# Deltares/xugrid

Hardware: AMD Instinct MI355X
Metric: target cells regridded/s (OverlapRegridder 1M->1M tri, weights + mean apply) (higher is better)
Workload: dtype f64; 1 GPU; BASELINE config 2: ~1M-triangle jittered-lattice Delaunay source -> ~1M-triangle target (seed 1, rotated 30 deg, scaled 0.7), OverlapRegridder area-weighted mean, K=1; target_faces=999660, candidate_pairs=6677422, nnz=4052965, parallelism=1 GPU

## Files before the change

include/xugrid_amd.h:

```cpp
#ifndef XUGRID_AMD_H
#define XUGRID_AMD_H

#include <stdint.h>

#ifdef __cplusplus
extern "C" {
#endif

#define XR_OK 0
#define XR_ERR_INVALID (-1)
#define XR_ERR_NO_DEVICE (-2)
#define XR_ERR_HIP (-3)
#define XR_ERR_LIMIT (-4)

#define XR_MEAN 0
#define XR_HARMONIC_MEAN 1
#define XR_GEOMETRIC_MEAN 2
#define XR_SUM 3
#define XR_MINIMUM 4
#define XR_MAXIMUM 5
#define XR_MODE 6
#define XR_PERCENTILE 7
#define XR_FIRST_ORDER_CONSERVATIVE 8
#define XR_MAX_OVERLAP 9
// ... 46 lines not shown
int xr_mesh_face_bounds_dev(xr_mesh *mesh, double *out_dev);

int xr_overlap(xr_mesh *tree, xr_mesh *query, int relative, xr_csr **out);
int xr_overlap_stats(const xr_mesh *tree, int64_t *n_candidates);
int xr_overlap_apply_dev(xr_mesh *tree, xr_mesh *query, int relative, int method, double percentile,
                         const void *source_dev, int source_dtype, int64_t K, double *out_dev, xr_csr **out);

int xr_locate_points(xr_mesh *mesh, const double *points, int64_t n, double tolerance,
                     int64_t *face_index_out);
int xr_locate_raster(xr_mesh *mesh, const double *x, int64_t nx, const double *y, int64_t ny,
                     double tolerance, int64_t *face_index_out);
int xr_barycentric(xr_mesh *mesh, const double *points, int64_t n, double tolerance,
                   int64_t *face_index_out, double *weights_out);

int xr_replace_interpolated_weights(const double *vertices, int64_t n_vertex, const int64_t *faces, int64_t n_face,
                                    int64_t m, const int64_t *face_index, double *weights, int64_t n,
                                    const int64_t *node_to_node_map, int64_t n_map);

int xr_locate_csr(xr_mesh *tree, xr_mesh *query, const double *points, int64_t n, double tolerance,
                  xr_csr **out);

int xr_barycentric_csr(xr_mesh *voronoi, xr_mesh *source, xr_mesh *query, const double *points,
                       int64_t n, double tolerance, const int64_t *vertex_face,
                       const int64_t *node_to_node_map, int64_t n_extra, xr_csr **out);
int xr_barycentric_csr_tail(xr_mesh *voronoi, xr_mesh *source, xr_mesh *query, const double *points, int64_t n,
                            double tolerance, int64_t n_identity, const int64_t *vertex_face_tail,
                            const int64_t *node_to_node_map, int64_t n_extra, int tree_order, xr_csr **out);

typedef struct xr_points xr_points;
int xr_locate_flags_begin(xr_mesh *source, xr_mesh *query, const double *points, int64_t n, xr_points **out);
int xr_points_destroy(xr_points *points);
int xr_barycentric_csr_points(xr_mesh *voronoi, xr_mesh *source, xr_points *points, double tolerance, int64_t n_identity,
                              const int64_t *vertex_face_tail, const int64_t *node_to_node_map, int64_t n_extra,
                              int tree_order, xr_csr **out);

typedef struct xr_voronoi xr_voronoi;
int xr_voronoi_create(xr_mesh *mesh, xr_voronoi **out);
int xr_voronoi_create_flags(xr_mesh *mesh, int add_exterior, int add_vertices, int skip_concave, const double *generators_dev,
                            xr_voronoi **out);
int xr_voronoi_vertex_info(const xr_voronoi *v, int64_t *n_generator_vertex, int64_t *max_used_face);
int xr_voronoi_info(const xr_voronoi *v, int64_t *n_node, int64_t *nnz, int64_t *n_exterior_edge,
                    int64_t *n_interior_cell, int64_t *max_interior_degree);
int xr_voronoi_download(const xr_voronoi *v, int64_t *indptr, int64_t *indices, int64_t *edge_nodes,
                        int64_t *edge_face, double *centroids);
int xr_voronoi_boundary_info(xr_voronoi *v, int64_t *n_boundary_node, int64_t *n_boundary_entry);
int xr_voronoi_boundary(xr_voronoi *v, int64_t *nodes, int64_t *row_ptr, int64_t *faces, double *face_xy,
                        int64_t *edge_nodes, int64_t *edge_face, double *edge_face_xy);
int xr_voronoi_mesh(const xr_voronoi *v, const double *extra_xy, int64_t n_extra_vertex,
                    const int64_t *boundary_cells, int64_t n_boundary_cell, int64_t n_max_boundary,
                    xr_mesh **out);
int xr_voronoi_mesh_auto(xr_voronoi *v, xr_mesh **out, int64_t *n_tail, int64_t *n_map);
int xr_voronoi_tail(xr_voronoi *v, int64_t *tail_face_index, int64_t *interpolation_map);
int xr_voronoi_boundary_cells_info(xr_voronoi *v, int64_t *n_extra_vertex, int64_t *n_cell, int64_t *n_max);
int xr_voronoi_boundary_cells(xr_voronoi *v, double *extra_xy, int64_t *cells);
int xr_voronoi_destroy(xr_voronoi *v);

int xr_csr_info(const xr_csr *csr, int64_t *n, int64_t *m, int64_t *nnz);
int xr_csr_download(const xr_csr *csr, double *data, int64_t *indices, int64_t *indptr);
int xr_csr_upload(const double *data, const int64_t *indices, const int64_t *indptr, int64_t n,
                  int64_t m, int64_t nnz, xr_csr **out);
int xr_csr_from_triplet(const int64_t *row, const int64_t *col, const double *data, int64_t nnz,
                        int64_t n, int64_t m, xr_csr **out);
int xr_csr_from_outer(const int64_t *indptr_y, const int64_t *source_y, const double *weight_y,
                      int64_t n_target_y, int64_t n_source_y, const int64_t *indptr_x,
                      const int64_t *source_x, const double *weight_x, int64_t n_target_x,
                      int64_t n_source_x, xr_csr **out);
int xr_outer_create(const int64_t *indptr_y, const int64_t *source_y, const double *weight_y,
                    int64_t n_target_y, int64_t n_source_y, const int64_t *indptr_x,
                    const int64_t *source_x, const double *weight_x, int64_t n_target_x,
                    int64_t n_source_x, xr_outer **out);
int xr_outer_info(const xr_outer *outer, int64_t *n, int64_t *m, int64_t *nnz);
int xr_outer_csr(xr_outer *outer, const xr_csr **out);
int xr_outer_destroy(xr_outer *outer);
int xr_edge_length_csr(xr_mesh *tree, const double *edge_xy, int64_t n_edge, xr_csr **out);
int xr_edge_length_csr_dev(xr_mesh *tree, const double *edge_xy_dev, int64_t n_edge, xr_csr **out);
int xr_edge_pieces(xr_mesh *tree, const xr_csr *csr, const double *edge_xy, int64_t n_edge,
                   double *intersections);
int xr_csr_set_row_keys(xr_csr *csr, const int64_t *keys, int64_t key_range);
int xr_csr_set_col_keys(xr_csr *csr, const int64_t *keys, int64_t key_range);
int xr_csr_col_order(const xr_csr *csr, int64_t *order_out);
int xr_csr_expect_permuted(xr_csr *csr, int permuted);
int xr_csr_output_stored_order(xr_csr *csr, int stored);
int xr_csr_row_order(const xr_csr *csr, int64_t K_hint, int64_t *order_out);
int xr_csr_destroy(xr_csr *csr);

int xr_apply_csr(const xr_csr *csr, int method, double percentile, const void *source,
                 int source_dtype, int64_t K, double *out);
int xr_apply_csr_dev(const xr_csr *csr, int method, double percentile, const void *source_dev,
                     int source_dtype, int64_t K, double *out_dev);
int xr_apply_outer(xr_outer *outer, int method, double percentile, const void *source,
                   int source_dtype, int64_t K, double *out);
int xr_apply_outer_dev(xr_outer *outer, int method, double percentile, const void *source_dev,
                       int source_dtype, int64_t K, double *out_dev);
int xr_apply_coo(const int64_t *row, const int64_t *col, int64_t nnz, int64_t T,
                 const void *source, int source_dtype, int64_t K, int64_t S, double *out);

int xr_shard_plan_dev(const double *src_xy_dev, const int64_t *src_faces_dev, int64_t n_src_face, int src_m,
                      const double *tgt_xy_dev, const int64_t *tgt_faces_dev, int64_t n_tgt_face, int tgt_m, int world, int rank,
                      int mode, int64_t *local_faces_dev, int64_t *n_local_faces, int64_t *local_targets_dev,
                      int64_t *n_local_targets, int32_t *owner_dev);

int xr_partial_components(int method);
int xr_partial_combine_is_max(int method);
int xr_apply_partial_dev(const xr_csr *csr, int method, const void *source_dev, int source_dtype, int64_t K,
                         double *out_dev, int rows_layout);
int xr_overlap_partial_dev(xr_mesh *tree, xr_mesh *query, int relative, int method, const void *source_dev, int source_dtype,
                           int64_t K, double *out_dev, int rows_layout, xr_csr **out);
int xr_partial_fill_identity_dev(int method, double *planes_dev, int64_t K, int64_t T);
int xr_finalize_partial_dev(int method, const double *planes_dev, int64_t K, int64_t T, double *out_dev);
int xr_reduce_partial_rows_dev(int method, const double *rows_dev, const int64_t *indptr_dev, const int64_t *order_dev,
                               int64_t n_targets, int64_t K, double *out_dev);

typedef struct xr_graph xr_graph;
int xr_graph_from_csr(const int64_t *indptr, const int64_t *indices, const double *data, int64_t n, int64_t nnz,
                      const int64_t *labels, xr_graph **out);
int xr_graph_info(const xr_graph *graph, int64_t *n, int64_t *nnz);
int xr_graph_download(const xr_graph *graph, int64_t *indptr, int64_t *indices, double *data, int64_t *labels);
int xr_graph_destroy(xr_graph *graph);
#define XR_FILL_CONVERGED 0
#define XR_FILL_MAXITER 1
#define XR_FILL_BREAKDOWN 2
#define XR_FILL_NODATA 3
int xr_graph_laplace_fill_dev(const xr_graph *graph, const double *in_dev, double *out_dev, int64_t K, int use_weights,
                              double atol, double rtol, int64_t maxiter, int64_t chunk, int64_t *iterations_out,
                              int *status_out);
int xr_nearest_fill_dev(const double *xy_dev, int64_t n, const double *in_dev, double *out_dev, int64_t K, double max_distance);

typedef struct xr_topology xr_topology;
int xr_topology_create(xr_mesh *mesh, xr_topology **out);
int xr_topology_info(const xr_topology *topology, int64_t *n_edge, int64_t *n_exterior_edge, int64_t *face_face_nnz,
                     int64_t *node_node_nnz, int64_t *n_nonmanifold);
int xr_topology_long_nodes(const xr_topology *topology, int64_t *n_long_nodes);
int xr_topology_download(const xr_topology *topology, int64_t *edge_node, int64_t *face_edge, int64_t *edge_face,
                         int64_t *ff_indptr, int64_t *ff_indices, int64_t *ff_data, int64_t *nn_indptr, int64_t *nn_indices,
                         int64_t *nn_data, int64_t *exterior_edge, int64_t *exterior_face);
int xr_topology_edge_xy_dev(const xr_topology *topology, double *xy_dev);
int xr_topology_exterior_face_dev(const xr_topology *topology, uint8_t *flags_dev);
int xr_topology_destroy(xr_topology *topology);
int xr_topology_download_node_tables(const xr_topology *topology, int64_t *nf_indptr, int64_t *nf_indices, int64_t *ne_indptr,
                                     int64_t *ne_indices);
int xr_graph_from_topology(const xr_topology *topology, int facet, xr_graph **out);
int xr_graph_label_rounds(const xr_graph *graph, int64_t *rounds);

int xr_graph_components_dev(const xr_graph *graph, int64_t *labels_dev, int64_t *n_components);
int xr_graph_binary_iterate_dev(const xr_graph *graph, const uint8_t *in_dev, uint8_t *out_dev, int64_t K, int value,
                                int64_t iterations, const uint8_t *mask_dev, const uint8_t *exterior_dev);

int xr_graph_rcm_dev(const xr_graph *graph, int64_t *order_dev, int64_t *levels_out);

int xr_graph_partition_dev(const xr_graph *graph, const double *xy_dev, const int64_t *weights_dev, int64_t n_part,
                           int64_t *labels_dev, int64_t *info);
int xr_mesh_reorder_faces_dev(const xr_mesh *mesh, const int64_t *order_dev, xr_mesh **out);

int xr_network_graph_dev(const double *node_xy_dev, int64_t n_node, const int64_t *edges_dev, int64_t n_edge, int facet,
                         xr_graph **out, int64_t *problems);
int xr_graph_nearest_dev(const xr_graph *graph, const uint8_t *is_source_dev, int64_t K, double limit, int64_t chunk,
                         double *distance_dev, int64_t *source_dev, int64_t *rounds_out);
int xr_graph_nearest_fill_dev(const xr_graph *graph, const double *in_dev, double *out_dev, int64_t K, double limit,
                              int64_t chunk, int64_t *rounds_out);

#define XR_FACET_MEAN 0
#define XR_FACET_SUM 1
#define XR_FACET_MIN 2
#define XR_FACET_MAX 3
#define XR_FACET_RAW 4
int xr_topology_facet_map_dev(xr_topology *topology, int target, int source, int form, const void *in_dev, int dtype, int64_t K,
// ... 139 lines not shown
```

xugrid_amd/_lib.py:

```python
import ctypes
import os

_HERE = os.path.dirname(os.path.abspath(__file__))
LIB_PATH = os.environ.get("XUGRID_AMD_LIB") or os.path.join(_HERE, "libxugrid_amd.so")

XR_OK = 0
XR_ERR_INVALID = -1
XR_ERR_NO_DEVICE = -2
XR_ERR_HIP = -3
XR_ERR_LIMIT = -4

XR_F64 = 0
XR_F32 = 1
XR_I32 = 2


class XugridAmdError(RuntimeError):
    """HIP runtime failure, missing device or missing shared library."""


c_i64 = ctypes.c_int64
c_f64 = ctypes.c_double
c_int = ctypes.c_int
vp = ctypes.c_void_p
# ... 2 lines not shown
p_int = ctypes.POINTER(ctypes.c_int)
p_vp = ctypes.POINTER(ctypes.c_void_p)

SIGNATURES = {
    "xr_last_error": (ctypes.c_char_p, []),
    "xr_device_count": (c_int, [p_int]),
    "xr_init": (c_int, [c_int]),
    "xr_current_device": (c_int, [p_int]),
    "xr_trim_pool": (c_int, []),
    "xr_version": (c_int, []),
    "xr_set_stream": (c_int, [vp, c_int, c_int]),
    "xr_set_async": (c_int, [c_int]),
    "xr_set_option": (c_int, [ctypes.c_char_p, ctypes.c_int64]),
    "xr_get_option": (c_int, [ctypes.c_char_p, ctypes.POINTER(ctypes.c_int64)]),
    "xr_host_copy": (c_int, [vp, vp, c_i64]),
    "xr_host_interleave2": (c_int, [vp, c_i64, vp, c_i64, c_i64, vp]),
    "xr_mesh_create": (c_int, [vp, c_i64, vp, c_int, c_i64, c_i64, c_i64, p_vp]),
    "xr_mesh_create_dev": (c_int, [vp, c_i64, vp, c_int, c_i64, c_i64, c_i64, p_vp]),
    "xr_mesh_create_rectilinear": (c_int, [vp, c_i64, vp, c_i64, p_vp]),
    "xr_mesh_destroy": (c_int, [vp]),
    "xr_mesh_info": (c_int, [vp, p_i64, p_i64, p_i64]),
    "xr_mesh_device_bytes": (c_int, [vp, p_i64]),
    "xr_mesh_prepare": (c_int, [vp]),
    "xr_mesh_build_index": (c_int, [vp]),
    "xr_mesh_invalidate": (c_int, [vp]),
    "xr_mesh_area": (c_int, [vp, vp]),
    "xr_mesh_centroids": (c_int, [vp, vp]),
    "xr_mesh_centroids_dev": (c_int, [vp, vp]),
    "xr_mesh_faces": (c_int, [vp, vp]),
    "xr_mesh_download": (c_int, [vp, vp, vp]),
    "xr_mesh_triangulate": (c_int, [vp, p_vp]),
    "xr_mesh_triangle_face_dev": (c_int, [vp, vp]),
    "xr_mesh_circumcenters_dev": (c_int, [vp, vp]),
    "xr_mesh_perimeter_dev": (c_int, [vp, vp]),
    "xr_mesh_face_bounds_dev": (c_int, [vp, vp]),
    "xr_voronoi_create": (c_int, [vp, p_vp]),
    "xr_voronoi_create_flags": (c_int, [vp, c_int, c_int, c_int, vp, p_vp]),
    "xr_voronoi_vertex_info": (c_int, [vp, p_i64, p_i64]),
    "xr_voronoi_info": (c_int, [vp, p_i64, p_i64, p_i64, p_i64, p_i64]),
    "xr_voronoi_download": (c_int, [vp, vp, vp, vp, vp, vp]),
    "xr_voronoi_boundary_info": (c_int, [vp, vp, vp]),
    "xr_voronoi_boundary": (c_int, [vp, vp, vp, vp, vp, vp, vp, vp]),
    "xr_voronoi_mesh": (c_int, [vp, vp, c_i64, vp, c_i64, c_i64, p_vp]),
    "xr_voronoi_mesh_auto": (c_int, [vp, p_vp, p_i64, p_i64]),
    "xr_voronoi_tail": (c_int, [vp, vp, vp]),
    "xr_voronoi_boundary_cells_info": (c_int, [vp, p_i64, p_i64, p_i64]),
    "xr_voronoi_boundary_cells": (c_int, [vp, vp, vp]),
    "xr_voronoi_destroy": (c_int, [vp]),
    "xr_overlap": (c_int, [vp, vp, c_int, p_vp]),
    "xr_overlap_stats": (c_int, [vp, p_i64]),
    "xr_overlap_apply_dev": (c_int, [vp, vp, c_int, c_int, c_f64, vp, c_int, c_i64, vp, p_vp]),
    "xr_overlap_partial_dev": (c_int, [vp, vp, c_int, c_int, vp, c_int, c_i64, vp, c_int, p_vp]),
    "xr_shard_plan_dev": (c_int, [vp, vp, c_i64, c_int, vp, vp, c_i64, c_int, c_int, c_int, c_int, vp, p_i64, vp, p_i64, vp]),
    "xr_locate_points": (c_int, [vp, vp, c_i64, c_f64, vp]),
    "xr_locate_raster": (c_int, [vp, vp, c_i64, vp, c_i64, c_f64, vp]),
    "xr_barycentric": (c_int, [vp, vp, c_i64, c_f64, vp, vp]),
    "xr_locate_csr": (c_int, [vp, vp, vp, c_i64, c_f64, p_vp]),
    "xr_replace_interpolated_weights": (c_int, [vp, c_i64, vp, c_i64, c_i64, vp, vp, c_i64, vp, c_i64]),
    "xr_barycentric_csr": (c_int, [vp, vp, vp, vp, c_i64, c_f64, vp, vp, c_i64, p_vp]),
    "xr_barycentric_csr_tail": (c_int, [vp, vp, vp, vp, c_i64, c_f64, c_i64, vp, vp, c_i64, c_int, p_vp]),
    "xr_locate_flags_begin": (c_int, [vp, vp, vp, c_i64, p_vp]),
    "xr_points_destroy": (c_int, [vp]),
    "xr_barycentric_csr_points": (c_int, [vp, vp, vp, c_f64, c_i64, vp, vp, c_i64, c_int, p_vp]),
    "xr_csr_info": (c_int, [vp, p_i64, p_i64, p_i64]),
    "xr_csr_download": (c_int, [vp, vp, vp, vp]),
    "xr_csr_upload": (c_int, [vp, vp, vp, c_i64, c_i64, c_i64, p_vp]),
    "xr_csr_from_triplet": (c_int, [vp, vp, vp, c_i64, c_i64, c_i64, p_vp]),
    "xr_csr_from_outer": (c_int, [vp, vp, vp, c_i64, c_i64, vp, vp, vp, c_i64, c_i64, p_vp]),
    "xr_outer_create": (c_int, [vp, vp, vp, c_i64, c_i64, vp, vp, vp, c_i64, c_i64, p_vp]),
    "xr_outer_info": (c_int, [vp, vp, vp, vp]),
    "xr_outer_csr": (c_int, [vp, p_vp]),
    "xr_outer_destroy": (c_int, [vp]),
    "xr_apply_outer": (c_int, [vp, c_int, c_f64, vp, c_int, c_i64, vp]),
    "xr_apply_outer_dev": (c_int, [vp, c_int, c_f64, vp, c_int, c_i64, vp]),
    "xr_edge_length_csr": (c_int, [vp, vp, c_i64, p_vp]),
    "xr_edge_length_csr_dev": (c_int, [vp, vp, c_i64, p_vp]),
    "xr_edge_pieces": (c_int, [vp, vp, vp, c_i64, vp]),
    "xr_csr_set_row_keys": (c_int, [vp, vp, c_i64]),
    "xr_csr_set_col_keys": (c_int, [vp, vp, c_i64]),
    "xr_csr_col_order": (c_int, [vp, vp]),
    "xr_csr_expect_permuted": (c_int, [vp, c_int]),
    "xr_csr_output_stored_order": (c_int, [vp, c_int]),
    "xr_csr_row_order": (c_int, [vp, c_i64, vp]),
    "xr_csr_destroy": (c_int, [vp]),
    "xr_apply_csr": (c_int, [vp, c_int, c_f64, vp, c_int, c_i64, vp]),
    "xr_apply_csr_dev": (c_int, [vp, c_int, c_f64, vp, c_int, c_i64, vp]),
    "xr_apply_coo": (c_int, [vp, vp, c_i64, c_i64, vp, c_int, c_i64, c_i64, vp]),
    "xr_partial_components": (c_int, [c_int]),
    "xr_partial_combine_is_max": (c_int, [c_int]),
    "xr_apply_partial_dev": (c_int, [vp, c_int, vp, c_int, c_i64, vp, c_int]),
    "xr_partial_fill_identity_dev": (c_int, [c_int, vp, c_i64, c_i64]),
    "xr_finalize_partial_dev": (c_int, [c_int, vp, c_i64, c_i64, vp]),
    "xr_reduce_partial_rows_dev": (c_int, [c_int, vp, vp, vp, c_i64, c_i64, vp]),
    "xr_graph_from_csr": (c_int, [vp, vp, vp, c_i64, c_i64, vp, p_vp]),
    "xr_graph_info": (c_int, [vp, p_i64, p_i64]),
    "xr_graph_download": (c_int, [vp, vp, vp, vp, vp]),
    "xr_graph_destroy": (c_int, [vp]),
    "xr_graph_laplace_fill_dev": (c_int, [vp, vp, vp, c_i64, c_int, c_f64, c_f64, c_i64, c_i64, vp, vp]),
    "xr_nearest_fill_dev": (c_int, [vp, c_i64, vp, vp, c_i64, c_f64]),
    "xr_network_graph_dev": (c_int, [vp, c_i64, vp, c_i64, c_int, p_vp, p_i64]),
    "xr_graph_nearest_dev": (c_int, [vp, vp, c_i64, c_f64, c_i64, vp, vp, p_i64]),
    "xr_graph_nearest_fill_dev": (c_int, [vp, vp, vp, c_i64, c_f64, c_i64, p_i64]),
    "xr_topology_create": (c_int, [vp, p_vp]),
    "xr_topology_info": (c_int, [vp, p_i64, p_i64, p_i64, p_i64, p_i64]),
    "xr_topology_long_nodes": (c_int, [vp, p_i64]),
    "xr_topology_download": (c_int, [vp, vp, vp, vp, vp, vp, vp, vp, vp, vp, vp, vp]),
    "xr_topology_download_node_tables": (c_int, [vp, vp, vp, vp, vp]),
    "xr_topology_edge_xy_dev": (c_int, [vp, vp]),
    "xr_topology_exterior_face_dev": (c_int, [vp, vp]),
    "xr_topology_destroy": (c_int, [vp]),
    "xr_graph_from_topology": (c_int, [vp, c_int, p_vp]),
    "xr_graph_label_rounds": (c_int, [vp, p_i64]),
    "xr_graph_components_dev": (c_int, [vp, vp, p_i64]),
    "xr_graph_binary_iterate_dev": (c_int, [vp, vp, vp, c_i64, c_int, c_i64, vp, vp]),
    "xr_graph_rcm_dev": (c_int, [vp, vp, p_i64]),
    "xr_mesh_reorder_faces_dev": (c_int, [vp, vp, p_vp]),
    "xr_graph_partition_dev": (c_int, [vp, vp, vp, c_i64, vp, p_i64]),
    "xr_topology_facet_map_dev": (c_int, [vp, c_int, c_int, c_int, vp, c_int, c_i64, vp]),
    "xr_topology_facet_width": (c_int, [vp, c_int, c_int, p_i64]),
    "xr_facet_map_dev": (c_int, [vp, vp, c_i64, c_i64, c_i64, c_int, vp, c_int, c_i64, vp]),
    "xr_nn_create_dev": (c_int, [vp, c_i64, p_vp]),
    "xr_nn_create_mesh": (c_int, [vp, c_int, p_vp]),
    "xr_nn_info": (c_int, [vp, p_i64, p_i64]),
    "xr_nn_destroy": (c_int, [vp]),
    "xr_nn_query_dev": (c_int, [vp, vp, c_i64, c_f64, vp]),
    "xr_gather_points_dev": (c_int, [vp, c_int, c_i64, c_i64, vp, c_i64, c_f64, vp]),
    "xr_section_coords_dev": (c_int, [vp, vp, c_i64, vp, c_i64, vp, vp]),
    "xr_burn_polygons_dev": (c_int, [vp, vp, c_i64, vp, c_i64, vp, c_i64, c_int, vp]),
    "xr_burn_lines_dev": (c_int, [vp, vp, c_i64, vp, c_i64, vp]),
    "xr_burn_points_dev": (c_int, [vp, vp, c_i64, vp]),
    "xr_burn_combine_dev": (c_int, [c_i64, vp, vp, vp, vp, vp, vp, c_f64, vp]),
    "xr_polygonize_dev": (c_int, [vp, vp, c_int, p_vp]),
    "xr_polygons_info": (c_int, [vp, p_i64, p_i64, p_i64, p_i64, p_i64]),
    "xr_polygons_readbacks": (c_int, [vp, p_i64]),
    "xr_polygons_copy_dev": (c_int, [vp, vp, vp, vp, vp, vp]),
    "xr_polygons_destroy": (c_int, [vp]),
    "xr_mesh_subset_dev": (c_int, [vp, vp, c_i64, p_vp, p_int, p_i64]),
    "xr_mesh_subset_node_index_dev": (c_int, [vp, vp]),
    "xr_index_check_dev": (c_int, [vp, c_i64, c_i64, p_i64]),
    "xr_index_mismatch_dev": (c_int, [vp, vp, c_i64, p_i64]),
    "xr_index_from_mask_dev": (c_int, [vp, c_i64, p_vp]),
    "xr_mesh_box_faces_dev": (c_int, [vp, c_f64, c_f64, c_f64, c_f64, p_vp]),
    "xr_mesh_faces_of_nodes_dev": (c_int, [vp, vp, c_i64, p_vp]),
    "xr_topology_faces_of_edges_dev": (c_int, [vp, vp, c_i64, p_vp]),
    "xr_topology_subset_edges_dev": (c_int, [vp, vp, c_i64, p_vp]),
    "xr_index_info": (c_int, [vp, p_i64]),
    "xr_index_copy_dev": (c_int, [vp, vp]),
    "xr_index_destroy": (c_int, [vp]),
    "xr_merge_meshes_dev": (c_int, [vp, c_i64, p_vp]),
    "xr_merge_edges_dev": (c_int, [vp, vp, c_i64, vp]),
    "xr_merge_info": (c_int, [vp, p_i64, p_i64, p_i64]),
    "xr_merge_take_mesh": (c_int, [vp, p_vp]),
    "xr_merge_index_info": (c_int, [vp, c_int, c_i64, p_i64]),
    "xr_merge_index_copy_dev": (c_int, [vp, c_int, c_i64, c_int, vp]),
    "xr_merge_node_inverse_copy_dev": (c_int, [vp, vp]),
    "xr_merge_destroy": (c_int, [vp]),
    "xr_index_like_dev": (c_int, [vp, vp, c_i64, c_f64, vp, p_i64]),
    "xr_labels_range_dev": (c_int, [vp, c_i64, p_i64, p_i64]),
    "xr_labels_order_dev": (c_int, [vp, c_i64, c_i64, p_vp, p_i64]),
    "xr_label_order_copy_dev": (c_int, [vp, c_i64, c_i64, vp]),
    "xr_label_order_destroy": (c_int, [vp]),
    "xr_dev_copy_columns": (c_int, [vp, c_i64, vp, c_i64, c_i64]),
    "xr_periodic_wrap_dev": (c_int, [vp, p_vp, p_i64]),
    "xr_periodic_unwrap_dev": (c_int, [vp, c_f64, p_vp]),
    "xr_periodic_edges_dev": (c_int, [vp, vp, vp, p_i64]),
    "xr_periodic_info": (c_int, [vp, p_i64]),
# ... 80 lines not shown
```

xugrid_amd/csrc/xr_apply.hip:

```cpp
#include <cstdlib>
#include <cstring>
#include <vector>

#include "xr_apply.h"
#include "xr_reduce.h"
#include "xr_prims.h"

namespace xr {

static constexpr int KT = 16;

template <int METHOD, typename SRC>
__device__ __forceinline__ void apply_row_block(const int32_t *__restrict__ indptr, const int32_t *__restrict__ indices,
                                                const double *__restrict__ data, const int32_t *__restrict__ row_order,
                                                int t, int64_t T, int64_t S, const SRC *__restrict__ source, int64_t K,
                                                double *__restrict__ out, double (*lds)[3]) {
    const int s = indptr[t], e = indptr[t + 1];
    const int64_t t_out = row_order ? (int64_t)row_order[t] : t;
    double normsum = 0.0;
    if (METHOD == XR_GEOMETRIC_MEAN) {
        Red<XR_SUM> ws;
        for (int j = s + threadIdx.x; j < e; j += AP_BLOCK) ws.b += data[j];
        block_merge<XR_SUM>(ws, lds);
        normsum = ws.b;
    }
    for (int64_t k = blockIdx.y; k < K; k += gridDim.y) {
        const SRC *src = source + k * S;
        Red<METHOD> r;
        int j = s + threadIdx.x;
        for (; j + 3 * AP_BLOCK < e; j += 4 * AP_BLOCK) {
            const int c0 = indices[j], c1 = indices[j + AP_BLOCK], c2 = indices[j + 2 * AP_BLOCK],
                      c3 = indices[j + 3 * AP_BLOCK];
            const double w0 = data[j], w1 = data[j + AP_BLOCK], w2 = data[j + 2 * AP_BLOCK],
                         w3 = data[j + 3 * AP_BLOCK];
            const double v0 = ld_src(src, c0), v1 = ld_src(src, c1), v2 = ld_src(src, c2), v3 = ld_src(src, c3);
            r.add(v0, w0, normsum);
            r.add(v1, w1, normsum);
            r.add(v2, w2, normsum);
            r.add(v3, w3, normsum);
        }
        for (; j < e; j += AP_BLOCK) r.add(ld_src(src, indices[j]), data[j], normsum);
        block_merge<METHOD>(r, lds);
        if (threadIdx.x == 0) {
            double v = r.fin();
            if (METHOD == XR_GEOMETRIC_MEAN && normsum == 0) v = NAN;
            out[k * T + t_out] = v;
        }
    }
}

template <int METHOD, typename SRC>
__global__ void __launch_bounds__(AP_BLOCK)
k_apply_long(const int32_t *__restrict__ indptr, const int32_t *__restrict__ indices, const double *__restrict__ data,
             const int32_t *__restrict__ row_order, const int32_t *__restrict__ long_rows,
             const int32_t *__restrict__ n_long, int64_t T, int64_t S, const SRC *__restrict__ source, int64_t K,
             double *__restrict__ out) {
    __shared__ double lds[AP_BLOCK / 64][3];
    const int nl = *n_long;
    for (int li = blockIdx.x; li < nl; li += gridDim.x)
        apply_row_block<METHOD, SRC>(indptr, indices, data, row_order, long_rows[li], T, S, source, K, out, lds);
}

static constexpr int APPLY_GROUP16 = 512;

template <int METHOD, typename SRC, int KTILE, int G>
__device__ __forceinline__ void apply_row_group(const int32_t *__restrict__ indices, const double *__restrict__ data,
                                                int s, int e, int64_t t_out, int64_t T, int64_t S,
                                                const SRC *__restrict__ source, int64_t K, double *__restrict__ out) {
    const int gl = threadIdx.x & (G - 1);
    int col4[4];
    double w4[4];
#pragma unroll
    for (int u = 0; u < 4; u++) {
        const int j = s + gl + G * u;
        col4[u] = j < e ? indices[j] : -1;
        w4[u] = j < e ? data[j] : 0.0;
    }
    double normsum = 0.0;
    if (METHOD == XR_GEOMETRIC_MEAN) {
        Red<XR_SUM> ws;
        for (int j = s + gl; j < e; j += G) ws.b += data[j];
        group_merge<XR_SUM, G>(ws);
        normsum = ws.b;
    }
    for (int64_t k0 = (int64_t)blockIdx.y * KTILE; k0 < K; k0 += (int64_t)gridDim.y * KTILE) {
        const int kn = (int)((K - k0) < KTILE ? (K - k0) : KTILE);
        const SRC *src = source + k0 * S;
        Red<METHOD> r[KTILE];
        double v[4][KTILE];
#pragma unroll
        for (int u = 0; u < 4; u++)
#pragma unroll
            for (int kk = 0; kk < KTILE; kk++)
                v[u][kk] = (col4[u] >= 0 && kk < kn) ? ld_src(src, (int64_t)kk * S + col4[u]) : 0.0;
#pragma unroll
        for (int u = 0; u < 4; u++) {
            if (col4[u] >= 0) {
#pragma unroll
                for (int kk = 0; kk < KTILE; kk++)
                    if (kk < kn) r[kk].add(v[u][kk], w4[u], normsum);
            }
        }
        for (int j = s + gl + 4 * G; j < e; j += G) {
            const int64_t col = indices[j];
            const double w = data[j];
            double vv[KTILE];
#pragma unroll
            for (int kk = 0; kk < KTILE; kk++) vv[kk] = kk < kn ? ld_src(src, (int64_t)kk * S + col) : 0.0;
#pragma unroll
            for (int kk = 0; kk < KTILE; kk++)
                if (kk < kn) r[kk].add(vv[kk], w, normsum);
        }
#pragma unroll
        for (int kk = 0; kk < KTILE; kk++) group_merge<METHOD, G>(r[kk]);
        if (gl == 0) {
#pragma unroll
            for (int kk = 0; kk < KTILE; kk++) {
                if (kk < kn) {
                    double res = r[kk].fin();
                    if (METHOD == XR_GEOMETRIC_MEAN && normsum == 0) res = NAN;
                    out[(k0 + kk) * T + t_out] = res;
                }
            }
        }
    }
}

template <int METHOD, typename SRC, int KTILE>
__device__ __forceinline__ void apply_wave_rows(const int32_t *__restrict__ indptr, const int32_t *__restrict__ indices,
                                                const double *__restrict__ data, const int32_t *__restrict__ row_order,
                                                const int32_t *__restrict__ long_rows, int nl, int wave, int n_waves,
                                                int64_t T, int64_t S, const SRC *__restrict__ source, int64_t K,
                                                double *__restrict__ out, int32_t *__restrict__ huge_rows) {
    const int lane = threadIdx.x & 63;
    for (int li0 = wave * 4; li0 < nl; li0 += n_waves * 4) {
        const int li = li0 + (lane >> 4);
        int s = 0, e = 0;
        int64_t t_out = 0;
        if (li < nl) {
            const int t = long_rows[li];
            s = indptr[t];
            e = indptr[t + 1];
            t_out = row_order ? (int64_t)row_order[t] : t;
            if (e - s > APPLY_GROUP16) e = s;
        }
        if (__any(e > s)) {
            if (e > s) apply_row_group<METHOD, SRC, KTILE, 16>(indices, data, s, e, t_out, T, S, source, K, out);
        }
    }
    for (int li = wave; li < nl; li += n_waves) {
        const int t = long_rows[li];
        const int s = indptr[t], e = indptr[t + 1];
        if (e - s <= APPLY_GROUP16) continue;
        if (e - s > APPLY_WAVE) {
            if (huge_rows && lane == 0 && blockIdx.y == 0) huge_rows[1 + atomicAdd(huge_rows, 1)] = t;
            continue;
        }
        const int64_t t_out = row_order ? (int64_t)row_order[t] : t;
        apply_row_group<METHOD, SRC, KTILE, 64>(indices, data, s, e, t_out, T, S, source, K, out);
    }
}

template <int METHOD, typename SRC, int KTILE>
__global__ void __launch_bounds__(AP_BLOCK)
k_apply_wave(const int32_t *__restrict__ indptr, const int32_t *__restrict__ indices, const double *__restrict__ data,
             const int32_t *__restrict__ row_order, const int32_t *__restrict__ long_rows,
             const int32_t *__restrict__ n_long, int64_t T, int64_t S, const SRC *__restrict__ source, int64_t K,
             double *__restrict__ out, int32_t *__restrict__ huge_rows) {
    const int wave = (blockIdx.x * AP_BLOCK + threadIdx.x) >> 6, n_waves = gridDim.x * (AP_BLOCK / 64);
    apply_wave_rows<METHOD, SRC, KTILE>(indptr, indices, data, row_order, long_rows, *n_long, wave, n_waves, T, S, source, K,
                                        out, huge_rows);
}

template <int METHOD, typename SRC>
__global__ void __launch_bounds__(AP_BLOCK)
k_apply_rows1(const int32_t *__restrict__ indptr, const int32_t *__restrict__ indices, const double *__restrict__ data,
              const int32_t *__restrict__ row_order, const int32_t *__restrict__ long_rows,
              const int32_t *__restrict__ n_long, int n_long_blocks, bool any_huge, int64_t T, int64_t S,
              const SRC *__restrict__ source, double *__restrict__ out, const int32_t *__restrict__ gate) {
    __shared__ double2 sh_win[AP_BLOCK / 64][W1_CAP];
    if (gate && *gate == 0) return;
    double(*sh_merge)[3] = reinterpret_cast<double(*)[3]>(&sh_win[0][0]);
    const int lane = threadIdx.x & 63, wib = threadIdx.x >> 6;
    if ((int)blockIdx.x < n_long_blocks) {
        const int nl = *n_long;
        apply_wave_rows<METHOD, SRC, 1>(indptr, indices, data, row_order, long_rows, nl, (int)blockIdx.x * (AP_BLOCK / 64) + wib,
                                        n_long_blocks * (AP_BLOCK / 64), T, S, source, 1, out, nullptr);
        if (any_huge) {
            int *sh_list = reinterpret_cast<int *>(&sh_win[1][0]), *sh_cnt = reinterpret_cast<int *>(&sh_win[2][0]);
            for (int base = 0; base < nl; base += n_long_blocks * AP_BLOCK) {
                if (threadIdx.x == 0) *sh_cnt = 0;
                __syncthreads();
                const int li = base + (int)blockIdx.x + n_long_blocks * (int)threadIdx.x;
                if (li < nl) {
                    const int t = long_rows[li];
                    if (indptr[t + 1] - indptr[t] > APPLY_WAVE) sh_list[atomicAdd(sh_cnt, 1)] = t;
                }
                __syncthreads();
                const int n_hit = *sh_cnt;
                for (int i = 0; i < n_hit; i++)
                    apply_row_block<METHOD, SRC>(indptr, indices, data, row_order, sh_list[i], T, S, source, 1, out, sh_merge);
                __syncthreads();
            }
        }
        return;
    }
    const int64_t row0 = ((int64_t)(gridDim.x - 1 - blockIdx.x) * (AP_BLOCK / 64) + wib) * 64;
    if (row0 >= T) return;
    const int64_t t = row0 + lane;
    int s = 0, e = 0;
    if (t < T) {
        s = indptr[t];
        e = indptr[t + 1];
    }
    const bool skip = n_long_blocks > 0 && (e - s > APPLY_LONG);
    const int seg0 = __shfl(s, 0, 64);
    const int seg1 = wave_reduce<OpMax>(e);
    if (skip) e = s;
    const bool jumpy = __any(skip);
    double2 *win = sh_win[wib];
    auto next_chunk = [&](int c0) -> int {
        if (!jumpy) return c0;
        int mine = (e > s && e > c0) ? (s > c0 ? s : c0) : INT_MAX;
        return wave_reduce<OpMin>(mine);
    };
    double normsum = 0.0;
    if (METHOD == XR_GEOMETRIC_MEAN) {
        for (int c0 = seg0; c0 < seg1; c0 += W1_CAP) {
            c0 = next_chunk(c0);
            if (c0 >= seg1) break;
            for (int j = c0 + lane; j < c0 + W1_CAP && j < seg1; j += 64) win[j - c0].x = data[j];
            __builtin_amdgcn_fence(__ATOMIC_RELEASE, "wavefront");
            __builtin_amdgcn_wave_barrier();
            __builtin_amdgcn_fence(__ATOMIC_ACQUIRE, "wavefront");
            const int a = s > c0 ? s : c0, b = e < c0 + W1_CAP ? e : c0 + W1_CAP;
            for (int j = a; j < b; j++) normsum += win[j - c0].x;
            __builtin_amdgcn_fence(__ATOMIC_RELEASE, "wavefront");
            __builtin_amdgcn_wave_barrier();
        }
    }
    Red<METHOD> red;
    for (int c0 = seg0; c0 < seg1; c0 += W1_CAP) {
        c0 = next_chunk(c0);
        if (c0 >= seg1) break;
        {
            constexpr int PER = W1_CAP / 64;
            int col[PER];
            double w[PER];
#pragma unroll
            for (int u = 0; u < PER; u++) {
                const int j = c0 + u * 64 + lane;
                col[u] = j < seg1 ? indices[j] : -1;
                w[u] = j < seg1 ? data[j] : 0.0;
            }
            double v[PER];
#pragma unroll
            for (int u = 0; u < PER; u++) v[u] = col[u] >= 0 ? ld_src(source, (int64_t)col[u]) : 0.0;
#pragma unroll
            for (int u = 0; u < PER; u++)
                if (col[u] >= 0) win[u * 64 + lane] = make_double2(w[u], v[u]);
        }
        __builtin_amdgcn_fence(__ATOMIC_RELEASE, "wavefront");
        __builtin_amdgcn_wave_barrier();
        __builtin_amdgcn_fence(__ATOMIC_ACQUIRE, "wavefront");
        const int a = s > c0 ? s : c0, b = e < c0 + W1_CAP ? e : c0 + W1_CAP;
        for (int j = a; j < b; j++) {
            const double2 wv = win[j - c0];
            red.add(wv.y, wv.x, normsum);
        }
        __builtin_amdgcn_fence(__ATOMIC_RELEASE, "wavefront");
        __builtin_amdgcn_wave_barrier();
    }
    if (t < T && !skip) {
        const int64_t t_out = row_order ? (int64_t)row_order[t] : t;
        double r = NAN;
        if (e > s) {
            r = red.fin();
            if (METHOD == XR_GEOMETRIC_MEAN && normsum == 0) r = NAN;
        }
        out[t_out] = r;
    }
}

template <int METHOD, typename SRC, int KTILE>
__global__ void __launch_bounds__(AP_BLOCK)
k_apply_direct(const int32_t *__restrict__ indptr, const int32_t *__restrict__ indices,
               const double *__restrict__ data, const int32_t *__restrict__ row_order, bool skip_long, int64_t T,
               int64_t S, const SRC *__restrict__ source, int64_t K, double *__restrict__ out,
               const int32_t *__restrict__ block_list) {
    const int64_t t = (int64_t)(block_list ? block_list[blockIdx.x] : blockIdx.x) * AP_BLOCK + threadIdx.x;
    if (t >= T) return;
    const int64_t k0 = (int64_t)blockIdx.y * KTILE;
    const int kn = (int)((K - k0) < KTILE ? (K - k0) : KTILE);
    const int s = indptr[t], e = indptr[t + 1];
    if (skip_long && e - s > APPLY_LONG) return;
    const int64_t t_out = row_order ? (int64_t)row_order[t] : t;
    const SRC *src = source + k0 * S;
    double normsum = 0.0;
    if (METHOD == XR_GEOMETRIC_MEAN)
        for (int j = s; j < e; j++) normsum += data[j];
    Red<METHOD> red[KTILE];
    int j = s;
    if (KTILE <= 4) {
        for (; j + 3 < e; j += 4) {
            int64_t col[4];
            double w[4], v[4][KTILE];
#pragma unroll
            for (int u = 0; u < 4; u++) {
                col[u] = indices[j + u];
                w[u] = data[j + u];
            }
#pragma unroll
            for (int u = 0; u < 4; u++)
#pragma unroll
                for (int kk = 0; kk < KTILE; kk++) v[u][kk] = kk < kn ? ld_src(src, (int64_t)kk * S + col[u]) : 0.0;
#pragma unroll
            for (int u = 0; u < 4; u++)
#pragma unroll
                for (int kk = 0; kk < KTILE; kk++)
                    if (kk < kn) red[kk].add(v[u][kk], w[u], normsum);
        }
    }
    for (; j < e; j++) {
        const int64_t col = indices[j];
        const double w = data[j];
        double v[KTILE];
#pragma unroll
        for (int kk = 0; kk < KTILE; kk++) v[kk] = kk < kn ? ld_src(src, (int64_t)kk * S + col) : 0.0;
#pragma unroll
        for (int kk = 0; kk < KTILE; kk++)
            if (kk < kn) red[kk].add(v[kk], w, normsum);
    }
#pragma unroll
    for (int kk = 0; kk < KTILE; kk++) {
        if (kk < kn) {
            double r = NAN;
            if (e > s) {
                r = red[kk].fin();
                if (METHOD == XR_GEOMETRIC_MEAN && normsum == 0) r = NAN;
            }
            out[(k0 + kk) * T + t_out] = r;
        }
    }
}

static constexpr int PLAN_LMAX = 4096;
static constexpr int PLAN_UMAX = 512;

__global__ void __launch_bounds__(AP_BLOCK)
k_plan_build(const int32_t *__restrict__ indptr, const int32_t *__restrict__ indices, int64_t T,
             int32_t *__restrict__ ucol, int32_t *__restrict__ nuniq, uint16_t *__restrict__ loc,
             int32_t *__restrict__ max_entries, int32_t *__restrict__ unplanned, int32_t *__restrict__ n_unplanned,
             int entry_cap) {
    __shared__ int32_t keys[PLAN_LMAX];
    __shared__ int32_t uniq[PLAN_UMAX];
    __shared__ int32_t sh_wave[4];
    __shared__ int32_t sh_lines;
    const int64_t row0 = (int64_t)blockIdx.x * AP_BLOCK;
    const int64_t row_end = row0 + AP_BLOCK < T ? row0 + AP_BLOCK : T;
    const int seg0 = indptr[row0], seg1 = indptr[row_end];
    const int n = seg1 - seg0;
    if (n > entry_cap) {
        if (threadIdx.x == 0) {
            nuniq[blockIdx.x] = -1;
// ... 700 lines not shown

template <int METHOD, typename SRC, int KT, int SUBS, bool MERGED, bool FAST>
static void launch_plan(const xr_csr *csr, const SRC *src, int64_t K, double *out) {
    const int plan_dbg = (int)option(OPT_PLAN_DBG);
    const int lmax = csr->plan_lmax;
    const size_t sub_bytes = ((sizeof(double) * ((size_t)KT * PLAN_UMAX + lmax) + sizeof(uint16_t) * lmax) + 15) / 16 * 16;
    const size_t stage_bytes = ((sizeof(double) * (size_t)lmax + sizeof(uint16_t) * (size_t)lmax) + 15) / 16 * 16;
    const size_t shmem = MERGED ? sizeof(double) * (size_t)KT * PLAN_GUMAX + stage_bytes * PLAN_GROUP : sub_bytes * SUBS;
    XR_REQUIRE(shmem <= (size_t)160 * 1024, XR_ERR_LIMIT, "internal: apply plan needs %zu bytes of LDS", shmem);
    {
        static std::mutex attr_mutex;
        static size_t granted = 0;
        std::lock_guard<std::mutex> lock(attr_mutex);
        if (shmem > granted) {
            XR_HIP(hipFuncSetAttribute(reinterpret_cast<const void *>(&k_apply_plan<METHOD, SRC, KT, SUBS, MERGED, FAST>),
                                       hipFuncAttributeMaxDynamicSharedMemorySize, (int)shmem));
            granted = shmem;
        }
    }
    const int64_t n_groups = div_up(div_up(csr->n, AP_BLOCK), SUBS);
    const int item_tiles = 64 / KT;
    const int super_blocks = K > (int64_t)KT * item_tiles ? (int)std::min<int64_t>((n_groups + 7) / 8, 1 << 30) : 0;
    int64_t plan_grid = (n_groups + 7) / 8 * 8;
    if (super_blocks > 0) {
        const int64_t per_xcd = (n_groups + 7) / 8;
        const int64_t n_items = div_up(K, (int64_t)KT * item_tiles);
        plan_grid = 8 * div_up(per_xcd, super_blocks) * super_blocks * n_items;
    }
    XR_LAUNCH("apply_plan", (k_apply_plan<METHOD, SRC, KT, SUBS, MERGED, FAST>), dim3((unsigned)plan_grid), dim3(AP_BLOCK * SUBS),
              shmem, csr->indptr.get(), csr->indices.get(), csr->data.get(), csr->plan_ucol.get(), csr->plan_nuniq.get(),
              csr->plan_loc.get(), row_order_of(csr), csr->has_long, csr->n, csr->m, src, K, out, csr->plan_lmax, super_blocks,
              item_tiles, plan_dbg);
}

template <int METHOD, typename SRC>
static void launch_stream(const xr_csr *csr, const SRC *src, int64_t K, double *out) {
    DevBuf<int32_t> huge;
    if (csr->has_long) huge.alloc((size_t)(csr->nnz / APPLY_WAVE + 2));
    auto launch_long_rows = [&](bool zeroed) {
        if (!zeroed) XR_HIP(hipMemsetAsync(huge.get(), 0, sizeof(int32_t), launch_stream()));
        if (K == 1) {
            dim3 wgrid((unsigned)engine().num_cu * 16, 1);
            XR_LAUNCH("apply_wave", (k_apply_wave<METHOD, SRC, 1>), wgrid, dim3(AP_BLOCK), 0, csr->indptr.get(),
                      csr->indices.get(), csr->data.get(), row_order_of(csr), csr->long_rows.get(), csr->n_long.get(),
                      csr->n, csr->m, src, K, out, huge.get());
        } else {
            constexpr int WT = 8;
            const unsigned wy = (unsigned)std::min<int64_t>(div_up(K, WT), 8);
            dim3 wgrid((unsigned)engine().num_cu * 16 / wy, wy);
            XR_LAUNCH("apply_wave", (k_apply_wave<METHOD, SRC, WT>), wgrid, dim3(AP_BLOCK), 0, csr->indptr.get(),
                      csr->indices.get(), csr->data.get(), row_order_of(csr), csr->long_rows.get(), csr->n_long.get(),
                      csr->n, csr->m, src, K, out, huge.get());
        }
        if (csr->max_row_len >= 0 && csr->max_row_len <= APPLY_WAVE) return;
        const unsigned gy = (unsigned)(K < 8 ? K : 8);
        dim3 grid((unsigned)engine().num_cu * (8 / gy), gy);
        XR_LAUNCH("apply_long", (k_apply_long<METHOD, SRC>), grid, dim3(AP_BLOCK), 0, csr->indptr.get(),
                  csr->indices.get(), csr->data.get(), row_order_of(csr), huge.get() + 1, huge.get(),
                  csr->n, csr->m, src, K, out);
    };
    const bool long_on_side = csr->has_long && K >= PLAN_KT;
    const bool use_plan = K > 1 && K >= PLAN_KT && option(OPT_APPLY_PLAN) != 0;
    if (use_plan) {
        ensure_tiled(csr);
        ensure_plan(csr);
    }
    auto launch_unplanned = [&]() {
        if (csr->plan_n_unplanned <= 0) return;
        dim3 grid((unsigned)csr->plan_n_unplanned, div_up(K, 4));
        XR_LAUNCH("apply_direct", (k_apply_direct<METHOD, SRC, 4>), grid, dim3(AP_BLOCK), 0, csr->indptr.get(),
                  csr->indices.get(), csr->data.get(), row_order_of(csr), csr->has_long, csr->n, csr->m, src, K, out,
                  csr->plan_unplanned.get());
    };
    const bool side_late = long_on_side && use_plan && side_mark();
    if (long_on_side && !side_late) {
        SideScope side;
        launch_long_rows(false);
        if (use_plan) launch_unplanned();
    }
    if (K == 1) {
        const int n_long_blocks = csr->has_long ? engine().num_cu / 2 : 0;
        const bool any_huge = csr->has_long && !(csr->max_row_len >= 0 && csr->max_row_len <= APPLY_WAVE);
        dim3 grid((unsigned)(div_up(csr->n, AP_BLOCK) + n_long_blocks), 1);
        XR_LAUNCH("apply_rows1", (k_apply_rows1<METHOD, SRC>), grid, dim3(AP_BLOCK), 0, csr->indptr.get(), csr->indices.get(),
                  csr->data.get(), row_order_of(csr), csr->long_rows.get(), csr->n_long.get(), n_long_blocks, any_huge,
                  csr->n, csr->m, src, out, csr->apply_gated ? csr->n_long.get() + 1 : (const int32_t *)nullptr);
    } else {
        if (use_plan) {
            constexpr bool FAST_OK = METHOD == XR_MEAN || METHOD == XR_FIRST_ORDER_CONSERVATIVE;
            const bool fast = FAST_OK && option(OPT_APPLY_CONTRACT) != 0;
            if (csr->plan_merged && fast) launch_plan<METHOD, SRC, 4, PLAN_GROUP, true, FAST_OK>(csr, src, K, out);
            else if (csr->plan_merged) launch_plan<METHOD, SRC, 4, PLAN_GROUP, true, false>(csr, src, K, out);
            else if (fast) launch_plan<METHOD, SRC, PLAN_KT, 1, false, FAST_OK>(csr, src, K, out);
            else launch_plan<METHOD, SRC, PLAN_KT, 1, false, false>(csr, src, K, out);
            if (side_late) {
                SideScope side(true);
                launch_long_rows(false);
                launch_unplanned();
            } else if (!long_on_side) {
                launch_unplanned();
            }
        } else {
            dim3 grid(div_up(csr->n, AP_BLOCK), div_up(K, KT));
            XR_LAUNCH("apply_direct", (k_apply_direct<METHOD, SRC, KT>), grid, dim3(AP_BLOCK), 0, csr->indptr.get(),
                      csr->indices.get(), csr->data.get(), row_order_of(csr), csr->has_long, csr->n, csr->m, src, K,
                      out, (const int32_t *)nullptr);
        }
    }
    if (csr->has_long && K > 1 && !long_on_side) launch_long_rows(false);
    if (long_on_side) side_join();
}

template <int METHOD, typename SRC>
static void launch_workspace(const xr_csr *csr, const SRC *src, int64_t K, double p, double *out) {
    int64_t kchunk = csr->nnz > 0 ? ((int64_t)64 << 20) / csr->nnz : K;
    if (kchunk < 1) kchunk = 1;
    if (kchunk > K) kchunk = K;
    if (kchunk > 65535) kchunk = 65535;
    DevBuf<double> ws((size_t)kchunk * (size_t)(csr->nnz > 0 ? csr->nnz : 1));
    for (int64_t k0 = 0; k0 < K; k0 += kchunk) {
        const int64_t kc = (K - k0) < kchunk ? (K - k0) : kchunk;
        dim3 grid(div_up(csr->n, AP_BLOCK), (unsigned)kc);
        XR_LAUNCH("apply_workspace", (k_apply_workspace<METHOD, SRC>), grid, dim3(AP_BLOCK), 0, csr->indptr.get(),
                  csr->indices.get(), csr->data.get(), row_order_of(csr), csr->n, csr->m, csr->nnz, src, k0, p,
                  ws.get(), out, csr->has_long);
    }
    if (csr->has_long) {
        const unsigned gy = (unsigned)std::min<int64_t>(K, 16);
        dim3 grid((unsigned)engine().num_cu * 32 / gy, gy);
        XR_LAUNCH("apply_sorted", (k_apply_sorted<METHOD, SRC>), grid, dim3(64), 0, csr->indptr.get(), csr->indices.get(),
                  csr->data.get(), row_order_of(csr), csr->long_rows.get(), csr->n_long.get(), csr->n, csr->m, src, K, p,
                  out);
    }
}

template <typename SRC>
static void apply_dispatch(const xr_csr *csr, int method, double p, const SRC *src, int64_t K, double *out) {
    if (csr->n == 0 || K == 0) return;
    with_reducer(method, [&](auto m) {
        constexpr int METHOD = decltype(m)::value;
        if constexpr (streamed_reducer<METHOD>) {
            launch_stream<METHOD, SRC>(csr, src, K, out);
        } else {
            if (METHOD == XR_PERCENTILE)
                XR_REQUIRE(p >= 0.0 && p <= 100.0, XR_ERR_INVALID,
                           "percentile must be in the range [0, 100], received: %g", p);
            launch_workspace<METHOD, SRC>(csr, src, K, p, out);
        }
    });
}

static void apply_dev(const xr_csr *csr, int method, double p, const void *src, int dtype, int64_t K, double *out) {
    with_source_type(dtype, [&](auto tag) {
        using SRC = decltype(tag);
        DevBuf<char> permuted;
        apply_dispatch<SRC>(csr, method, p, stored_source(csr, static_cast<const SRC *>(src), K, permuted), K, out);
    });
}

void csr_apply_dev(const xr_csr *csr, int method, double percentile, const void *src_dev, int dtype, int64_t K, double *out_dev) {
    apply_dev(csr, method, percentile, src_dev, dtype, K, out_dev);
}

}

using namespace xr;

extern "C" {

// ... 69 lines not shown
```

xugrid_amd/csrc/xr_csr.hip:

```cpp
#include <vector>

#include "xr_apply.h"
#include "xr_prims.h"

namespace xr {

__global__ void k_narrow_i64(const int64_t *__restrict__ in, int32_t *__restrict__ out, int64_t n) {
    const int64_t i = (int64_t)blockIdx.x * 256 + threadIdx.x;
    if (i < n) out[i] = (int32_t)in[i];
}
__global__ void k_bincount(const int32_t *__restrict__ row, int64_t nnz, int32_t *__restrict__ count) {
    const int64_t i = (int64_t)blockIdx.x * 256 + threadIdx.x;
    if (i < nnz) atomicAdd(&count[row[i]], 1);
}

__global__ void k_gather_i32(const int32_t *__restrict__ table, const int32_t *__restrict__ idx, int64_t n,
                             int32_t *__restrict__ out) {
    const int64_t i = (int64_t)blockIdx.x * 256 + threadIdx.x;
    if (i < n) out[i] = table[idx[i]];
}
__global__ void k_scatter_iota_i32(const int32_t *__restrict__ perm, int64_t n, int32_t *__restrict__ inverse) {
    const int64_t i = (int64_t)blockIdx.x * 256 + threadIdx.x;
    if (i < n) inverse[perm[i]] = (int32_t)i;
}
// ... 289 lines not shown
        csr->tile_key_range = key_range;
        csr->has_tile_key = key_range > 1;
    }
    XR_API_END
}

int xr_csr_set_col_keys(xr_csr *csr, const int64_t *keys, int64_t key_range) {
    XR_API_BEGIN
    XR_REQUIRE(csr && (keys || csr->m == 0), XR_ERR_INVALID, "xr_csr_set_col_keys: NULL argument");
    XR_REQUIRE(key_range >= 1 && key_range <= ((int64_t)1 << 24), XR_ERR_INVALID,
               "xr_csr_set_col_keys: key_range must be in [1, 2^24]");
    XR_REQUIRE(!csr->has_col_perm, XR_ERR_INVALID, "xr_csr_set_col_keys: the columns of this matrix are renumbered already");
    for (int64_t i = 0; i < csr->m; i++)
        XR_REQUIRE(keys[i] >= 0 && keys[i] < key_range, XR_ERR_INVALID, "xr_csr_set_col_keys: key %lld outside [0,%lld)",
                   (long long)keys[i], (long long)key_range);
    const int64_t m = csr->m;
    if (m > 0 && key_range > 1) {
        DevBuf<int32_t> key((size_t)m), hist((size_t)key_range + 1), start((size_t)key_range + 1), members((size_t)m),
            rank((size_t)m);
        upload_narrow(keys, m, key.get());
        fill_i32(hist.get(), 0, key_range + 1);
        XR_LAUNCH("bincount", k_bincount, dim3(div_up(m, 256)), dim3(256), 0, key.get(), m, hist.get());
        exclusive_scan_i32(hist.get(), start.get(), key_range);
        fill_i32(hist.get(), 0, key_range + 1);
        XR_LAUNCH("tile_scatter", k_tile_scatter, dim3(div_up(m, 256)), dim3(256), 0, key.get(), m, start.get(), hist.get(),
                  members.get());
        csr->col_of.alloc((size_t)m);
        XR_LAUNCH("tile_rank", k_tile_rank, dim3(div_up(m, 256)), dim3(256), 0, key.get(), start.get(), members.get(), m,
                  csr->col_of.get());
        XR_LAUNCH("col_inverse", k_scatter_iota_i32, dim3(div_up(m, 256)), dim3(256), 0, csr->col_of.get(), m, rank.get());
        if (csr->nnz > 0)
            XR_LAUNCH("col_relabel", k_relabel_i32, dim3(div_up(csr->nnz, 256)), dim3(256), 0, rank.get(),
                      csr->indices.get(), csr->nnz);
        stream_sync();
        csr->has_col_perm = true;
        csr->plan_ready = false;
    }
    XR_API_END
}

int xr_csr_col_order(const xr_csr *csr, int64_t *order_out) {
    XR_API_BEGIN
    XR_REQUIRE(csr && (order_out || csr->m == 0), XR_ERR_INVALID, "xr_csr_col_order: NULL argument");
    if (csr->has_col_perm) {
        DevBuf<int64_t> wide((size_t)csr->m);
        download_wide(csr->col_of.get(), csr->m, order_out, wide);
        stream_sync();
    } else {
        for (int64_t i = 0; i < csr->m; i++) order_out[i] = i;
    }
    XR_API_END
}

int xr_csr_expect_permuted(xr_csr *csr, int permuted) {
    XR_API_BEGIN
    XR_REQUIRE(csr, XR_ERR_INVALID, "xr_csr_expect_permuted: NULL argument");
    csr->source_permuted = permuted != 0;
    XR_API_END
}

int xr_csr_output_stored_order(xr_csr *csr, int stored) {
    XR_API_BEGIN
    XR_REQUIRE(csr, XR_ERR_INVALID, "xr_csr_output_stored_order: NULL argument");
    if (stored) settle_row_layout(csr);
    csr->output_stored = stored != 0;
    XR_API_END
}

int xr_csr_row_order(const xr_csr *csr, int64_t K_hint, int64_t *order_out) {
    XR_API_BEGIN
    (void)K_hint;
    XR_REQUIRE(csr && (order_out || csr->n == 0), XR_ERR_INVALID, "xr_csr_row_order: NULL argument");
    settle_row_layout(csr);
    if (csr->has_row_order) {
        DevBuf<int64_t> wide((size_t)csr->n);
        download_wide(csr->row_order.get(), csr->n, order_out, wide);
        stream_sync();
    } else {
        for (int64_t i = 0; i < csr->n; i++) order_out[i] = i;
    }
    XR_API_END
}

int xr_csr_destroy(xr_csr *csr) {
    XR_API_BEGIN
    if (csr) {
        release_point();
        delete csr;
    }
    XR_API_END
}

}
```

xugrid_amd/csrc/xr_engine.hip:

```cpp
#include <cstdarg>

#include <algorithm>
#include <atomic>
#include <chrono>
#include <map>
#include <cstring>
#include <thread>
#include <condition_variable>
#include <functional>

#include "xr_internal.h"

namespace xr {

static thread_local char g_err[512] = "";

void set_error(const char *fmt, ...) {
    va_list ap;
    va_start(ap, fmt);
    vsnprintf(g_err, sizeof(g_err), fmt, ap);
    va_end(ap);
}

std::recursive_mutex &engine_mutex() {
    static std::recursive_mutex m;
    return m;
}
std::shared_mutex &engine_rw() {
    static std::shared_mutex m;
    return m;
}

static thread_local int t_exclusive_depth = 0;
static thread_local Lane *t_lane = nullptr;
static constexpr int N_LANES = 4;
static Lane g_lanes[N_LANES];
static std::mutex g_pool_mutex;
static std::mutex g_main_turn;

Lane *current_lane() { return t_lane; }
bool exclusive_held() { return t_exclusive_depth > 0; }

static thread_local hipStream_t t_stream_override = nullptr;
hipStream_t stream_override() { return t_stream_override; }
StreamOverride::StreamOverride(hipStream_t s) : prev(t_stream_override) { t_stream_override = s; }
StreamOverride::~StreamOverride() { t_stream_override = prev; }

namespace {
struct OptionDef {
    const char *name;
    int64_t def;
};
const OptionDef k_option_defs[] = {
    {"overlap_fused", 1}, {"queue_margin", 0}, {"clip_quad", 1}, {"dust", 1}, {"debug", 0}, {"host_stamps", 0}, {"apply_plan", 1},
    {"apply_contract", 0}, {"plan_merge", -1}, {"plan_dbg", 0}, {"apply_chunk_bytes", 0}, {"outer_apply", 0}, {"edge_big", 0},
    {"edge_stage", 0}, {"edge_queue", 0}, {"edge_sort", 1}, {"nn_query_sort", -1}, {"burn_strips", 0},
    {"facet_tile", 0}, {"scan_fused_tiles", 0}, {"merge_table_slack", 0},
    {"front_fused", 1},
};
static_assert(sizeof(k_option_defs) / sizeof(k_option_defs[0]) == OPT_COUNT, "one table row per enum Option");
std::atomic<int64_t> g_options[OPT_COUNT];
std::once_flag g_options_once;
int64_t option_word(const char *v) {
    static const struct { const char *word; int64_t value; } words[] = {{"free", 1}, {"csr", 2}};
    for (const auto &w : words)
        if (!strcmp(v, w.word)) return w.value;
    char *end = nullptr;
    const long long n = strtoll(v, &end, 10);
    return end && end != v ? (int64_t)n : 0;
}
void options_init() {
    std::call_once(g_options_once, [] {
        for (int i = 0; i < OPT_COUNT; i++) {
            char env[64] = "XR_";
            size_t k = 3;
            for (const char *c = k_option_defs[i].name; *c && k + 1 < sizeof(env); c++) env[k++] = (char)toupper((unsigned char)*c);
            env[k] = 0;
            const char *v = getenv(env);
            g_options[i].store(v ? option_word(v) : k_option_defs[i].def, std::memory_order_relaxed);
        }
    });
}
int option_index(const char *name) {
    for (int i = 0; i < OPT_COUNT; i++)
        if (!strcmp(name, k_option_defs[i].name)) return i;
    return -1;
}
}
int64_t option(Option o) {
    options_init();
    return g_options[o].load(std::memory_order_relaxed);
}

static thread_local bool t_mark_open = false;
ExclusiveScope::ExclusiveScope() {
    if (t_exclusive_depth++ == 0) {
        t_mark_open = false;
        engine_mutex().lock();
        engine_rw().lock();
    }
}
ExclusiveScope::~ExclusiveScope() {
    if (--t_exclusive_depth == 0) {
        engine_rw().unlock();
        engine_mutex().unlock();
    }
}

static void lane_release_blocks(Lane *lane);

SharedScope::SharedScope() {
    if (t_exclusive_depth > 0 || t_lane) return;
    t_mark_open = false;
    engine_rw().lock_shared();
    leased = true;
    Engine &e = engine();
    if (e.stream != e.own_stream || e.own_async) {
        g_main_turn.lock();
        serial = true;
        return;
    }
    const size_t h = std::hash<std::thread::id>()(std::this_thread::get_id());
    Lane *lane = nullptr;
    for (int i = 0; i < N_LANES && !lane; i++) {
        Lane &c = g_lanes[(h + i) % N_LANES];
        if (c.busy.try_lock()) lane = &c;
    }
    if (!lane) {
        lane = &g_lanes[h % N_LANES];
        lane->busy.lock();
    }
    if (!lane->stream) {
        if (hipStreamCreateWithFlags(&lane->stream, hipStreamNonBlocking) != hipSuccess) {
            (void)hipGetLastError();
            lane->stream = nullptr;
            lane->busy.unlock();
            engine_rw().unlock_shared();
            leased = false;
            set_error("could not create a HIP stream for a concurrent apply");
            throw Failure{XR_ERR_HIP};
        }
// ... 945 lines not shown
```

xugrid_amd/csrc/xr_internal.h:

```cpp
#pragma once
#include <memory>

#include <hip/hip_runtime.h>

#include <cstdint>
#include <cstdio>
#include <cstring>
#include <map>
#include <functional>
#include <mutex>
#include <shared_mutex>
#include <string>
#include <type_traits>
#include <vector>

#include "../../include/xugrid_amd.h"

namespace xr {

void set_error(const char *fmt, ...);

struct Failure {
    int code;
};
// ... 148 lines not shown
    return v;
}

struct ProfScope {
    const char *name;
    hipEvent_t e0 = nullptr, e1 = nullptr;
    bool on_side = false;
    hipStream_t lane_stream = nullptr;
    explicit ProfScope(const char *name);
    ~ProfScope();
};
void prof_flush();

#define XR_LAUNCH(name, kernel, grid, block, shmem, ...)                                        \
    do {                                                                                        \
        xr::ProfScope _ps(name);                                                                \
        hipLaunchKernelGGL(kernel, grid, block, shmem, xr::launch_stream(), __VA_ARGS__);       \
        XR_HIP(hipGetLastError());                                                              \
    } while (0)

struct Lane {
    hipStream_t stream = nullptr;
    char *stage[2] = {nullptr, nullptr};
    hipEvent_t stage_ev[2] = {nullptr, nullptr};
    hipStream_t side = nullptr;
    hipEvent_t fork_event = nullptr, join_event = nullptr;
    bool on_side = false;
    bool side_active = false;
    std::mutex busy;
};
Lane *current_lane();
bool exclusive_held();

hipStream_t stream_override();
inline hipStream_t launch_stream() {
    if (hipStream_t s = stream_override()) return s;
    if (Lane *l = current_lane()) return l->on_side ? l->side : l->stream;
    return engine().on_side ? engine().side : engine().stream;
}
struct StreamOverride {
    explicit StreamOverride(hipStream_t s);
    ~StreamOverride();
    hipStream_t prev;
};

struct SideScope {
    explicit SideScope(bool at_mark = false);
    ~SideScope();
    int mode = 0;
};
struct SideForkScope {
    SideForkScope();
    void end_launches();
    ~SideForkScope();
    bool active = false, launching = false;
    hipStream_t prev = nullptr;
};
void side_join();
bool side_mark();

enum Option : int {
    OPT_OVERLAP_FUSED,
    OPT_QUEUE_MARGIN,
    OPT_CLIP_QUAD,
    OPT_DUST,
    OPT_DEBUG,
    OPT_HOST_STAMPS,
    OPT_APPLY_PLAN,
    OPT_APPLY_CONTRACT,
    OPT_PLAN_MERGE,
    OPT_PLAN_DBG,
    OPT_APPLY_CHUNK_BYTES,
    OPT_OUTER_APPLY,
    OPT_EDGE_BIG,
    OPT_EDGE_STAGE,
    OPT_EDGE_QUEUE,
    OPT_EDGE_SORT,
    OPT_NN_QUERY_SORT,
    OPT_BURN_STRIPS,
    OPT_FACET_TILE,
    OPT_SCAN_FUSED_TILES,
    OPT_MERGE_TABLE_SLACK,
    OPT_FRONT_FUSED,
    OPT_COUNT
};
int64_t option(Option o);

inline unsigned div_up(int64_t a, int64_t b) { return (unsigned)((a + b - 1) / b); }

template <typename F> void with_nodes_per_face(int m, F &&f) {
    if (m == 3) f(std::integral_constant<int, 3>());
    else if (m == 4) f(std::integral_constant<int, 4>());
    else f(std::integral_constant<int, 0>());
}

template <typename F> void with_source_type(int dtype, F &&f) {
    XR_REQUIRE(dtype == XR_F64 || dtype == XR_F32, XR_ERR_INVALID, "unsupported source dtype id %d", dtype);
    if (dtype == XR_F64) f(double());
    else f(float());
}

template <auto KERNEL> void allow_dynamic_lds(size_t bytes) {
    static const bool set = [&] {
        XR_HIP(hipFuncSetAttribute(reinterpret_cast<const void *>(KERNEL), hipFuncAttributeMaxDynamicSharedMemorySize, (int)bytes));
        return true;
    }();
    (void)set;
}

enum class OnFailure { FreeOnly, WaitFirst };
template <typename T> struct Building {
    std::unique_ptr<T> p{new T()};
    OnFailure rule;
    explicit Building(OnFailure r = OnFailure::FreeOnly) : rule(r) {}
    Building(const Building &) = delete;
    Building &operator=(const Building &) = delete;
    ~Building() {
        if (!p || rule != OnFailure::WaitFirst) return;
        try {
            stream_sync();
        } catch (const Failure &) {
        }
    }
    T *operator->() const { return p.get(); }
    T *get() const { return p.get(); }
    T *release() { return p.release(); }
};

void exclusive_scan_i32(const int32_t *in, int32_t *out, int64_t n, int32_t *host_total = nullptr,
                        const int32_t *extra_src = nullptr, int32_t *extra_host = nullptr);
void fill_i32(int32_t *p, int32_t v, int64_t n);
void fill_f64(double *p, double v, int64_t n);

}
```

xugrid_amd/csrc/xr_objects.h:

```cpp
#pragma once
#include <memory>
#include <vector>

#include "xr_geom.h"
#include "xr_internal.h"

struct xr_mesh {
    int64_t n_node = 0, n_face = 0;
    int m = 0;

    xr::DevBuf<double> node_xy;
    xr::DevBuf<int32_t> faces_raw;

    bool prepared = false;
    bool has_attrs = false;
    bool area_valid = false;
    xr::DevBuf<double> fxy;
    bool fxy_valid = false;
    xr::DevBuf<int32_t> fxy_off;
    xr::DevBuf<uint8_t> len;
    xr::DevBuf<double> bbox;
    xr::DevBuf<double> area;
    hipEvent_t centroids_event = nullptr;
    hipStream_t centroids_stream = nullptr;
    std::shared_ptr<xr::DevBuf<double>> centroids_dev;
    xr::DevBuf<double> stats;
    bool stats_valid = false;
    bool stats_sampled = false;
    double h_stats[8] = {0, 0, 0, 0, 0, 0, 0, 0};
    double *stats_host = nullptr;
    hipEvent_t stats_event = nullptr;
    xr::DevBuf<unsigned> stats_done;
    double stats_seq = 0.0;
    bool stats_event_pending = false;
    bool stats_polled = false;
    xr_mesh() = default;
    xr_mesh(const xr_mesh &) = delete;
    xr_mesh &operator=(const xr_mesh &) = delete;
    ~xr_mesh() {
        if (stats_host) (void)hipHostFree(stats_host);
        if (centroids_event) (void)hipEventDestroy(centroids_event);
        if (stats_event) (void)hipEventDestroy(stats_event);
    }

    bool query_ready = false;
    bool query_identity = false;
    xr::DevBuf<int32_t> q_perm;
    xr::DevBuf<double> q_fxy;
    xr::DevBuf<int32_t> q_off;
    xr::DevBuf<uint8_t> q_len;
    xr::DevBuf<double> q_bbox;

    bool indexed = false;
    xr::GridParams grid{};
    xr::DevBuf<int32_t> cell_start;
    xr::DevBuf<float> rec_bb;
    xr::DevBuf<int32_t> rec_face;
    xr::DevBuf<double> rec_fxy;
    xr::DevBuf<int32_t> rec_off;
    xr::DevBuf<uint8_t> rec_len;

    int64_t last_candidates = 0;

    xr::DevBuf<int32_t> tri_face;
    bool is_triangulation = false;

    xr::DevBuf<int32_t> sub_node;
    bool is_subset = false;

    std::vector<int64_t> bary_ids_host;
    xr::DevBuf<int64_t> bary_ids;
    int64_t bary_n_identity = -1, bary_n_extra = -1;
    xr::DevBuf<uint8_t> bary_cell_flag;
    bool bary_flag_valid = false;

    bool ragged() const { return m > xr::DENSE_MAX_NODES; }
    const int32_t *caller_off() const { return ragged() ? fxy_off.get() : nullptr; }
    const int32_t *record_off() const { return ragged() ? rec_off.get() : nullptr; }
    const int32_t *qo_off() const { return !ragged() ? nullptr : query_identity ? fxy_off.get() : q_off.get(); }
    const double *qo_fxy() const { return query_identity ? fxy.get() : q_fxy.get(); }
    const uint8_t *qo_len() const { return query_identity ? len.get() : q_len.get(); }
    const double *qo_bbox() const { return query_identity ? bbox.get() : q_bbox.get(); }
    const int32_t *qo_perm() const { return query_identity ? nullptr : q_perm.get(); }
};

static constexpr int XR_APPLY_LONG_ROW = 32;
static constexpr int XR_APPLY_WAVE_ROW = 2048;

struct xr_csr {
    int64_t n = 0, m = 0, nnz = 0;
    xr::DevBuf<int32_t> indptr;
    xr::DevBuf<int32_t> indices;
    xr::DevBuf<double> data;
    xr::DevBuf<int32_t> row_order;
    bool has_row_order = false;
    xr::DevBuf<int32_t> long_rows;
    xr::DevBuf<int32_t> n_long;
    bool apply_gated = false;
    int64_t max_row_len = -1;
    bool has_long = false;
    xr::DevBuf<int32_t> tile_key;
    bool has_tile_key = false;
    int64_t tile_key_range = 0;
    xr::DevBuf<int32_t> col_of;
    bool has_col_perm = false;
    bool source_permuted = false;
    bool output_stored = false;
    bool plan_ready = false;
    bool plan_merged = false;
    xr::DevBuf<int32_t> plan_unplanned;
    int plan_n_unplanned = 0;
    int plan_lmax = 0;
    xr::DevBuf<int32_t> plan_ucol;
    xr::DevBuf<int32_t> plan_nuniq;
    xr::DevBuf<uint16_t> plan_loc;
};

struct xr_outer {
    int64_t nty = 0, nsy = 0, ntx = 0, nsx = 0, Py = 0, Px = 0;
    xr::DevBuf<int32_t> ipy, ipx;
    xr::DevBuf<int32_t> sy, sx;
    xr::DevBuf<double> wy, wx;
    xr::DevBuf<int32_t> tx;
    int64_t max_cy = 0, max_cx = 0;
    xr_csr *csr = nullptr;
    ~xr_outer() { delete csr; }
};

struct xr_graph {
    int64_t n = 0, nnz = 0;
    xr::DevBuf<int32_t> indptr;
    xr::DevBuf<int32_t> indices;
    xr::DevBuf<double> data;
    xr::DevBuf<int32_t> labels;
    bool has_data = false;
    int64_t label_rounds = 0;
};

namespace xr {
void label_components(xr_graph *g);
void mesh_prepare_pair(xr_mesh *tree, xr_mesh *query);
void mesh_prepare(xr_mesh *mesh, bool want_fxy = true, bool stats_on_side = false, bool allow_sampled = false);
const double *mesh_area(xr_mesh *mesh);
void mesh_face_coords(xr_mesh *mesh);
void mesh_query_order(xr_mesh *mesh);
void mesh_build_index(xr_mesh *mesh);
void flush_pending_points();
void flush_pending_points_of(const xr_mesh *mesh);
void mesh_read_stats(xr_mesh *mesh, bool need_exact = false);
void csr_apply_dev(const xr_csr *csr, int method, double percentile, const void *src_dev, int dtype, int64_t K, double *out_dev);
void csr_partial_dev(const xr_csr *csr, int method, const void *src_dev, int dtype, int64_t K, double *out_dev, int rows_layout);
void mesh_centroids_dev(xr_mesh *mesh, double *cxy_dev);
std::shared_ptr<xr::DevBuf<double>> mesh_centroids_shared(xr_mesh *mesh);
double locate_points_dev(xr_mesh *mesh, const double *pts_dev, int64_t n, double tolerance, int64_t *out_dev);
void mesh_faces_ccw_dev(xr_mesh *mesh, int64_t *faces_dev, bool caller_order = false);
}
```

xugrid_amd/csrc/xr_overlap.hip:

```cpp
#include "xr_objects.h"
#include "xr_clip_tri.h"
#include "xr_prims.h"

namespace xr {

static constexpr int BIG_VISITS = 160;

__device__ __forceinline__ bool rec_hit(float4 b, float qx0, float qx1, float qy0, float qy1) {
    return box_gap(b, qx0, qx1, qy0, qy1) < 0.0f;
}

static constexpr int SLOTS = 16;
static constexpr int QCUR_STRIDE = 32;
static constexpr int TILE_RUN = 16;

__device__ __forceinline__ int64_t xcd_block(int64_t n_blocks, bool remap) {
    if (!remap) return blockIdx.x;
    const int64_t per_xcd = (n_blocks + 7) >> 3;
    return (int64_t)(blockIdx.x & 7) * per_xcd + (blockIdx.x >> 3);
}

static constexpr int WALK_PAD = 8;
static constexpr int BIGREC_MAX = 1024;
static constexpr int BIGREC_BLOCK = 64;

template <bool PACK, int MC>
__global__ void __launch_bounds__(256)
k_search(const double *__restrict__ q_bbox, const double *__restrict__ q_fxy, const uint8_t *__restrict__ q_len,
         int64_t n_query, GridParams g, int64_t n_tree,
         const int32_t *__restrict__ cell_start,
         const float *__restrict__ rec_bb, int32_t *__restrict__ cand_count, int32_t *__restrict__ cand_off,
         int32_t *__restrict__ cand_tgt, int32_t *__restrict__ cand_src, int32_t *__restrict__ queue_cursor,
         int2 *__restrict__ block_seg, uint8_t *__restrict__ is_big, int32_t *__restrict__ big_list,
         int32_t *__restrict__ n_big, MortonParams tile, int32_t *__restrict__ tile_key, int32_t *__restrict__ nnz_row,
         bool remap, int32_t *__restrict__ blk_rows = nullptr ,
         int32_t *__restrict__ blk_surv = nullptr ,
         int region_cap = 0 ) {
    __shared__ __attribute__((aligned(16))) int32_t sh_slots[SLOTS + 1][256];
    __shared__ uint8_t sh_owner[PACK ? 1 : SLOTS * 256];
    __shared__ __attribute__((aligned(16))) float4 sh_bigbb[BIGREC_BLOCK];
    __shared__ int32_t sh_bigrec[BIGREC_BLOCK];
    __shared__ float sh_box[4][4];
    __shared__ int32_t sh_nbig;
    __shared__ int32_t sh_wave[4];
    __shared__ int32_t sh_base;
    const int64_t n_blocks = (n_query + 255) / 256;
    const int64_t lb = xcd_block(n_blocks, remap);
    if (threadIdx.x == 0 && blk_surv) blk_surv[lb] = 0;
    if (lb >= n_blocks) {
        if (threadIdx.x == 0 && blk_rows) blk_rows[lb] = 0;
        return;
    }
    const int64_t t = lb * 256 + threadIdx.x;
    const float4 *__restrict__ rbb = reinterpret_cast<const float4 *>(rec_bb);
    int l_split = g.n_levels, big0 = (int)n_tree;
    for (int l = g.n_levels - 1; l >= 1; l--) {
        const int first = cell_start[g.base[l]];
        if ((int)n_tree - first > BIGREC_MAX) break;
        l_split = l;
        big0 = first;
    }
    double4 bb = make_double4(0, 0, 0, 0);
    float qx0 = INFINITY, qx1 = -INFINITY, qy0 = INFINITY, qy1 = -INFINITY;
    if (t < n_query) {
        bb = query_face_box<MC>(q_bbox, q_fxy, q_len, t);
        qx0 = f32_below(bb.x - g.x0), qx1 = f32_above(bb.y - g.x0);
        qy0 = f32_below(bb.z - g.y0), qy1 = f32_above(bb.w - g.y0);
    }
    int l_coop = l_split;
    for (int l = l_split - 1; l >= 1; l--) {
        const int first = cell_start[g.base[l]];
        if (((int64_t)big0 - first) * 64 > n_tree) break;
        l_coop = l;
    }
    if (threadIdx.x == 0) sh_nbig = 0;
    if (big0 < (int)n_tree || l_coop < l_split) {
        float bx0 = wave_reduce<OpMin>(qx0), bx1 = wave_reduce<OpMax>(qx1), by0 = wave_reduce<OpMin>(qy0), by1 = wave_reduce<OpMax>(qy1);
        if ((threadIdx.x & 63) == 0) {
            const int w = threadIdx.x >> 6;
            sh_box[w][0] = bx0; sh_box[w][1] = bx1; sh_box[w][2] = by0; sh_box[w][3] = by1;
        }
        __syncthreads();
#pragma unroll
        for (int w = 0; w < 4; w++) {
            bx0 = fminf(bx0, sh_box[w][0]); bx1 = fmaxf(bx1, sh_box[w][1]);
            by0 = fminf(by0, sh_box[w][2]); by1 = fmaxf(by1, sh_box[w][3]);
        }
        for (int r = big0 + threadIdx.x; r < (int)n_tree; r += 256) {
            const float4 rb = rbb[r];
            if (rec_hit(rb, bx0, bx1, by0, by1)) {
                const int k = atomicAdd(&sh_nbig, 1);
                if (k < BIGREC_BLOCK) {
                    sh_bigrec[k] = r;
                    sh_bigbb[k] = rb;
                }
            }
// ... 708 lines not shown
           int32_t *__restrict__ indices, double *__restrict__ data, int32_t *__restrict__ long_rows,
           int32_t *__restrict__ n_long, int32_t *__restrict__ apply_long_rows,
           int32_t *__restrict__ n_apply_long, bool remap) {
    __shared__ int32_t sh_src[ROW_LDS];
    __shared__ uint16_t sh_row[ROW_LDS];
    __shared__ int32_t sh_c0[256];
    __shared__ int32_t sh_lds[257];
    __shared__ int32_t sh_ptr[256];
    __shared__ int32_t sh_wave[4];
    const int64_t n_blocks = (n_query + 255) / 256;
    const int64_t lb = xcd_block(n_blocks, remap);
    if (lb >= n_blocks) return;
    const int64_t t0 = lb * 256;
    const int64_t t = t0 + threadIdx.x;
    const int2 seg = block_seg[lb];
    const int seg0 = seg.x, seg1 = seg.x + seg.y;
    int c0 = 0, len = 0;
    bool is_short = true;
    if (t < n_query) {
        c0 = cand_off[t];
        len = cand_count[t];
        is_short = len <= ROW_SHORT && !is_big[t];
        sh_ptr[threadIdx.x] = indptr[t];
        if (!is_short) long_rows[atomicAdd(n_long, 1)] = (int32_t)t;
        if (indptr[t + 1] - indptr[t] > XR_APPLY_LONG_ROW) apply_long_rows[atomicAdd(n_apply_long, 1)] = (int32_t)t;
    }
    const int slen = is_short ? len : 0;
    sh_c0[threadIdx.x] = is_short ? c0 : -1;
    const int lane = threadIdx.x & 63, wave = threadIdx.x >> 6;
    const int incl = wave_incl_scan(slen);
    if (lane == 63) sh_wave[wave] = incl;
    __syncthreads();
    int woff = 0, total = 0;
#pragma unroll
    for (int w = 0; w < 4; w++) {
        if (w < wave) woff += sh_wave[w];
        total += sh_wave[w];
    }
    sh_lds[threadIdx.x] = woff + incl - slen;
    if (threadIdx.x == 0) sh_lds[256] = total;
    __syncthreads();
    if (total <= ROW_LDS) {
        for (int j = seg0 + threadIdx.x; j < seg1; j += 256) {
            const int row = cand_tgt[j] - (int)t0;
            const int rc0 = sh_c0[row];
            if (rc0 < 0) continue;
            const int k = sh_lds[row] + (j - rc0);
            sh_src[k] = cand_area[j] > 0 ? cand_sid[j] : 0x7fffffff;
            sh_row[k] = (uint16_t)row;
        }
        __syncthreads();
        for (int k = threadIdx.x; k < total; k += 256) {
            const int s = sh_src[k];
            if (s == 0x7fffffff) continue;
            const int row = sh_row[k];
            const int a0 = sh_lds[row], a1 = row == 255 ? total : sh_lds[row + 1];
            int rank = 0;
            for (int i = a0; i < a1; i++) rank += sh_src[i] < s ? 1 : 0;
            const double a = cand_area[sh_c0[row] + (k - a0)];
            const int pos = sh_ptr[row] + rank;
            indices[pos] = s;
            data[pos] = relative ? a / src_area[s] : a;
        }
    } else if (t < n_query && is_short) {
        const int base = indptr[t];
        for (int i = c0; i < c0 + len; i++) {
            const double a = cand_area[i];
            if (!(a > 0)) continue;
            const int s = cand_sid[i];
            int rank = 0;
            for (int j = c0; j < c0 + len; j++) rank += (cand_area[j] > 0 && cand_sid[j] < s) ? 1 : 0;
            indices[base + rank] = s;
            data[base + rank] = relative ? a / src_area[s] : a;
        }
    }
}

static constexpr int ROW_BLOCK = 512;

static constexpr int BM_WORDS = 32768;
static constexpr int BM_BITS = BM_WORDS * 32;
static constexpr int BM_SEG = BM_WORDS / 256;
static constexpr int BM_STAGE = 4096;
static constexpr size_t ROW_FILL_LIGHT_LDS = sizeof(int32_t) * (8 + BM_STAGE);
static constexpr size_t ROW_FILL_LONG_LDS =
    ROW_FILL_LIGHT_LDS + sizeof(uint32_t) * (256 + BM_WORDS) + sizeof(uint16_t) * (BM_WORDS / 8);

__global__ void __launch_bounds__(256)
k_row_fill_long(const int32_t *__restrict__ cand_off, const int32_t *__restrict__ cand_count,
                const int32_t *__restrict__ cand_sid,
                const double *__restrict__ cand_area, const int32_t *__restrict__ indptr,
                const double *__restrict__ src_area, bool relative, int64_t n_tree, int32_t *__restrict__ indices,
                double *__restrict__ data, const int32_t *__restrict__ long_rows,
                const int32_t *__restrict__ n_long, int64_t row_base ,
                const int32_t *__restrict__ skip_if ,
                const int32_t *__restrict__ scan_nnz = nullptr ,
                int32_t *__restrict__ scan_indptr = nullptr ,
                int32_t *__restrict__ scan_total = nullptr ,
                int row_class = 0 ) {
    __builtin_amdgcn_s_setprio(3);
    extern __shared__ __attribute__((aligned(16))) char smem[];
    int32_t *red = reinterpret_cast<int32_t *>(smem);
    int32_t *stage = red + 8;
    uint32_t *tbase = reinterpret_cast<uint32_t *>(stage + BM_STAGE);
    uint32_t *bm = tbase + 256;
    uint16_t *gcnt = reinterpret_cast<uint16_t *>(bm + BM_WORDS);
    const int tid = threadIdx.x, lane = tid & 63, wave = tid >> 6;
    if (skip_if && *skip_if > 0) return;
    const int nl = *n_long;
    auto length_sum = [&](int k0, int k1) -> long long {
        long long v = 0;
        for (int k = k0 + tid; k < k1; k += 256) v += scan_nnz[long_rows[k]];
        v = wave_reduce<OpSum>(v);
        __syncthreads();
        if (lane == 0) red[wave] = (int32_t)(v > 0x7fffffffll ? 0x7fffffff : v);
        __syncthreads();
        return (long long)red[0] + red[1] + red[2] + red[3];
    };
    long long scan_base = 0;
    if (scan_nnz) {
        scan_base = length_sum(0, blockIdx.x < nl ? (int)blockIdx.x : nl);
        if (blockIdx.x == 0 && nl == 0 && tid == 0) {
            scan_indptr[0] = 0;
            *scan_total = 0;
        }
    }
    for (int li = blockIdx.x; li < nl; li += gridDim.x) {
        const int t = long_rows[li];
        const int c0 = cand_off[t], n = cand_count[t];
        int base;
        if (scan_nnz) {
            const long long capped = scan_base > 0x7fffffffll ? 0x7fffffffll : scan_base;
            base = (int)capped;
            if (tid == 0) {
                scan_indptr[li] = base;
                if (li == nl - 1) {
                    const long long all = capped + scan_nnz[t];
                    scan_indptr[nl] = (int32_t)(all > 0x7fffffffll ? 0x7fffffff : all);
                    *scan_total = scan_indptr[nl];
                }
            }
            const int next = li + (int)gridDim.x;
            scan_base += length_sum(li, next < nl ? next : nl);
        } else {
            base = row_base >= 0 ? indptr[row_base + li] : indptr[t];
        }
        __syncthreads();
        if (row_class != 0 && (row_class == 1) != (n <= ROW_BLOCK)) continue;
        for (int i0 = tid; i0 < n && i0 < BM_STAGE; i0 += 4 * 256) {
            double a[4];
            int sd[4];
#pragma unroll
            for (int u = 0; u < 4; u++) {
                const int i = i0 + u * 256;
                const bool in = i < n && i < BM_STAGE;
                a[u] = in ? cand_area[c0 + i] : 0.0;
                sd[u] = in ? cand_sid[c0 + i] : -1;
            }
#pragma unroll
            for (int u = 0; u < 4; u++) {
                const int i = i0 + u * 256;
                if (i < n && i < BM_STAGE) stage[i] = a[u] > 0 ? sd[u] : -1;
            }
        }
        if (n <= ROW_BLOCK) {
            __syncthreads();
            const int n4 = (n + 3) & ~3;
            if (tid < n4 - n) stage[n + tid] = -1;
            __syncthreads();
            const int4 *quad = reinterpret_cast<const int4 *>(stage);
            for (int i = tid; i < n; i += 256) {
                const int sd = stage[i];
                if (sd < 0) continue;
                int rank = 0;
                for (int j = 0; j < n4 / 4; j++) {
                    const int4 q = quad[j];
                    rank += ((unsigned)q.x < (unsigned)sd) + ((unsigned)q.y < (unsigned)sd) + ((unsigned)q.z < (unsigned)sd) +
                            ((unsigned)q.w < (unsigned)sd);
                }
                const double a = cand_area[c0 + i];
                indices[base + rank] = sd;
                data[base + rank] = relative ? a / src_area[sd] : a;
            }
            continue;
        }
        auto survivor = [&](int i) -> int {
            if (i < BM_STAGE) return stage[i];
            return cand_area[c0 + i] > 0 ? cand_sid[c0 + i] : -1;
        };
        int running = 0;
        for (int64_t cb64 = 0; cb64 < n_tree; cb64 += BM_BITS) {
            const int cb = (int)cb64;
            __syncthreads();
            {
                uint4 *bm4 = reinterpret_cast<uint4 *>(bm);
                for (int w = tid; w < BM_WORDS / 4; w += 256) bm4[w] = make_uint4(0u, 0u, 0u, 0u);
            }
            __syncthreads();
            for (int i = tid; i < n; i += 256) {
                const int s = survivor(i) - cb;
                if (s >= 0 && s < BM_BITS) atomicOr(&bm[s >> 5], 1u << (s & 31));
            }
            __syncthreads();
            for (int g = tid; g < BM_WORDS / 8; g += 256) {
                const uint4 x = reinterpret_cast<const uint4 *>(bm)[2 * g], y = reinterpret_cast<const uint4 *>(bm)[2 * g + 1];
                gcnt[g] = (uint16_t)(__popc(x.x) + __popc(x.y) + __popc(x.z) + __popc(x.w) + __popc(y.x) + __popc(y.y) +
                                     __popc(y.z) + __popc(y.w));
            }
            __syncthreads();
            uint32_t acc = 0;
#pragma unroll
            for (int k = 0; k < BM_SEG / 8; k++) {
                const uint32_t c = gcnt[tid * (BM_SEG / 8) + k];
                gcnt[tid * (BM_SEG / 8) + k] = (uint16_t)acc;
                acc += c;
            }
            const uint32_t incl = wave_incl_scan(acc);
            if (lane == 63) red[wave] = (int32_t)incl;
            __syncthreads();
            uint32_t woff = 0, chunk_total = 0;
            for (int w = 0; w < 4; w++) {
                if (w < wave) woff += (uint32_t)red[w];
                chunk_total += (uint32_t)red[w];
            }
            tbase[tid] = woff + incl - acc;
            __syncthreads();
// ... 46 lines not shown
              dim3(div_up(C, BLOCK)), dim3(BLOCK), shmem, query->qo_fxy(), query->qo_len(), query->qo_off(), query->m,
              query->qo_perm(), tree->rec_fxy.get(), tree->rec_len.get(), tree->record_off(), tree->m, cand_tgt, cand_src, C, cand_area,
              redo_only, tree->rec_face.get(), cand_sid, overflow_count, nnz_row, overlap_dust_threshold(tree, query));
}

static void launch_clip_for(const xr_mesh *tree, const xr_mesh *query, const int32_t *cand_tgt, const int32_t *cand_src,
                            int64_t C, double *cand_area, int32_t *cand_sid, int32_t *overflow_count,
                            int32_t *nnz_row) {
    const int vmax = query->m + tree->m;
    if (vmax > 16) return launch_clip<64, 64>(tree, query, cand_tgt, cand_src, C, cand_area, false, cand_sid, overflow_count, nnz_row);
    if (vmax > 8) return launch_clip<16, 128>(tree, query, cand_tgt, cand_src, C, cand_area, false, cand_sid, overflow_count, nnz_row);
    constexpr int BLOCK = 256;
    const bool remap = REMAP_CLIP;
    const dim3 grid(xcd_grid(div_up(C, BLOCK), remap));
    const double dust = overlap_dust_threshold(tree, query);
    if (vmax <= 6) {
        constexpr int MAXV = 6;
        const size_t shmem = (size_t)(MAXV + 1) * BLOCK * sizeof(double2);
        XR_LAUNCH("clip_tri", (k_clip_tri<BLOCK, 3>), grid, dim3(BLOCK), shmem, query->qo_fxy(), (const uint8_t *)nullptr,
                  tree->rec_fxy.get(), cand_tgt, cand_src, C, cand_area, tree->rec_face.get(), cand_sid, overflow_count, nnz_row, remap,
                  dust);
    } else if (query->m == 4 && tree->m == 3 && option(OPT_CLIP_QUAD) != 0) {
        const size_t shmem = (size_t)(QUAD_MAXV + 2) * BLOCK * sizeof(double2);
        XR_LAUNCH("clip_quad_tri", (k_clip_tri<BLOCK, 4>), grid, dim3(BLOCK), shmem,
                  query->qo_fxy(), query->qo_len(), tree->rec_fxy.get(), cand_tgt, cand_src, C, cand_area, tree->rec_face.get(),
                  cand_sid, overflow_count, nnz_row, remap, dust);
    } else {
        constexpr int MAXV = 8;
        const size_t shmem = (size_t)(MAXV + 1) * BLOCK * sizeof(double2);
        XR_LAUNCH("clip_small", (k_clip_small<MAXV, BLOCK>), grid, dim3(BLOCK),
                  shmem, query->qo_fxy(), query->qo_len(), query->qo_off(), query->m, query->qo_perm(), tree->rec_fxy.get(),
                  tree->rec_len.get(), tree->record_off(), tree->m, cand_tgt, cand_src, C, cand_area, tree->rec_face.get(), cand_sid,
                  overflow_count, nnz_row, remap, dust);
    }
}

struct SearchLists {
    DevBuf<int32_t> cand_count, cand_off, big_list, pending, nnz_row;
    DevBuf<uint8_t> is_big;
    DevBuf<int2> block_seg;
    explicit SearchLists(int64_t T)
        : cand_count((size_t)T), cand_off((size_t)T + 1), big_list((size_t)T), pending((size_t)T), nnz_row((size_t)T),
          is_big((size_t)T), block_seg((size_t)div_up(T, 256)) {}
};
struct PairQueue {
    int32_t *tgt, *src, *cursor;
    int64_t capacity;
};

static void launch_search(const xr_mesh *tree, const xr_mesh *query, const SearchLists &l, const PairQueue &q, int32_t *n_big,
                          const MortonParams &tile, int32_t *tile_key, int32_t *blk_rows = nullptr, int32_t *blk_surv = nullptr) {
    const int64_t T = query->n_face;
    const dim3 grid(xcd_grid(div_up(T, 256), REMAP_SEARCH));
    auto launch = [&](auto packed) {
        with_nodes_per_face(query->m, [&](auto mc) {
            XR_LAUNCH("search", (k_search<decltype(packed)::value, mc()>), grid, dim3(256), 0, query->qo_bbox(), query->qo_fxy(),
                      query->qo_len(), T, tree->grid, tree->n_face, tree->cell_start.get(), tree->rec_bb.get(), l.cand_count.get(),
                      l.cand_off.get(), q.tgt, q.src, q.cursor, l.block_seg.get(), l.is_big.get(), l.big_list.get(), n_big, tile,
                      tile_key, l.nnz_row.get(), REMAP_SEARCH, blk_rows, blk_surv, blk_rows ? (int)q.capacity : 0);
        });
    };
    if (tree->n_face <= ((int64_t)1 << 24)) launch(std::true_type());
    else launch(std::false_type());
}

static void launch_search_big(const xr_mesh *tree, const xr_mesh *query, const SearchLists &l, const PairQueue &q,
                              const int32_t *n_big, int32_t *n_pending, int32_t *slot_face = nullptr) {
    XR_LAUNCH("search_big", k_search_big<true>, dim3(engine().num_cu * 8), dim3(256), sizeof(int32_t) * (size_t)BIG_STAGE,
              query->qo_bbox(), query->qo_fxy(), query->qo_len(), query->qo_off(), query->m, tree->grid, tree->cell_start.get(),
              tree->rec_bb.get(), tree->rec_face.get(), l.big_list.get(), n_big, l.cand_off.get(), l.cand_count.get(), q.tgt,
              q.src, q.cursor, q.capacity, l.pending.get(), n_pending, BIG_STAGE, slot_face);
}

struct LongRows {
    const int32_t *cand_sid;
    const double *cand_area;
    const int32_t *indptr;
    int32_t *indices;
    double *data;
    const int32_t *long_rows, *n_long;
    int64_t row_base;
    const int32_t *skip_if = nullptr, *scan_nnz = nullptr;
    int32_t *scan_indptr = nullptr, *scan_total = nullptr;
};
static void launch_row_fill_long(int row_class, const xr_mesh *tree, const SearchLists &l, const double *tree_area, bool relative,
                                 const LongRows &r) {
    allow_dynamic_lds<&k_row_fill_long>(ROW_FILL_LONG_LDS);
    const bool light = row_class == 1;
    XR_LAUNCH(row_class == 2 ? "row_fill_huge" : "row_fill_long", k_row_fill_long, dim3(engine().num_cu * (light ? 6 : 1)), dim3(256),
              light ? ROW_FILL_LIGHT_LDS : ROW_FILL_LONG_LDS, l.cand_off.get(), l.cand_count.get(), r.cand_sid, r.cand_area,
              r.indptr, tree_area, relative, tree->n_face, r.indices, r.data, r.long_rows, r.n_long, r.row_base, r.skip_if,
              r.scan_nnz, r.scan_indptr, r.scan_total, row_class);
}

struct EarlyApply {
    std::function<void(const xr_csr *)> fn;
    bool done = false;
};

static bool overlap_tri(xr_mesh *tree, xr_mesh *query, const double *tree_area, bool relative, xr_csr *csr,
                        const MortonParams &tile, EarlyApply *early) {
    const int64_t T = query->n_face;
    hipStream_t st = launch_stream();
    const int64_t n_blocks = div_up(T, FB);
    const bool remap = REMAP_SEARCH;
    const unsigned grid = xcd_grid(n_blocks, remap);
    const int64_t margin_opt = option(OPT_QUEUE_MARGIN);
    int64_t big_capacity = margin_opt > 0 ? margin_opt : ((int64_t)4 << 20);
    const int64_t region_cap = div_up(div_up(T, FB), 8) * FB * SLOTS;
    const int64_t reg_capacity = 8 * region_cap;
    int64_t per_face = 8;
    int32_t *mail = const_cast<int32_t *>(engine().mailbox);
    DevBuf<int32_t> ctl_tail(2 * (size_t)grid), ctl_own;
    int32_t *blk_surv = ctl_tail.get(), *blk_rows = blk_surv + grid;
    DevBuf<int32_t> blk_base(2 * (size_t)grid);
    const int scan_mode = grid <= 8192 ? 2 : 1;
    SearchLists l(T);
    DevBuf<int32_t> slot_face((size_t)T), big_indptr((size_t)T + 1);
    DevBuf<int32_t> cand_tgt((size_t)reg_capacity), cand_src((size_t)reg_capacity), cand_sid((size_t)reg_capacity);
    DevBuf<double> cand_area((size_t)reg_capacity);
    csr->n_long.alloc(2);
    csr->row_order.alloc((size_t)T);
    csr->has_row_order = true;
    int32_t *const tile_key = csr->has_tile_key ? csr->tile_key.get() : nullptr;
    const bool tri_pair = tree->m == 3 && query->m == 3;
    const double dust = overlap_dust_threshold(tree, query);
    auto launch_clip_queue = [&](const char *name, auto count, int blocks_per_cu, const PairQueue &q, double *area, int32_t *sid,
                                 int32_t *error, int32_t *nnz_row, const int32_t *skip_if, int32_t *blk_surv) {
        constexpr int BLOCK = 256;
        const int64_t capacity = count() == 1 ? -q.capacity : q.capacity;
        auto launch = [&](auto kind, size_t maxv, const uint8_t *q_len, const uint8_t *s_len) {
            XR_LAUNCH(name, (k_clip_tri_queue<BLOCK, count(), kind()>), dim3(engine().num_cu * blocks_per_cu), dim3(BLOCK),
                      (maxv + 1) * BLOCK * sizeof(double2), query->qo_fxy(), tree->rec_fxy.get(), tree->rec_face.get(), q.tgt, q.src,
                      q.cursor, capacity, area, sid, error, nnz_row, skip_if, blk_surv, dust, q_len, s_len, query->m, tree->m);
        };
        if (tri_pair) launch(std::integral_constant<int, 0>(), TRI_MAXV, nullptr, nullptr);
        else launch(std::integral_constant<int, 1>(), 8, query->qo_len(), tree->rec_len.get());
    };
    for (int attempt = 0;; attempt++) {
        XR_REQUIRE(attempt < 8, XR_ERR_LIMIT, "xr_overlap: the weight matrix does not fit the device buffers");
        const int64_t cap = per_face * T + big_capacity;
        XR_REQUIRE(cap < ((int64_t)1 << 31), XR_ERR_LIMIT, "nnz exceeds the int32 range");
        csr->indices.alloc((size_t)cap);
        csr->data.alloc((size_t)cap);
        csr->long_rows.alloc((size_t)(cap / XR_APPLY_LONG_ROW + 1));
        DevBuf<int32_t> big_tgt((size_t)big_capacity), big_src((size_t)big_capacity), big_sid((size_t)big_capacity),
            big_indices((size_t)big_capacity);
        DevBuf<double> big_area((size_t)big_capacity), big_data((size_t)big_capacity);
        int32_t *ctl = zero_scratch(1, CTL_WORDS);
        const bool ctl_cached = ctl != nullptr;
        if (!ctl_cached) {
            ctl_own.alloc(CTL_WORDS);
            ctl = ctl_own.get();
            XR_HIP(hipMemsetAsync(ctl, 0, CTL_WORDS * sizeof(int32_t), st));
        }
        FusedCounters *fc = reinterpret_cast<FusedCounters *>(ctl + CTL_COUNTERS);
        int32_t *const region_cursors = ctl + CTL_REGION_CURSOR, *const big_cursor = ctl + CTL_BIG_CURSOR,
                       *const n_big_dev = ctl + CTL_N_BIG, *const n_pending_dev = ctl + CTL_N_PENDING;
        const PairQueue reg_queue{cand_tgt.get(), cand_src.get(), region_cursors, region_cap},
            big_queue{big_tgt.get(), big_src.get(), big_cursor, big_capacity};
        launch_search(tree, query, l, reg_queue, n_big_dev, tile, nullptr, blk_rows, blk_surv);
        {
            SideScope side;
            launch_search_big(tree, query, l, big_queue, n_big_dev, n_pending_dev, slot_face.get());
            launch_clip_queue("clip_big", std::integral_constant<int, 2>(), 1, big_queue, big_area.get(), big_sid.get(),
                              &fc->error, l.nnz_row.get(), n_pending_dev, nullptr);
            const LongRows big_rows{big_sid.get(), big_area.get(), big_indptr.get(), big_indices.get(), big_data.get(), slot_face.get(),
                                    n_big_dev, 0, n_pending_dev, l.nnz_row.get(), big_indptr.get(), &fc->p_big};
            SideForkScope fork;
            launch_row_fill_long(2, tree, l, tree_area, relative, big_rows);
            fork.end_launches();
            launch_row_fill_long(1, tree, l, tree_area, relative, big_rows);
        }
        launch_clip_queue(tri_pair ? "clip_tri" : "clip_small", std::integral_constant<int, 1>(), tri_pair ? 5 : 4, reg_queue,
                          cand_area.get(), cand_sid.get(), &fc->error, nullptr, nullptr, blk_surv);
        if (scan_mode == 1)
            XR_LAUNCH("assemble_scan", k_assemble_scan, dim3(1), dim3(1024), 0, blk_rows, blk_surv, (int64_t)n_blocks, (int)grid,
                      remap, blk_base.get(), blk_base.get() + grid, fc, csr->indptr.get());
        XR_LAUNCH("assemble", k_assemble, dim3(grid), dim3(FB), 0, query->qo_bbox(), query->qo_fxy(), query->qo_len(), query->m,
                  query->qo_perm(), T, cand_tgt.get(), l.cand_off.get(), l.cand_count.get(), l.block_seg.get(), l.is_big.get(), cand_area.get(), cand_sid.get(),
                  tree_area, relative, tile, tile_key, fc,
                  csr->indptr.get(), csr->indices.get(), csr->data.get(), csr->row_order.get(),
                  csr->long_rows.get(), cap, remap, scan_mode == 1 ? blk_base.get() : (const int32_t *)nullptr,
                  scan_mode == 1 ? blk_base.get() + grid : (const int32_t *)nullptr,
                  scan_mode == 2 ? blk_rows : (const int32_t *)nullptr, scan_mode == 2 ? blk_surv : (const int32_t *)nullptr);
        side_join();
        XR_LAUNCH("place_big", k_place_big, dim3(64), dim3(256), 0, n_big_dev, slot_face.get(), big_indptr.get(),
                  big_indices.get(), big_data.get(), T, query->qo_perm(), query->qo_bbox(), query->qo_fxy(), query->qo_len(),
                  query->m, tile, tile_key, fc, csr->indptr.get(), csr->indices.get(),
                  csr->data.get(), csr->row_order.get(), csr->long_rows.get(), cap, n_pending_dev);
        host_stamp(5);
        const int32_t seq = mailbox_next_seq();
        XR_LAUNCH("publish", k_publish_all, dim3(1), dim3(64), 0, ctl, fc, csr->n_long.get(), mail, seq, cap, big_capacity);
        if (ctl_cached) zero_scratch_done(1);
        if (early) {
            csr->nnz = 0;
            csr->has_long = true;
            csr->max_row_len = -1;
            csr->apply_gated = true;
            early->fn(csr);
            csr->apply_gated = false;
        }
        host_stamp(6);
        mailbox_wait_seq(seq);
        host_stamp(7);
        const int32_t C_reg = mail[MAIL_REG_PAIRS], C_big = mail[MAIL_BIG_PAIRS], n_big = mail[MAIL_N_BIG], n_pending = mail[MAIL_N_PENDING];
        const int32_t err = mail[MAIL_ERROR], rows_regular = mail[MAIL_ROWS_REGULAR], n_apply_long = mail[MAIL_N_APPLY_LONG],
                      p_regular = mail[MAIL_P_REGULAR], p_big = mail[MAIL_P_BIG];
        XR_REQUIRE(C_reg >= 0 && C_big >= 0, XR_ERR_LIMIT, "candidate pair count exceeds the int32 range");
        if (debug_fused()) {
            const int32_t *len = mail + MAIL_REGION_LEN;
            fprintf(stderr, "[tri] T=%lld C=%d big: %d faces %d pairs (%d pending) p_regular=%d p_big=%d err=%d rows=%d long=%d regions %d %d %d %d %d %d %d %d of %lld\n",
                    (long long)T, C_reg, n_big, C_big, n_pending, p_regular, p_big, err, rows_regular, n_apply_long, len[0], len[1], len[2],
                    len[3], len[4], len[5], len[6], len[7], (long long)region_cap);
        }
        if (err & 1) {
            csr->has_row_order = false;
            return false;
        }
        if (n_pending > 0 || C_big > big_capacity) {
            big_capacity = (int64_t)C_big + 1024;
            continue;
        }
        if ((err & 4) || (int64_t)p_regular + p_big > cap) {
            per_face *= 2;
            continue;
        }
        XR_REQUIRE(rows_regular == T - n_big, XR_ERR_INVALID, "xr_overlap: internal row count mismatch");
        tree->last_candidates = (int64_t)C_reg + C_big;
        csr->nnz = (int64_t)p_regular + p_big;
        csr->has_long = n_apply_long > 0;
        csr->max_row_len = n_apply_long > 0 ? mail[MAIL_MAX_ROW] : XR_APPLY_LONG_ROW;
        if (early) early->done = true;
        return true;
    }
}

static MortonParams tile_key_params(const xr_mesh *query, xr_csr *csr) {
    MortonParams tile{};
    csr->has_tile_key = false;
    if (!query->query_identity) return tile;
    const int64_t T = query->n_face;
    const double *hs = query->h_stats;
    double span = std::max(hs[1] - hs[0], hs[3] - hs[2]);
    if (!(span > 0)) span = 1.0;
    double h = 12.0 * hs[4] / (double)T;
    if (!(h > 0)) h = span;
    int bits = 0;
    while (bits < 12 && ldexp(h, bits) < span) bits++;
    tile = MortonParams{hs[0], hs[2], (double)(1 << bits) / (span * (1.0 + 1e-9)), 1 << bits};
    tile.n_run = TILE_RUN;
    csr->tile_key.alloc((size_t)T);
    csr->tile_key_range = (int64_t)1 << (2 * bits);
    csr->has_tile_key = bits > 0;
    return tile;
}

static void overlap_general(xr_mesh *tree, xr_mesh *query, const double *tree_area, bool relative, xr_csr *csr,
                            const MortonParams &tile) {
    const int64_t T = query->n_face;
    hipStream_t st = launch_stream();
    DevBuf<int32_t> counters(GEN_WORDS);
    auto word = [&](GenWord w) { return counters.get() + w; };
    XR_HIP(hipMemsetAsync(counters.get(), 0, sizeof(int32_t) * GEN_WORDS, st));
    SearchLists l(T);
    const int64_t margin_opt = option(OPT_QUEUE_MARGIN);
    int64_t capacity = T * SLOTS + (margin_opt > 0 ? margin_opt : ((int64_t)4 << 20));
    XR_REQUIRE(capacity < ((int64_t)1 << 31), XR_ERR_LIMIT, "candidate pair queue exceeds the int32 range");
    DevBuf<int32_t> cand_tgt((size_t)capacity), cand_src((size_t)capacity);
    const PairQueue queue{cand_tgt.get(), cand_src.get(), word(GEN_QUEUE_CURSOR), capacity};
    launch_search(tree, query, l, queue, word(GEN_N_BIG), tile, csr->has_tile_key ? csr->tile_key.get() : nullptr);
    launch_search_big(tree, query, l, queue, word(GEN_N_BIG), word(GEN_N_PENDING));
    int32_t *mail = const_cast<int32_t *>(engine().mailbox);
    XR_LAUNCH("publish", k_publish, dim3(1), dim3(64), 0, word(GEN_QUEUE_CURSOR), mail + GMAIL_PAIRS, word(GEN_N_PENDING),
              mail + GMAIL_N_PENDING);
    mailbox_wait();
    const int32_t C32 = mail[GMAIL_PAIRS], n_pending = mail[GMAIL_N_PENDING];
    XR_REQUIRE(C32 >= 0, XR_ERR_LIMIT, "candidate pair count exceeds the int32 range");
    const int64_t C = C32;
    tree->last_candidates = C;
    if (n_pending > 0) {
        DevBuf<int32_t> bigger_tgt((size_t)C), bigger_src((size_t)C);
        XR_HIP(hipMemcpyAsync(bigger_tgt.get(), cand_tgt.get(), sizeof(int32_t) * (size_t)capacity, hipMemcpyDeviceToDevice, st));
        XR_HIP(hipMemcpyAsync(bigger_src.get(), cand_src.get(), sizeof(int32_t) * (size_t)capacity, hipMemcpyDeviceToDevice, st));
        stream_sync();
// ... 30 lines not shown
    const int64_t P = nnz;
    csr->nnz = P;
    csr->indices.alloc((size_t)P);
    csr->data.alloc((size_t)P);
    if (query->qo_perm()) {
        csr->row_order.alloc((size_t)T);
        XR_HIP(hipMemcpyAsync(csr->row_order.get(), query->qo_perm(), sizeof(int32_t) * (size_t)T,
                              hipMemcpyDeviceToDevice, st));
        csr->has_row_order = true;
    }
    if (P > 0) {
        DevBuf<int32_t> long_rows((size_t)T);
        csr->long_rows.alloc((size_t)(P / XR_APPLY_LONG_ROW + 1));
        csr->n_long.alloc(1);
        csr->has_long = true;
        XR_HIP(hipMemsetAsync(csr->n_long.get(), 0, sizeof(int32_t), st));
        const bool remap = REMAP_ROW_FILL;
        XR_LAUNCH("row_fill", k_row_fill, dim3(xcd_grid(div_up(T, 256), remap)), dim3(256), 0, l.cand_off.get(), l.cand_count.get(),
                  l.block_seg.get(), l.is_big.get(), cand_tgt.get(), cand_sid.get(), cand_area.get(), T, csr->indptr.get(), tree_area, relative,
                  csr->indices.get(), csr->data.get(), long_rows.get(), word(GEN_N_LONG_ROWS), csr->long_rows.get(),
                  csr->n_long.get(), remap);
        launch_row_fill_long(0, tree, l, tree_area, relative,
                             LongRows{cand_sid.get(), cand_area.get(), csr->indptr.get(), csr->indices.get(), csr->data.get(),
                                      long_rows.get(), word(GEN_N_LONG_ROWS), -1});
    }
}

static void overlap(xr_mesh *tree, xr_mesh *query, bool relative, xr_csr *csr, EarlyApply *early = nullptr) {
    mesh_prepare_pair(tree, query);
    host_stamp(2);
    mesh_build_index(tree);
    host_stamp(3);
    mesh_query_order(query);
    host_stamp(4);
    const double *tree_area = relative ? mesh_area(tree) : nullptr;
    const int64_t T = query->n_face, S = tree->n_face;
    XR_REQUIRE(T < ((int64_t)1 << 31) - 1, XR_ERR_LIMIT, "too many query faces for int32 row offsets");
    csr->n = T;
    csr->m = S;
    csr->nnz = 0;
    csr->indptr.alloc((size_t)T + 1);
    tree->last_candidates = 0;
    if (T == 0 || S == 0) {
        XR_HIP(hipMemsetAsync(csr->indptr.get(), 0, sizeof(int32_t) * ((size_t)T + 1), launch_stream()));
        csr->indices.alloc(0);
        csr->data.alloc(0);
        return;
    }
    const MortonParams tile = tile_key_params(query, csr);
    const bool fused = option(OPT_OVERLAP_FUSED) != 0 && tree->m <= DENSE_MAX_NODES && query->m <= DENSE_MAX_NODES &&
                       (T + 8 * FB) * SLOTS < ((int64_t)1 << 31);
    if (fused && overlap_tri(tree, query, tree_area, relative, csr, tile, early)) return;
    overlap_general(tree, query, tree_area, relative, csr, tile);
}

}

using namespace xr;

extern "C" {

int xr_overlap(xr_mesh *tree, xr_mesh *query, int relative, xr_csr **out) {
    XR_API_BEGIN
    XR_REQUIRE(tree && query && out, XR_ERR_INVALID, "xr_overlap: NULL argument");
    Building<xr_csr> csr;
    overlap(tree, query, relative != 0, csr.get());
    stream_sync();
    *out = csr.release();
    XR_API_END
}

int xr_overlap_apply_dev(xr_mesh *tree, xr_mesh *query, int relative, int method, double percentile, const void *source_dev,
                         int source_dtype, int64_t K, double *out_dev, xr_csr **out) {
    XR_API_BEGIN
    XR_REQUIRE(tree && query && out, XR_ERR_INVALID, "xr_overlap_apply_dev: NULL argument");
    XR_REQUIRE(K >= 0 && (source_dev || tree->n_face == 0 || K == 0) && (out_dev || query->n_face == 0 || K == 0), XR_ERR_INVALID,
               "xr_overlap_apply_dev: NULL data argument");
    XR_REQUIRE(source_dtype == XR_F64 || source_dtype == XR_F32, XR_ERR_INVALID, "unsupported source dtype id %d", source_dtype);
    host_stamp(0);
    Building<xr_csr> csr(OnFailure::WaitFirst);
    EarlyApply early;
    early.fn = [&](const xr_csr *c) { csr_apply_dev(c, method, percentile, source_dev, source_dtype, K, out_dev); };
    const bool can_early = K == 1 && method != XR_MODE && method != XR_PERCENTILE;
    overlap(tree, query, relative != 0, csr.get(), can_early ? &early : nullptr);
    host_stamp(8);
    if (!early.done && K > 0) csr_apply_dev(csr.get(), method, percentile, source_dev, source_dtype, K, out_dev);
    dev_call_done();
    host_stamp(9);
    *out = csr.release();
    XR_API_END
}

int xr_overlap_partial_dev(xr_mesh *tree, xr_mesh *query, int relative, int method, const void *source_dev, int source_dtype,
                           int64_t K, double *out_dev, int rows_layout, xr_csr **out) {
    XR_API_BEGIN
    XR_REQUIRE(tree && query && out, XR_ERR_INVALID, "xr_overlap_partial_dev: NULL argument");
    XR_REQUIRE(K >= 0 && (source_dev || tree->n_face == 0 || K == 0) && (out_dev || query->n_face == 0 || K == 0), XR_ERR_INVALID,
               "xr_overlap_partial_dev: NULL data argument");
    XR_REQUIRE(xr_partial_components(method) > 0, XR_ERR_INVALID, "xr_overlap_partial_dev: method %d has no partial state", method);
    XR_REQUIRE(source_dtype == XR_F32 || source_dtype == XR_F64, XR_ERR_INVALID, "xr_overlap_partial_dev: source_dtype must be XR_F32 or XR_F64");
    XR_REQUIRE(K < 65536, XR_ERR_LIMIT, "xr_overlap_partial_dev: at most 65535 variables per call");
    Building<xr_csr> csr(OnFailure::WaitFirst);
    EarlyApply early;
    early.fn = [&](const xr_csr *c) { csr_partial_dev(c, method, source_dev, source_dtype, K, out_dev, rows_layout); };
    const bool can_early = K == 1;
    overlap(tree, query, relative != 0, csr.get(), can_early ? &early : nullptr);
    if (!early.done && K > 0) csr_partial_dev(csr.get(), method, source_dev, source_dtype, K, out_dev, rows_layout);
    dev_call_done();
    *out = csr.release();
    XR_API_END
}

int xr_overlap_stats(const xr_mesh *tree, int64_t *n_candidates) {
    XR_API_BEGIN
    XR_REQUIRE(tree && n_candidates, XR_ERR_INVALID, "xr_overlap_stats: NULL argument");
    *n_candidates = tree->last_candidates;
    XR_API_END
}

}
```

xugrid_amd/csrc/xr_overlap_fused.h:

```cpp
#pragma once

namespace xr {

static constexpr int FB = 256;
static constexpr int FWAVES = FB / 64;

struct FusedCounters {
    int32_t n_apply_long;
    int32_t error;
    int32_t p_regular;
    int32_t rows_regular;
    int32_t p_big;
    int32_t pad0;
    int32_t max_row;
    int32_t pad2;
};

enum CtlWord : int {
    CTL_REG_CURSOR = 0,
    CTL_BIG_CURSOR = 1,
    CTL_N_BIG = 2,
    CTL_N_PENDING = 3,
    CTL_BIG_OVERFLOW = 4,
    CTL_COUNTERS = 8,
    CTL_LINE = 16,
    CTL_REGION_CURSOR = 32,
    CTL_WORDS = CTL_REGION_CURSOR + 8 * QCUR_STRIDE
};
#define XR_CTL_COUNTER(field) (xr::CTL_COUNTERS + (int)(offsetof(xr::FusedCounters, field) / sizeof(int32_t)))
static_assert(CTL_COUNTERS + sizeof(FusedCounters) / sizeof(int32_t) <= CTL_LINE && CTL_BIG_OVERFLOW < CTL_COUNTERS &&
                  CTL_LINE <= CTL_REGION_CURSOR && CTL_LINE + 8 <= 64,
              "the counters lie inside the line k_publish_all's one wave fetches, the region cursors behind it");
enum MailSlot : int {
    MAIL_REG_PAIRS = 0,
    MAIL_BIG_PAIRS = 1,
    MAIL_N_BIG = 2,
    MAIL_N_PENDING = 3,
    MAIL_BIG_OVERFLOW = 4,
    MAIL_ERROR = 5,
    MAIL_ROWS_REGULAR = 6,
    MAIL_N_APPLY_LONG = 7,
    MAIL_P_REGULAR = 8,
    MAIL_P_BIG = 9,
    MAIL_MAX_ROW = 10,
    MAIL_REGION_LEN = 11,
    MAIL_FUSED_SLOTS = MAIL_REGION_LEN + 8
};
static_assert(MAIL_BIG_OVERFLOW - MAIL_REG_PAIRS == CTL_BIG_OVERFLOW - CTL_REG_CURSOR && MAIL_FUSED_SLOTS <= MAIL_SEQ_SLOT,
              "the first control words map to the first mailbox slots one to one");

enum GenWord : int {
    GEN_CLIP_OVERFLOW = 0,
    GEN_N_PENDING = 1,
    GEN_N_LONG_ROWS = 1,
    GEN_N_BIG = 2,
    GEN_QUEUE_CURSOR = 3,
    GEN_WORDS = 4
};
enum GenMailSlot : int { GMAIL_PAIRS = 0, GMAIL_NNZ = 1, GMAIL_CLIP_OVERFLOW = 2, GMAIL_N_PENDING = 3 };

template <int BLOCK, int COUNT, int KIND = 0>
__global__ void __launch_bounds__(BLOCK) __attribute__((amdgpu_waves_per_eu(KIND == 0 ? 5 : 4)))
k_clip_tri_queue(const double *__restrict__ q_fxy, const double *__restrict__ rec_fxy,
                 const int32_t *__restrict__ rec_face, const int32_t *cand_tgt,
                 const int32_t *cand_src, const int32_t *__restrict__ n_cand_dev, int64_t capacity,
                 double *__restrict__ cand_area, int32_t *__restrict__ cand_sid, int32_t *__restrict__ error_bits,
                 int32_t *__restrict__ nnz_row ,
                 const int32_t *__restrict__ skip_if ,
                 int32_t *__restrict__ blk_surv = nullptr ,
                 double dust = 0.0 ,
                 const uint8_t *__restrict__ q_len = nullptr, const uint8_t *__restrict__ s_len = nullptr, int q_m = 3, int s_m = 3) {
    extern __shared__ __attribute__((aligned(16))) char smem[];
    constexpr int CS = 1;
    constexpr int SMALL_MAXV = 8;
    double2 *col = reinterpret_cast<double2 *>(smem) + (KIND == 1 ? threadIdx.x : threadIdx.x * (TRI_MAXV + 1));
    __shared__ uint2 sh_lut[KIND == 1 ? 1 : TRI_LUT];
    if (skip_if) __builtin_amdgcn_s_setprio(3);
    if (skip_if && *skip_if > 0) return;
    if (KIND == 0) {
        tri_lut_init(sh_lut);
        __syncthreads();
    }
    const bool regions = capacity < 0;
    const int64_t region_cap = regions ? -capacity : 0;
    int64_t n_cand = 0, per_xcd;
    auto region_len = [&](int x) -> int64_t {
        const int64_t n = n_cand_dev[x * QCUR_STRIDE];
        return n < region_cap ? n : region_cap;
    };
    if (regions) {
        int64_t longest = 0;
#pragma unroll
        for (int x = 0; x < 8; x++) longest = region_len(x) > longest ? region_len(x) : longest;
        per_xcd = (longest + BLOCK - 1) / BLOCK;
    } else {
        n_cand = *n_cand_dev < capacity ? *n_cand_dev : capacity;
        per_xcd = ((n_cand + BLOCK - 1) / BLOCK + 7) >> 3;
    }
    const int64_t n_slots = per_xcd * 8;
    auto slot_first = [&](int64_t j, int64_t *end) -> int64_t {
        if (regions) {
            const int x = (int)(j & 7);
            *end = (int64_t)x * region_cap + region_len(x);
            return (int64_t)x * region_cap + (j >> 3) * BLOCK;
        }
        *end = n_cand;
        return ((j & 7) * per_xcd + (j >> 3)) * BLOCK;
    };
    const double2 *tfx = reinterpret_cast<const double2 *>(q_fxy);
    const double2 *sfx = reinterpret_cast<const double2 *>(rec_fxy);
    const int tid = threadIdx.x;
    int n_tq = 0, n_s = 0;
    auto load_idx = [&](int64_t slot, int &tq, int &s) {
        tq = 0;
        s = 0;
// ... 38 lines not shown
                    const double2 a = tfx[(int64_t)n_tq * 3 + j], b2 = sfx[(int64_t)n_s * 3 + j];
                    tv[j] = P2{a.x, a.y};
                    sv[j] = P2{b2.x, b2.y};
                }
                sid = rec_face[n_s];
            }
            load_idx(slot + stride, n_tq, n_s);
            area = tri_clip_area<CS>(tv, sv, col, sh_lut, active);
            const bool suspicious = active && area > 0 && area <= dust;
            if (__any(suspicious)) {
                if (suspicious && !pair_passes_box_and_sat(tfx + (int64_t)cur_tq * 3, 3, sfx + (int64_t)cand_src[c] * 3, 3)) area = 0.0;
            }
        }
        const int tq_now = active ? cur_tq : -1;
        if (active) {
            overflow = overflow || area == TRI_AREA_OVERFLOW;
            cand_area[c] = area;
            cand_sid[c] = area > 0 ? sid : 0x7fffffff;
        }
        if (COUNT == 1) {
            const int lane = tid & 63;
            const int blk_now = active ? (cur_tq >> 8) : -1;
            const unsigned long long surv = __ballot(active && area > 0);
            const int blk_first = __builtin_amdgcn_readfirstlane(blk_now), blk_last = __shfl(blk_now, 63, 64);
            if (blk_first == blk_last) {
                if (lane == 0 && blk_first >= 0 && surv) atomicAdd(&blk_surv[blk_first], __popcll(surv));
            } else {
                wave_run_add(blk_now, active && area > 0, blk_surv);
            }
        }
        if (COUNT == 2) wave_run_add(tq_now, active && area > 0, nnz_row);
    }
    if (overflow) atomicOr(error_bits, 1);
}

__global__ void __launch_bounds__(1024)
k_assemble_scan(const int32_t *__restrict__ blk_rows, const int32_t *__restrict__ blk_surv, int64_t n_blocks, int n_chain,
                bool remap, int32_t *__restrict__ base_rows, int32_t *__restrict__ base_nnz, FusedCounters *counters,
                int32_t *__restrict__ indptr) {
    __shared__ long long sh_w[16];
    const int tid = threadIdx.x, lane = tid & 63, wave = tid >> 6;
    long long carry = 0;
    const int64_t per_xcd = (n_blocks + 7) >> 3;
    for (int b0 = 0; b0 < n_chain; b0 += 1024) {
        const int b = b0 + tid;
        long long v = 0;
        if (b < n_chain) {
            const int64_t lb = remap ? (int64_t)(b & 7) * per_xcd + (b >> 3) : b;
            if (lb < n_blocks) v = ((long long)blk_rows[lb] << 31) | (long long)blk_surv[lb];
        }
        const long long incl = wave_incl_scan(v);
        if (lane == 63) sh_w[wave] = incl;
        __syncthreads();
        long long woff = 0, tot = 0;
        for (int w = 0; w < 16; w++) {
            if (w < wave) woff += sh_w[w];
            tot += sh_w[w];
        }
        const long long excl = carry + woff + incl - v;
        if (b < n_chain) {
            base_nnz[b] = (int32_t)(excl & 0x7fffffffll);
            base_rows[b] = (int32_t)(excl >> 31);
        }
        carry += tot;
        __syncthreads();
    }
    if (tid == 0) {
        const long long entries = carry & 0x7fffffffll, rows = carry >> 31;
        counters->p_regular = (int32_t)entries;
        counters->rows_regular = (int32_t)rows;
        indptr[rows] = (int32_t)entries;
    }
}

__global__ void __launch_bounds__(FB, 2)
k_assemble(const double *__restrict__ q_bbox, const double *__restrict__ q_fxy, const uint8_t *__restrict__ q_len, int q_m,
           const int32_t *__restrict__ q_perm, int64_t n_query,
           const int32_t *__restrict__ cand_tgt, const int32_t *__restrict__ cand_off,
           const int32_t *__restrict__ cand_count, const int2 *__restrict__ block_seg,
           const uint8_t *__restrict__ is_big, const double *__restrict__ cand_area,
           const int32_t *__restrict__ cand_sid, const double *__restrict__ src_area, bool relative, MortonParams tile,
           int32_t *__restrict__ tile_key, FusedCounters *__restrict__ counters,
           int32_t *__restrict__ indptr, int32_t *__restrict__ indices, double *__restrict__ data, int32_t *__restrict__ row_order,
           int32_t *__restrict__ apply_long_rows, int64_t csr_capacity, bool remap,
           const int32_t *__restrict__ base_rows = nullptr, const int32_t *__restrict__ base_nnz = nullptr,
           const int32_t *__restrict__ blk_rows = nullptr, const int32_t *__restrict__ blk_surv = nullptr) {
    __shared__ int32_t sh_stage[SLOTS * FB];
    __shared__ int32_t sh_nnz[FB];
    __shared__ uint16_t sh_lo[FB];
    __shared__ uint16_t sh_rowoff[FB];
    __shared__ uint8_t sh_cnt[FB];
    __shared__ int32_t sh_wave[FWAVES];
    __shared__ long long sh_base;
    const int tid = threadIdx.x;
    const int64_t n_blocks = (n_query + FB - 1) / FB;
    const int64_t lb = xcd_block(n_blocks, remap);
    const bool valid_block = lb < n_blocks;
    sh_nnz[tid] = 0;
    const int64_t t0 = lb * FB;
    const int64_t t = t0 + tid;
    const bool in_range = valid_block && t < n_query;
    const int2 seg = valid_block ? block_seg[lb] : make_int2(0, 0);
    const int total = seg.y;
    bool regular = false;
    int my_cnt = 0;
    if (in_range) {
        regular = !is_big[t];
        my_cnt = regular ? cand_count[t] : 0;
        sh_lo[tid] = (uint16_t)(regular ? cand_off[t] - seg.x : 0);
    } else {
        sh_lo[tid] = 0;
    }
    sh_cnt[tid] = (uint8_t)my_cnt;
    __syncthreads();
    for (int i0 = tid; i0 < total; i0 += 4 * FB) {
        int s[4], row[4];
#pragma unroll
        for (int u = 0; u < 4; u++) {
            const int i = i0 + u * FB;
            const int64_t c = (int64_t)seg.x + (i < total ? i : total - 1);
            s[u] = cand_sid[c];
            row[u] = cand_tgt[c] - (int)t0;
        }
#pragma unroll
        for (int u = 0; u < 4; u++) {
            const int i = i0 + u * FB;
            if (i < total) {
                sh_stage[i] = s[u];
                if (s[u] != 0x7fffffff) atomicAdd(&sh_nnz[row[u]], 1);
            }
        }
    }
    __syncthreads();
    const int my_nnz = regular ? sh_nnz[tid] : 0;
    int block_nnz = 0, block_rows = 0;
    const int rowoff = block_excl_scan<FB>(my_nnz, &block_nnz, sh_wave);
    const int rowidx = block_excl_scan<FB>(regular ? 1 : 0, &block_rows, sh_wave);
    sh_rowoff[tid] = (uint16_t)rowoff;
    const int b = (int)blockIdx.x, n_chain = (int)gridDim.x;
    if (blk_surv) {
        const int64_t per_xcd = (n_blocks + 7) >> 3;
        long long acc = 0;
        for (int hb = tid; hb < b; hb += FB) {
            const int64_t plb = remap ? (int64_t)(hb & 7) * per_xcd + (hb >> 3) : hb;
            if (plb < n_blocks) acc += ((long long)blk_rows[plb] << 31) | (long long)blk_surv[plb];
        }
        acc = wave_reduce<OpSum>(acc);
        __shared__ long long sh_part[FWAVES];
        if ((tid & 63) == 0) sh_part[tid >> 6] = acc;
        __syncthreads();
        if (tid == 0) {
            long long tot = 0;
#pragma unroll
            for (int w = 0; w < FWAVES; w++) tot += sh_part[w];
            sh_base = tot;
        }
    } else {
        if (tid == 0) sh_base = ((long long)base_rows[b] << 31) | (long long)base_nnz[b];
    }
    __syncthreads();
    const long long base = sh_base & 0x7fffffffll, row_base = sh_base >> 31;
    if (!base_nnz && b == n_chain - 1 && tid == 0) {
        const long long entries = base + block_nnz, rows = row_base + block_rows;
        counters->p_regular = (int32_t)entries;
        counters->rows_regular = (int32_t)rows;
        indptr[rows] = (int32_t)entries;
    }
    if (regular) {
        const long long r = row_base + rowidx;
        indptr[r] = (int32_t)(base + rowoff);
        row_order[r] = q_perm ? q_perm[t] : (int32_t)t;
        if (tile_key) {
            const int64_t mid = (t & ~(int64_t)(tile.n_run - 1)) + tile.n_run / 2;
            tile_key[r] = morton_key(tile, query_face_box_rt(q_bbox, q_fxy, q_len, q_m, mid < n_query ? mid : n_query - 1));
        }
        if (my_nnz > XR_APPLY_LONG_ROW) {
            apply_long_rows[atomicAdd(&counters->n_apply_long, 1)] = (int32_t)r;
            atomicMax(&counters->max_row, my_nnz);
        }
    }
    bool overflow_cap = false;
    for (int i0 = tid; i0 < total; i0 += 4 * FB) {
        double area[4];
        int row[4];
#pragma unroll
        for (int u = 0; u < 4; u++) {
            const int i = i0 + u * FB;
            const int64_t c = (int64_t)seg.x + (i < total ? i : total - 1);
            area[u] = cand_area[c];
            row[u] = cand_tgt[c] - (int)t0;
        }
#pragma unroll
        for (int u = 0; u < 4; u++) {
            const int i = i0 + u * FB;
            if (i >= total) continue;
            const int s = sh_stage[i];
            if (s == 0x7fffffff) continue;
            const int a0 = sh_lo[row[u]], a1 = a0 + sh_cnt[row[u]];
            int rank = 0;
            for (int j = a0; j < a1; j++) rank += sh_stage[j] < s ? 1 : 0;
            const long long pos = base + sh_rowoff[row[u]] + rank;
            if (pos < csr_capacity) {
                indices[pos] = s;
                data[pos] = relative ? area[u] / src_area[s] : area[u];
            } else {
                overflow_cap = true;
            }
        }
    }
    if (overflow_cap) atomicOr(&counters->error, 4);
}


__global__ void __launch_bounds__(256)
k_place_big(const int32_t *__restrict__ n_big_dev, const int32_t *__restrict__ slot_face,
            const int32_t *__restrict__ big_indptr, const int32_t *__restrict__ big_indices,
            const double *__restrict__ big_data, int64_t n_query, const int32_t *__restrict__ q_perm,
            const double *__restrict__ q_bbox, const double *__restrict__ q_fxy, const uint8_t *__restrict__ q_len, int q_m,
            MortonParams tile, int32_t *__restrict__ tile_key,
            FusedCounters *counters, int32_t *__restrict__ indptr, int32_t *__restrict__ indices,
            double *__restrict__ data, int32_t *__restrict__ row_order, int32_t *__restrict__ apply_long_rows,
            int64_t csr_capacity, const int32_t *__restrict__ skip_if) {
    const int n_big = *n_big_dev;
    if (n_big == 0 || *skip_if > 0) return;
    const int64_t p_regular = counters->p_regular, t_reg = n_query - n_big;
    const int64_t p_big = big_indptr[n_big];
    if (p_regular + p_big > csr_capacity) {
        if (blockIdx.x == 0 && threadIdx.x == 0) atomicOr(&counters->error, 4);
        return;
    }
    const int64_t i0 = (int64_t)blockIdx.x * 256 + threadIdx.x, stride = (int64_t)gridDim.x * 256;
    for (int64_t k = i0; k < n_big; k += stride) {
        const int f = slot_face[k];
        const int64_t r = t_reg + k;
        const int n = big_indptr[k + 1] - big_indptr[k];
        indptr[r] = (int32_t)(p_regular + big_indptr[k]);
        row_order[r] = q_perm ? q_perm[f] : f;
        if (tile_key) {
            const int64_t mid = ((int64_t)f & ~(int64_t)(tile.n_run - 1)) + tile.n_run / 2;
            tile_key[r] = morton_key(tile, query_face_box_rt(q_bbox, q_fxy, q_len, q_m, mid < n_query ? mid : n_query - 1));
        }
        if (n > XR_APPLY_LONG_ROW) {
            apply_long_rows[atomicAdd(&counters->n_apply_long, 1)] = (int32_t)r;
            atomicMax(&counters->max_row, n);
        }
    }
    for (int64_t e = i0; e < p_big; e += stride) {
        indices[p_regular + e] = big_indices[e];
        data[p_regular + e] = big_data[e];
    }
    if (i0 == 0) indptr[n_query] = (int32_t)(p_regular + p_big);
}

__global__ void k_publish_all(int32_t *c , FusedCounters *fc,
                              int32_t *__restrict__ n_apply_long_out, int32_t *mail , int32_t seq, int64_t cap,
                              int64_t big_capacity) {
    const int t = threadIdx.x;
    int32_t w = 0;
    if (t < CTL_LINE) w = c[t];
    const bool region_lane = t >= CTL_LINE && t < CTL_LINE + 8;
    const int32_t cur = region_lane ? c[CTL_REGION_CURSOR + (t - CTL_LINE) * QCUR_STRIDE] : 0;
    const int32_t c_reg_sum = wave_reduce<OpSum>(cur);
    if (t == CTL_REG_CURSOR) w = c_reg_sum;
    int slot = -1;
    if (t <= CTL_BIG_OVERFLOW) slot = MAIL_REG_PAIRS + t;
    else if (t == XR_CTL_COUNTER(error)) slot = MAIL_ERROR;
    else if (t == XR_CTL_COUNTER(rows_regular)) slot = MAIL_ROWS_REGULAR;
    else if (t == XR_CTL_COUNTER(n_apply_long)) slot = MAIL_N_APPLY_LONG;
    else if (t == XR_CTL_COUNTER(p_regular)) slot = MAIL_P_REGULAR;
    else if (t == XR_CTL_COUNTER(p_big)) slot = MAIL_P_BIG;
    else if (t == XR_CTL_COUNTER(max_row)) slot = MAIL_MAX_ROW;
    if (slot >= 0) mail[slot] = w;
    if (region_lane) mail[MAIL_REGION_LEN + (t - CTL_LINE)] = cur;
    if (t == XR_CTL_COUNTER(n_apply_long)) *n_apply_long_out = w;
    if (t == 0) {
        const int32_t c_reg = c_reg_sum, c_big = c[CTL_BIG_CURSOR], n_pending = c[CTL_N_PENDING], err = c[XR_CTL_COUNTER(error)],
                      p_reg = c[XR_CTL_COUNTER(p_regular)], p_big = c[XR_CTL_COUNTER(p_big)];
        const bool ok = c_reg >= 0 && c_big >= 0 && !(err & (1 | 4 | 8)) && n_pending == 0 && (int64_t)c_big <= big_capacity &&
                        (int64_t)p_reg + p_big <= cap;
        n_apply_long_out[1] = ok ? 1 : 0;
    }
    __builtin_amdgcn_s_waitcnt(0);
    if (t < CTL_LINE) c[t] = 0;
    if (region_lane) c[CTL_REGION_CURSOR + (t - CTL_LINE) * QCUR_STRIDE] = 0;
    (void)fc;
    __threadfence_system();
    if (t == 0) __hip_atomic_store(&mail[MAIL_SEQ_SLOT], seq, __ATOMIC_RELEASE, __HIP_MEMORY_SCOPE_SYSTEM);
}

}
```

xugrid_amd/engine.py:

```python
import ctypes

import numpy as np

from . import _lib
from ._lib import XR_F32, XR_F64, check

IntDType = np.intp
FloatDType = np.float64

METHOD_IDS = {
    "mean": 0,
    "harmonic_mean": 1,
    "geometric_mean": 2,
    "sum": 3,
    "minimum": 4,
    "maximum": 5,
    "mode": 6,
    "percentile": 7,
    "first_order_conservative": 8,
    "conductance": 8,
    "max_overlap": 9,
    "select": 10,
}

# ... 1019 lines not shown
        self.n, self.m, self.nnz = n.value, m.value, nnz.value

    def __del__(self):
        if getattr(self, "_owner", None) is None:
            super().__del__()

    @classmethod
    def from_arrays(cls, data, indices, indptr, n, m):
        data = np.ascontiguousarray(data, dtype=np.float64)
        indices = np.ascontiguousarray(indices, dtype=np.int64)
        indptr = np.ascontiguousarray(indptr, dtype=np.int64)
        if indptr.size != n + 1 or indices.size != data.size:
            raise ValueError("inconsistent CSR arrays")
        handle = ctypes.c_void_p()
        check(
            _lib.load().xr_csr_upload(
                _ptr(data), _ptr(indices), _ptr(indptr), int(n), int(m), data.size, ctypes.byref(handle)
            )
        )
        return cls(handle)

    @classmethod
    def from_triplet(cls, row, col, data, n, m):
        row = np.ascontiguousarray(row, dtype=np.int64)
        col = np.ascontiguousarray(col, dtype=np.int64)
        data = np.ascontiguousarray(data, dtype=np.float64)
        handle = ctypes.c_void_p()
        check(
            _lib.load().xr_csr_from_triplet(
                _ptr(row), _ptr(col), _ptr(data), data.size, int(n), int(m), ctypes.byref(handle)
            )
        )
        return cls(handle)

    @classmethod
    def from_outer(cls, axis_y, n_source_y, axis_x, n_source_x):
        (ipy, sy, wy), (ipx, sx, wx) = _axis_arrays(axis_y, axis_x)
        handle = ctypes.c_void_p()
        check(
            _lib.load().xr_csr_from_outer(
                _ptr(ipy), _ptr(sy), _ptr(wy), ipy.size - 1, int(n_source_y),
                _ptr(ipx), _ptr(sx), _ptr(wx), ipx.size - 1, int(n_source_x), ctypes.byref(handle),
            )
        )
        return cls(handle)

    def set_row_keys(self, keys, key_range):
        keys = np.ascontiguousarray(keys, dtype=np.int64)
        if keys.shape != (self.n,):
            raise ValueError("one key per row expected")
        check(_lib.load().xr_csr_set_row_keys(self._h, _ptr(keys), int(key_range)))

    def set_col_keys(self, keys, key_range):
        keys = np.ascontiguousarray(keys, dtype=np.int64)
        if keys.shape != (self.m,):
            raise ValueError("one key per column expected")
        check(_lib.load().xr_csr_set_col_keys(self._h, _ptr(keys), int(key_range)))

    def col_order(self):
        out = np.empty(self.m, dtype=np.int64)
        check(_lib.load().xr_csr_col_order(self._h, _ptr(out)))
        return out

    def expect_permuted(self, permuted=True):
        check(_lib.load().xr_csr_expect_permuted(self._h, 1 if permuted else 0))

    def engine_order(self, source_xy, target_xy, K=256, row_tile=4, col_tile=8):
        rk, rr = morton_row_keys(target_xy, faces_per_tile=row_tile)
        self.set_row_keys(rk, rr)
        ck, cr = morton_row_keys(source_xy, faces_per_tile=col_tile)
        self.set_col_keys(ck, cr)
        self.expect_permuted(True)
        self.output_stored_order(True)
        return self.col_order(), self.row_order()

    def output_stored_order(self, stored=True):
        check(_lib.load().xr_csr_output_stored_order(self._h, 1 if stored else 0))

    def row_order(self, K=None):
        out = np.empty(self.n, dtype=np.int64)
        check(_lib.load().xr_csr_row_order(self._h, 0, _ptr(out)))
        return out

    def download(self):
        data = np.empty(self.nnz, dtype=np.float64)
        indices = np.empty(self.nnz, dtype=np.int64)
        indptr = np.empty(self.n + 1, dtype=np.int64)
        check(_lib.load().xr_csr_download(self._h, _ptr(data), _ptr(indices), _ptr(indptr)))
        return data, indices.astype(IntDType, copy=False), indptr.astype(IntDType, copy=False)

    def apply(self, source, method_id=0, percentile=0.0, out=None):
        return _apply_host(_lib.load().xr_apply_csr, self, source, method_id, percentile, out)

    def apply_dev(self, source_ptr, dtype, K, out_ptr, method_id=0, percentile=0.0):
        _apply_dev(_lib.load().xr_apply_csr_dev, self, source_ptr, dtype, K, out_ptr, method_id, percentile)

    def partial_dev(self, source_ptr, dtype, K, out_ptr, method_id, rows_layout):
        check(
            _lib.load().xr_apply_partial_dev(
                self._h, int(method_id), ctypes.c_void_p(source_ptr), int(dtype), int(K), ctypes.c_void_p(out_ptr),
                1 if rows_layout else 0,
            )
        )


class DeviceOuter(Handle):

    _destroy = "xr_outer_destroy"

    def __init__(self, axis_y, n_source_y, axis_x, n_source_x):
        (ipy, sy, wy), (ipx, sx, wx) = _axis_arrays(axis_y, axis_x)
        handle = ctypes.c_void_p()
        check(
            _lib.load().xr_outer_create(
                _ptr(ipy), _ptr(sy), _ptr(wy), ipy.size - 1, int(n_source_y),
                _ptr(ipx), _ptr(sx), _ptr(wx), ipx.size - 1, int(n_source_x), ctypes.byref(handle),
            )
        )
        self._h = handle
        n, m, nnz = ctypes.c_int64(), ctypes.c_int64(), ctypes.c_int64()
        check(_lib.load().xr_outer_info(handle, ctypes.byref(n), ctypes.byref(m), ctypes.byref(nnz)))
        self.n, self.m, self.nnz = n.value, m.value, nnz.value

    def csr(self) -> "DeviceCSR":
        handle = ctypes.c_void_p()
        check(_lib.load().xr_outer_csr(self._h, ctypes.byref(handle)))
        return DeviceCSR(handle, owner=self)

    def download(self):
        return self.csr().download()

    def apply(self, source, method_id=0, percentile=0.0, out=None):
        return _apply_host(_lib.load().xr_apply_outer, self, source, method_id, percentile, out)

    def apply_dev(self, source_ptr, dtype, K, out_ptr, method_id=0, percentile=0.0):
        _apply_dev(_lib.load().xr_apply_outer_dev, self, source_ptr, dtype, K, out_ptr, method_id, percentile)


SHARD_MODES = {"hash": 0, "morton": 1, "balanced": 2}


def shard_plan_dev(src_xy_ptr, src_faces_ptr, n_src_face, src_m, tgt_xy_ptr, tgt_faces_ptr, n_tgt_face, tgt_m, world, rank, mode,
                   local_faces_ptr, local_targets_ptr, owner_ptr=0):
    n_f, n_t = ctypes.c_int64(0), ctypes.c_int64(0)
    check(_lib.load().xr_shard_plan_dev(
        ctypes.c_void_p(int(src_xy_ptr)), ctypes.c_void_p(int(src_faces_ptr)), int(n_src_face), int(src_m),
        ctypes.c_void_p(int(tgt_xy_ptr)), ctypes.c_void_p(int(tgt_faces_ptr)), int(n_tgt_face), int(tgt_m), int(world), int(rank),
        SHARD_MODES[mode], ctypes.c_void_p(int(local_faces_ptr)), ctypes.byref(n_f), ctypes.c_void_p(int(local_targets_ptr)),
        ctypes.byref(n_t), ctypes.c_void_p(int(owner_ptr)) if owner_ptr else None))
    return n_f.value, n_t.value


def partial_components(method_id):
    return int(_lib.load().xr_partial_components(int(method_id)))


def partial_combine_is_max(method_id):
    return bool(_lib.load().xr_partial_combine_is_max(int(method_id)))


def partial_fill_identity_dev(method_id, planes_ptr, K, n):
    check(_lib.load().xr_partial_fill_identity_dev(int(method_id), ctypes.c_void_p(planes_ptr), int(K), int(n)))


def finalize_partial_dev(method_id, planes_ptr, K, n, out_ptr):
    check(_lib.load().xr_finalize_partial_dev(int(method_id), ctypes.c_void_p(planes_ptr), int(K), int(n),
# ... 61 lines not shown
```

Before: 2.165 billion target cells/s.

## Fuse big-row placement into the apply tail kernel, reading rows in place

Adds a k_apply_tail1 kernel that places the overflowed big rows into the CSR and applies them in the same launch. Big rows are read directly from their side buffers through a TailRows accessor, so apply no longer waits for the copy. Long-row detection moves out of the fused build kernel, and the publish kernel now exports n_big and p_regular to the tail. The aim is to cut a kernel launch and a serial dependency between placement and apply in each step, at the cost of more branching in row access and more code paths.

```diff
diff --git a/include/xugrid_amd.h b/include/xugrid_amd.h
--- a/include/xugrid_amd.h
+++ b/include/xugrid_amd.h
@@ -152,6 +152,7 @@
 int xr_csr_expect_permuted(xr_csr *csr, int permuted);
 int xr_csr_output_stored_order(xr_csr *csr, int stored);
 int xr_csr_row_order(const xr_csr *csr, int64_t K_hint, int64_t *order_out);
+int xr_csr_long_rows(const xr_csr *csr, int64_t capacity, int64_t *rows_out, int64_t *n_out);
 int xr_csr_destroy(xr_csr *csr);
 
 int xr_apply_csr(const xr_csr *csr, int method, double percentile, const void *source,
diff --git a/profiles/tail_timeline.py b/profiles/tail_timeline.py
--- /dev/null
+++ b/profiles/tail_timeline.py
@@ -0,0 +1,37 @@
+#!/usr/bin/env python
+import csv
+import sys
+from collections import defaultdict
+
+
+def short(name):
+    return name.split("(")[0].split("<")[0].replace("void ", "").replace("xr::", "").strip()
+
+
+def med(xs):
+    xs = sorted(xs)
+    return xs[len(xs) // 2]
+
+
+def main():
+    path, steps = sys.argv[1], int(sys.argv[2]) if len(sys.argv) > 2 else 10
+    ker = sorted((int(r["Start_Timestamp"]), int(r["End_Timestamp"]), short(r["Kernel_Name"])) for r in csv.DictReader(open(path)))
+    ends = [i for i, k in enumerate(ker) if k[2].startswith("k_apply_rows1") or k[2].startswith("k_apply_tail1")][-steps:]
+    spans = defaultdict(list)
+    lengths = []
+    for a, b in zip(ends[:-1], ends[1:]):
+        step = ker[a + 1:b + 1]
+        t0 = step[0][0]
+        seen = defaultdict(int)
+        for s, e, name in step:
+            seen[name] += 1
+            spans[(name, seen[name])].append((s - t0, e - t0))
+        lengths.append(step[-1][1] - ker[a][1])
+    for (name, k), xs in sorted(spans.items(), key=lambda kv: med([x[0] for x in kv[1]])):
+        s, e = med([x[0] for x in xs]) / 1e3, med([x[1] for x in xs]) / 1e3
+        print("  %-26s %7.1f -> %7.1f  (dur %5.1f)%s" % (name + ("" if k == 1 else " #%d" % k), s, e, e - s, "" if len(xs) == len(lengths) else "  [%d of %d steps]" % (len(xs), len(lengths))))
+    print("  step (end of apply to end of apply), median: %.1f us" % (med(lengths) / 1e3))
+
+
+if __name__ == "__main__":
+    main()
diff --git a/xugrid_amd/_lib.py b/xugrid_amd/_lib.py
--- a/xugrid_amd/_lib.py
+++ b/xugrid_amd/_lib.py
@@ -108,6 +108,7 @@
     "xr_csr_expect_permuted": (c_int, [vp, c_int]),
     "xr_csr_output_stored_order": (c_int, [vp, c_int]),
     "xr_csr_row_order": (c_int, [vp, c_i64, vp]),
+    "xr_csr_long_rows": (c_int, [vp, c_i64, vp, vp]),
     "xr_csr_destroy": (c_int, [vp]),
     "xr_apply_csr": (c_int, [vp, c_int, c_f64, vp, c_int, c_i64, vp]),
     "xr_apply_csr_dev": (c_int, [vp, c_int, c_f64, vp, c_int, c_i64, vp]),
diff --git a/xugrid_amd/csrc/xr_apply.hip b/xugrid_amd/csrc/xr_apply.hip
--- a/xugrid_amd/csrc/xr_apply.hip
+++ b/xugrid_amd/csrc/xr_apply.hip
@@ -3,6 +3,7 @@
 #include <vector>
 
 #include "xr_apply.h"
+#include "xr_overlap_tail.h"
 #include "xr_reduce.h"
 #include "xr_prims.h"
 
@@ -10,13 +11,46 @@
 
 static constexpr int KT = 16;
 
-template <int METHOD, typename SRC>
-__device__ __forceinline__ void apply_row_block(const int32_t *__restrict__ indptr, const int32_t *__restrict__ indices,
-                                                const double *__restrict__ data, const int32_t *__restrict__ row_order,
-                                                int t, int64_t T, int64_t S, const SRC *__restrict__ source, int64_t K,
-                                                double *__restrict__ out, double (*lds)[3]) {
-    const int s = indptr[t], e = indptr[t + 1];
-    const int64_t t_out = row_order ? (int64_t)row_order[t] : t;
+struct CsrRows {
+    const int32_t *__restrict__ indptr, *__restrict__ indices;
+    const double *__restrict__ data;
+    const int32_t *__restrict__ row_order;
+    __device__ __forceinline__ void segment(int t, int &s, int &e) const {
+        s = indptr[t];
+        e = indptr[t + 1];
+    }
+    __device__ __forceinline__ const int32_t *columns(int) const { return indices; }
+    __device__ __forceinline__ const double *weights(int) const { return data; }
+    __device__ __forceinline__ int64_t out_row(int t) const { return row_order ? (int64_t)row_order[t] : t; }
+};
+struct TailRows {
+    CsrRows reg;
+    int t_big;
+    const int32_t *__restrict__ big_indptr, *__restrict__ big_indices;
+    const double *__restrict__ big_data;
+    const int32_t *__restrict__ slot_face, *__restrict__ q_perm;
+    __device__ __forceinline__ void segment(int t, int &s, int &e) const {
+        const int32_t *ip = t >= t_big ? big_indptr + (t - t_big) : reg.indptr + t;
+        s = ip[0];
+        e = ip[1];
+    }
+    __device__ __forceinline__ const int32_t *columns(int t) const { return t >= t_big ? big_indices : reg.indices; }
+    __device__ __forceinline__ const double *weights(int t) const { return t >= t_big ? big_data : reg.data; }
+    __device__ __forceinline__ int64_t big_out_row(int k) const {
+        const int f = slot_face[k];
+        return q_perm ? (int64_t)q_perm[f] : f;
+    }
+    __device__ __forceinline__ int64_t out_row(int t) const { return t >= t_big ? big_out_row(t - t_big) : reg.out_row(t); }
+};
+
+template <int METHOD, typename SRC, typename ROWS>
+__device__ __forceinline__ void apply_row_block(const ROWS &rows, int t, int64_t T, int64_t S, const SRC *__restrict__ source,
+                                                int64_t K, double *__restrict__ out, double (*lds)[3]) {
+    int s, e;
+    rows.segment(t, s, e);
+    const int32_t *__restrict__ indices = rows.columns(t);
+    const double *__restrict__ data = rows.weights(t);
+    const int64_t t_out = rows.out_row(t);
     double normsum = 0.0;
     if (METHOD == XR_GEOMETRIC_MEAN) {
         Red<XR_SUM> ws;
@@ -58,7 +92,7 @@
     __shared__ double lds[AP_BLOCK / 64][3];
     const int nl = *n_long;
     for (int li = blockIdx.x; li < nl; li += gridDim.x)
-        apply_row_block<METHOD, SRC>(indptr, indices, data, row_order, long_rows[li], T, S, source, K, out, lds);
+        apply_row_block<METHOD, SRC>(CsrRows{indptr, indices, data, row_order}, long_rows[li], T, S, source, K, out, lds);
 }
 
 static constexpr int APPLY_GROUP16 = 512;
@@ -126,38 +160,36 @@
     }
 }
 
-template <int METHOD, typename SRC, int KTILE>
-__device__ __forceinline__ void apply_wave_rows(const int32_t *__restrict__ indptr, const int32_t *__restrict__ indices,
-                                                const double *__restrict__ data, const int32_t *__restrict__ row_order,
-                                                const int32_t *__restrict__ long_rows, int nl, int wave, int n_waves,
-                                                int64_t T, int64_t S, const SRC *__restrict__ source, int64_t K,
+template <int METHOD, typename SRC, int KTILE, typename ROWS>
+__device__ __forceinline__ void apply_wave_rows(const ROWS &rows, const int32_t *__restrict__ long_rows, int nl, int wave,
+                                                int n_waves, int64_t T, int64_t S, const SRC *__restrict__ source, int64_t K,
                                                 double *__restrict__ out, int32_t *__restrict__ huge_rows) {
     const int lane = threadIdx.x & 63;
     for (int li0 = wave * 4; li0 < nl; li0 += n_waves * 4) {
         const int li = li0 + (lane >> 4);
-        int s = 0, e = 0;
+        int t = 0, s = 0, e = 0;
         int64_t t_out = 0;
         if (li < nl) {
-            const int t = long_rows[li];
-            s = indptr[t];
-            e = indptr[t + 1];
-            t_out = row_order ? (int64_t)row_order[t] : t;
+            t = long_rows[li];
+            rows.segment(t, s, e);
+            t_out = rows.out_row(t);
             if (e - s > APPLY_GROUP16) e = s;
         }
         if (__any(e > s)) {
-            if (e > s) apply_row_group<METHOD, SRC, KTILE, 16>(indices, data, s, e, t_out, T, S, source, K, out);
+            if (e > s)
+                apply_row_group<METHOD, SRC, KTILE, 16>(rows.columns(t), rows.weights(t), s, e, t_out, T, S, source, K, out);
         }
     }
     for (int li = wave; li < nl; li += n_waves) {
         const int t = long_rows[li];
-        const int s = indptr[t], e = indptr[t + 1];
+        int s, e;
+        rows.segment(t, s, e);
         if (e - s <= APPLY_GROUP16) continue;
         if (e - s > APPLY_WAVE) {
             if (huge_rows && lane == 0 && blockIdx.y == 0) huge_rows[1 + atomicAdd(huge_rows, 1)] = t;
             continue;
         }
-        const int64_t t_out = row_order ? (int64_t)row_order[t] : t;
-        apply_row_group<METHOD, SRC, KTILE, 64>(indices, data, s, e, t_out, T, S, source, K, out);
+        apply_row_group<METHOD, SRC, KTILE, 64>(rows.columns(t), rows.weights(t), s, e, rows.out_row(t), T, S, source, K, out);
     }
 }
 
@@ -168,44 +200,46 @@
              const int32_t *__restrict__ n_long, int64_t T, int64_t S, const SRC *__restrict__ source, int64_t K,
              double *__restrict__ out, int32_t *__restrict__ huge_rows) {
     const int wave = (blockIdx.x * AP_BLOCK + threadIdx.x) >> 6, n_waves = gridDim.x * (AP_BLOCK / 64);
-    apply_wave_rows<METHOD, SRC, KTILE>(indptr, indices, data, row_order, long_rows, *n_long, wave, n_waves, T, S, source, K,
-                                        out, huge_rows);
+    apply_wave_rows<METHOD, SRC, KTILE>(CsrRows{indptr, indices, data, row_order}, long_rows, *n_long, wave, n_waves, T, S,
+                                        source, K, out, huge_rows);
+}
+
+template <int METHOD, typename SRC, typename ROWS>
+__device__ __forceinline__ void rows1_long_role(const ROWS &rows, const int32_t *__restrict__ long_rows, int nl, int block,
+                                                int n_blocks, bool any_huge, int64_t T, int64_t S,
+                                                const SRC *__restrict__ source, double *__restrict__ out, double2 *sh_win) {
+    double(*sh_merge)[3] = reinterpret_cast<double(*)[3]>(sh_win);
+    const int wib = threadIdx.x >> 6;
+    apply_wave_rows<METHOD, SRC, 1>(rows, long_rows, nl, block * (AP_BLOCK / 64) + wib, n_blocks * (AP_BLOCK / 64), T, S, source, 1,
+                                    out, nullptr);
+    if (any_huge) {
+        int *sh_list = reinterpret_cast<int *>(sh_win + W1_CAP), *sh_cnt = reinterpret_cast<int *>(sh_win + 2 * W1_CAP);
+        for (int base = 0; base < nl; base += n_blocks * AP_BLOCK) {
+            if (threadIdx.x == 0) *sh_cnt = 0;
+            __syncthreads();
+            const int li = base + block + n_blocks * (int)threadIdx.x;
+            if (li < nl) {
+                const int t = long_rows[li];
+                int s, e;
+                rows.segment(t, s, e);
+                if (e - s > APPLY_WAVE) sh_list[atomicAdd(sh_cnt, 1)] = t;
+            }
+            __syncthreads();
+            const int n_hit = *sh_cnt;
+            for (int i = 0; i < n_hit; i++)
+                apply_row_block<METHOD, SRC>(rows, sh_list[i], T, S, source, 1, out, sh_merge);
+            __syncthreads();
+        }
+    }
 }
 
 template <int METHOD, typename SRC>
-__global__ void __launch_bounds__(AP_BLOCK)
-k_apply_rows1(const int32_t *__restrict__ indptr, const int32_t *__restrict__ indices, const double *__restrict__ data,
-              const int32_t *__restrict__ row_order, const int32_t *__restrict__ long_rows,
-              const int32_t *__restrict__ n_long, int n_long_blocks, bool any_huge, int64_t T, int64_t S,
-              const SRC *__restrict__ source, double *__restrict__ out, const int32_t *__restrict__ gate) {
-    __shared__ double2 sh_win[AP_BLOCK / 64][W1_CAP];
-    if (gate && *gate == 0) return;
-    double(*sh_merge)[3] = reinterpret_cast<double(*)[3]>(&sh_win[0][0]);
+__device__ __forceinline__ void rows1_regular_role(const int32_t *__restrict__ indptr, const int32_t *__restrict__ indices,
+                                                   const double *__restrict__ data, const int32_t *__restrict__ row_order,
+                                                   int block, int n_blocks, bool skip_long, int64_t T,
+                                                   const SRC *__restrict__ source, double *__restrict__ out, double2 *sh_win) {
     const int lane = threadIdx.x & 63, wib = threadIdx.x >> 6;
-    if ((int)blockIdx.x < n_long_blocks) {
-        const int nl = *n_long;
-        apply_wave_rows<METHOD, SRC, 1>(indptr, indices, data, row_order, long_rows, nl, (int)blockIdx.x * (AP_BLOCK / 64) + wib,
-                                        n_long_blocks * (AP_BLOCK / 64), T, S, source, 1, out, nullptr);
-        if (any_huge) {
-            int *sh_list = reinterpret_cast<int *>(&sh_win[1][0]), *sh_cnt = reinterpret_cast<int *>(&sh_win[2][0]);
-            for (int base = 0; base < nl; base += n_long_blocks * AP_BLOCK) {
-                if (threadIdx.x == 0) *sh_cnt = 0;
-                __syncthreads();
-                const int li = base + (int)blockIdx.x + n_long_blocks * (int)threadIdx.x;
-                if (li < nl) {
-                    const int t = long_rows[li];
-                    if (indptr[t + 1] - indptr[t] > APPLY_WAVE) sh_list[atomicAdd(sh_cnt, 1)] = t;
-                }
-                __syncthreads();
-                const int n_hit = *sh_cnt;
-                for (int i = 0; i < n_hit; i++)
-                    apply_row_block<METHOD, SRC>(indptr, indices, data, row_order, sh_list[i], T, S, source, 1, out, sh_merge);
-                __syncthreads();
-            }
-        }
-        return;
-    }
-    const int64_t row0 = ((int64_t)(gridDim.x - 1 - blockIdx.x) * (AP_BLOCK / 64) + wib) * 64;
+    const int64_t row0 = ((int64_t)(n_blocks - 1 - block) * (AP_BLOCK / 64) + wib) * 64;
     if (row0 >= T) return;
     const int64_t t = row0 + lane;
     int s = 0, e = 0;
@@ -213,12 +247,12 @@
         s = indptr[t];
         e = indptr[t + 1];
     }
-    const bool skip = n_long_blocks > 0 && (e - s > APPLY_LONG);
+    const bool skip = skip_long && (e - s > APPLY_LONG);
     const int seg0 = __shfl(s, 0, 64);
     const int seg1 = wave_reduce<OpMax>(e);
     if (skip) e = s;
     const bool jumpy = __any(skip);
-    double2 *win = sh_win[wib];
+    double2 *win = sh_win + (size_t)wib * W1_CAP;
     auto next_chunk = [&](int c0) -> int {
         if (!jumpy) return c0;
         int mine = (e > s && e > c0) ? (s > c0 ? s : c0) : INT_MAX;
@@ -280,6 +314,82 @@
         }
         out[t_out] = r;
     }
+}
+
+template <int METHOD, typename SRC>
+__global__ void __launch_bounds__(AP_BLOCK)
+k_apply_rows1(const int32_t *__restrict__ indptr, const int32_t *__restrict__ indices, const double *__restrict__ data,
+              const int32_t *__restrict__ row_order, const int32_t *__restrict__ long_rows,
+              const int32_t *__restrict__ n_long, int n_long_blocks, bool any_huge, int64_t T, int64_t S,
+              const SRC *__restrict__ source, double *__restrict__ out, const int32_t *__restrict__ gate) {
+    __shared__ double2 sh_win[AP_BLOCK / 64][W1_CAP];
+    if (gate && *gate == 0) return;
+    if ((int)blockIdx.x < n_long_blocks)
+        return rows1_long_role<METHOD, SRC>(CsrRows{indptr, indices, data, row_order}, long_rows, *n_long, (int)blockIdx.x,
+                                            n_long_blocks, any_huge, T, S, source, out, &sh_win[0][0]);
+    rows1_regular_role<METHOD, SRC>(indptr, indices, data, row_order, (int)blockIdx.x - n_long_blocks,
+                                    (int)gridDim.x - n_long_blocks, n_long_blocks > 0, T, source, out, &sh_win[0][0]);
+}
+
+template <int METHOD, typename SRC>
+__global__ void __launch_bounds__(AP_BLOCK)
+k_apply_tail1(ApplyTail tail, const int32_t *__restrict__ long_rows, int n_long_blocks, int64_t T, int64_t S,
+              const SRC *__restrict__ source, double *__restrict__ out) {
+    __shared__ double2 sh_win[AP_BLOCK / 64][W1_CAP];
+    const PlaceBig &p = tail.place;
+    if (tail.words[TAIL_GATE] == 0) return;
+    const int n_big = tail.words[TAIL_N_BIG];
+    const int t_big = (int)(T - n_big);
+    const int b = (int)blockIdx.x;
+    const TailRows rows{CsrRows{p.indptr, p.indices, p.data, p.row_order}, t_big, p.big_indptr, p.big_indices, p.big_data,
+                        p.slot_face, p.q_perm};
+    if (b < TAIL_PLACE_BLOCKS) {
+        if (n_big == 0) return;
+        place_big_copy<true>(p, n_big, tail.words[TAIL_P_REGULAR], p.big_indptr[n_big], b, TAIL_PLACE_BLOCKS);
+        for (int k = b * AP_BLOCK + (int)threadIdx.x; k < n_big; k += TAIL_PLACE_BLOCKS * AP_BLOCK) {
+            const int s = p.big_indptr[k], e = p.big_indptr[k + 1];
+            if (e - s > APPLY_LONG) continue;
+            double normsum = 0.0;
+            if (METHOD == XR_GEOMETRIC_MEAN) {
+                for (int j0 = s; j0 < e; j0 += 8) {
+                    double w[8];
+#pragma unroll
+                    for (int u = 0; u < 8; u++) w[u] = j0 + u < e ? p.big_data[j0 + u] : 0.0;
+#pragma unroll
+                    for (int u = 0; u < 8; u++)
+                        if (j0 + u < e) normsum += w[u];
+                }
+            }
+            Red<METHOD> red;
+            for (int j0 = s; j0 < e; j0 += 8) {
+                int col[8];
+                double w[8], v[8];
+#pragma unroll
+                for (int u = 0; u < 8; u++) {
+                    col[u] = j0 + u < e ? p.big_indices[j0 + u] : -1;
+                    w[u] = j0 + u < e ? p.big_data[j0 + u] : 0.0;
+                }
+#pragma unroll
+                for (int u = 0; u < 8; u++) v[u] = col[u] >= 0 ? ld_src(source, (int64_t)col[u]) : 0.0;
+#pragma unroll
+                for (int u = 0; u < 8; u++)
+                    if (col[u] >= 0) red.add(v[u], w[u], normsum);
+            }
+            double r = NAN;
+            if (e > s) {
+                r = red.fin();
+                if (METHOD == XR_GEOMETRIC_MEAN && normsum == 0) r = NAN;
+            }
+            out[rows.big_out_row(k)] = r;
+        }
+        return;
+    }
+    if (b < TAIL_PLACE_BLOCKS + n_long_blocks)
+        return rows1_long_role<METHOD, SRC>(rows, long_rows, tail.words[TAIL_N_LONG], b - TAIL_PLACE_BLOCKS, n_long_blocks, true, T,
+                                            S, source, out, &sh_win[0][0]);
+    const int n_lead = TAIL_PLACE_BLOCKS + n_long_blocks;
+    rows1_regular_role<METHOD, SRC>(p.indptr, p.indices, p.data, p.row_order, b - n_lead, (int)gridDim.x - n_lead, true, t_big,
+                                    source, out, &sh_win[0][0]);
 }
 
 template <int METHOD, typename SRC, int KTILE>
@@ -1146,9 +1256,17 @@
         const int n_long_blocks = csr->has_long ? engine().num_cu / 2 : 0;
         const bool any_huge = csr->has_long && !(csr->max_row_len >= 0 && csr->max_row_len <= APPLY_WAVE);
         dim3 grid((unsigned)(div_up(csr->n, AP_BLOCK) + n_long_blocks), 1);
-        XR_LAUNCH("apply_rows1", (k_apply_rows1<METHOD, SRC>), grid, dim3(AP_BLOCK), 0, csr->indptr.get(), csr->indices.get(),
-                  csr->data.get(), row_order_of(csr), csr->long_rows.get(), csr->n_long.get(), n_long_blocks, any_huge,
-                  csr->n, csr->m, src, out, csr->apply_gated ? csr->n_long.get() + 1 : (const int32_t *)nullptr);
+        if (csr->apply_tail) {
+            XR_REQUIRE(csr->apply_gated && n_long_blocks > 0 && row_order_of(csr) == csr->row_order.get() && !csr->has_col_perm,
+                       XR_ERR_INVALID, "xr_apply: the tail of a weight build needs its fresh matrix");
+            grid.x += TAIL_PLACE_BLOCKS;
+            XR_LAUNCH("apply_rows1", (k_apply_tail1<METHOD, SRC>), grid, dim3(AP_BLOCK), 0, *csr->apply_tail, csr->long_rows.get(),
+                      n_long_blocks, csr->n, csr->m, src, out);
+        } else {
+            XR_LAUNCH("apply_rows1", (k_apply_rows1<METHOD, SRC>), grid, dim3(AP_BLOCK), 0, csr->indptr.get(), csr->indices.get(),
+                      csr->data.get(), row_order_of(csr), csr->long_rows.get(), csr->n_long.get(), n_long_blocks, any_huge,
+                      csr->n, csr->m, src, out, csr->apply_gated ? csr->n_long.get() + 1 : (const int32_t *)nullptr);
+        }
     } else {
         if (use_plan) {
             constexpr bool FAST_OK = METHOD == XR_MEAN || METHOD == XR_FIRST_ORDER_CONSERVATIVE;
diff --git a/xugrid_amd/csrc/xr_csr.hip b/xugrid_amd/csrc/xr_csr.hip
--- a/xugrid_amd/csrc/xr_csr.hip
+++ b/xugrid_amd/csrc/xr_csr.hip
@@ -395,6 +395,21 @@
     XR_API_END
 }
 
+int xr_csr_long_rows(const xr_csr *csr, int64_t capacity, int64_t *rows_out, int64_t *n_out) {
+    XR_API_BEGIN
+    XR_REQUIRE(csr && n_out && (rows_out || capacity == 0) && capacity >= 0, XR_ERR_INVALID, "xr_csr_long_rows: invalid argument");
+    stream_sync();
+    const int64_t n = csr->n_long.get() ? read_scalar(csr->n_long.get()) : 0;
+    *n_out = n;
+    const int64_t take = n < capacity ? n : capacity;
+    if (take > 0) {
+        DevBuf<int64_t> wide((size_t)take);
+        download_wide(csr->long_rows.get(), take, rows_out, wide);
+        stream_sync();
+    }
+    XR_API_END
+}
+
 int xr_csr_destroy(xr_csr *csr) {
     XR_API_BEGIN
     if (csr) {
diff --git a/xugrid_amd/csrc/xr_engine.hip b/xugrid_amd/csrc/xr_engine.hip
--- a/xugrid_amd/csrc/xr_engine.hip
+++ b/xugrid_amd/csrc/xr_engine.hip
@@ -56,7 +56,7 @@
     {"apply_contract", 0}, {"plan_merge", -1}, {"plan_dbg", 0}, {"apply_chunk_bytes", 0}, {"outer_apply", 0}, {"edge_big", 0},
     {"edge_stage", 0}, {"edge_queue", 0}, {"edge_sort", 1}, {"nn_query_sort", -1}, {"burn_strips", 0},
     {"facet_tile", 0}, {"scan_fused_tiles", 0}, {"merge_table_slack", 0},
-    {"front_fused", 1},
+    {"front_fused", 1}, {"tail_fused", 1},
 };
 static_assert(sizeof(k_option_defs) / sizeof(k_option_defs[0]) == OPT_COUNT, "one table row per enum Option");
 std::atomic<int64_t> g_options[OPT_COUNT];
diff --git a/xugrid_amd/csrc/xr_internal.h b/xugrid_amd/csrc/xr_internal.h
--- a/xugrid_amd/csrc/xr_internal.h
+++ b/xugrid_amd/csrc/xr_internal.h
@@ -254,6 +254,7 @@
     OPT_SCAN_FUSED_TILES,
     OPT_MERGE_TABLE_SLACK,
     OPT_FRONT_FUSED,
+    OPT_TAIL_FUSED,
     OPT_COUNT
 };
 int64_t option(Option o);
diff --git a/xugrid_amd/csrc/xr_objects.h b/xugrid_amd/csrc/xr_objects.h
--- a/xugrid_amd/csrc/xr_objects.h
+++ b/xugrid_amd/csrc/xr_objects.h
@@ -87,6 +87,10 @@
 static constexpr int XR_APPLY_LONG_ROW = 32;
 static constexpr int XR_APPLY_WAVE_ROW = 2048;
 
+namespace xr {
+struct ApplyTail;
+}
+
 struct xr_csr {
     int64_t n = 0, m = 0, nnz = 0;
     xr::DevBuf<int32_t> indptr;
@@ -97,6 +101,7 @@
     xr::DevBuf<int32_t> long_rows;
     xr::DevBuf<int32_t> n_long;
     bool apply_gated = false;
+    const xr::ApplyTail *apply_tail = nullptr;
     int64_t max_row_len = -1;
     bool has_long = false;
     xr::DevBuf<int32_t> tile_key;
diff --git a/xugrid_amd/csrc/xr_overlap.hip b/xugrid_amd/csrc/xr_overlap.hip
--- a/xugrid_amd/csrc/xr_overlap.hip
+++ b/xugrid_amd/csrc/xr_overlap.hip
@@ -1,5 +1,6 @@
 #include "xr_objects.h"
 #include "xr_clip_tri.h"
+#include "xr_overlap_tail.h"
 #include "xr_prims.h"
 
 namespace xr {
@@ -11,7 +12,7 @@
 }
 
 static constexpr int SLOTS = 16;
-static constexpr int QCUR_STRIDE = 32;
+static_assert(SLOTS <= XR_APPLY_LONG_ROW, "a regular row is never one of the apply's long rows: only k_row_fill_long lists");
 static constexpr int TILE_RUN = 16;
 
 __device__ __forceinline__ int64_t xcd_block(int64_t n_blocks, bool remap) {
@@ -886,10 +887,11 @@
 static constexpr int BM_BITS = BM_WORDS * 32;
 static constexpr int BM_SEG = BM_WORDS / 256;
 static constexpr int BM_STAGE = 4096;
-static constexpr size_t ROW_FILL_LIGHT_LDS = sizeof(int32_t) * (8 + BM_STAGE);
+static constexpr size_t ROW_FILL_LIGHT_LDS = sizeof(int32_t) * (16 + BM_STAGE);
 static constexpr size_t ROW_FILL_LONG_LDS =
     ROW_FILL_LIGHT_LDS + sizeof(uint32_t) * (256 + BM_WORDS) + sizeof(uint16_t) * (BM_WORDS / 8);
 
+template <bool LIST>
 __global__ void __launch_bounds__(256)
 k_row_fill_long(const int32_t *__restrict__ cand_off, const int32_t *__restrict__ cand_count,
                 const int32_t *__restrict__ cand_sid,
@@ -901,29 +903,56 @@
                 const int32_t *__restrict__ scan_nnz = nullptr ,
                 int32_t *__restrict__ scan_indptr = nullptr ,
                 int32_t *__restrict__ scan_total = nullptr ,
-                int row_class = 0 ) {
+                int row_class = 0 ,
+                int32_t *__restrict__ apply_long_rows = nullptr ,
+                FusedCounters *listed = nullptr, int64_t n_stored = 0) {
     __builtin_amdgcn_s_setprio(3);
     extern __shared__ __attribute__((aligned(16))) char smem[];
     int32_t *red = reinterpret_cast<int32_t *>(smem);
-    int32_t *stage = red + 8;
+    int32_t *stage = red + 16;
     uint32_t *tbase = reinterpret_cast<uint32_t *>(stage + BM_STAGE);
     uint32_t *bm = tbase + 256;
     uint16_t *gcnt = reinterpret_cast<uint16_t *>(bm + BM_WORDS);
     const int tid = threadIdx.x, lane = tid & 63, wave = tid >> 6;
     if (skip_if && *skip_if > 0) return;
     const int nl = *n_long;
-    auto length_sum = [&](int k0, int k1) -> long long {
+    auto length_sum = [&](int k0, int k1, int *n_longer, int *longest) -> long long {
         long long v = 0;
-        for (int k = k0 + tid; k < k1; k += 256) v += scan_nnz[long_rows[k]];
+        int c = 0, m = 0;
+        for (int k = k0 + tid; k < k1; k += 256) {
+            const int len = scan_nnz[long_rows[k]];
+            v += len;
+            if (LIST) {
+                c += len > XR_APPLY_LONG_ROW ? 1 : 0;
+                m = len > m ? len : m;
+            }
+        }
         v = wave_reduce<OpSum>(v);
+        if (LIST) {
+            c = wave_reduce<OpSum>(c);
+            m = wave_reduce<OpMax>(m);
+        }
         __syncthreads();
-        if (lane == 0) red[wave] = (int32_t)(v > 0x7fffffffll ? 0x7fffffff : v);
+        if (lane == 0) {
+            red[wave] = (int32_t)(v > 0x7fffffffll ? 0x7fffffff : v);
+            if (LIST) {
+                red[4 + wave] = c;
+                red[8 + wave] = m;
+            }
+        }
         __syncthreads();
+        if (LIST) {
+            *n_longer = red[4] + red[5] + red[6] + red[7];
+            const int m01 = red[8] > red[9] ? red[8] : red[9], m23 = red[10] > red[11] ? red[10] : red[11];
+            *longest = m01 > m23 ? m01 : m23;
+        }
         return (long long)red[0] + red[1] + red[2] + red[3];
     };
     long long scan_base = 0;
+    int list_base = 0;
+    int list_max = 0;
     if (scan_nnz) {
-        scan_base = length_sum(0, blockIdx.x < nl ? (int)blockIdx.x : nl);
+        scan_base = length_sum(0, blockIdx.x < nl ? (int)blockIdx.x : nl, &list_base, &list_max);
         if (blockIdx.x == 0 && nl == 0 && tid == 0) {
             scan_indptr[0] = 0;
             *scan_total = 0;
@@ -936,16 +965,31 @@
         if (scan_nnz) {
             const long long capped = scan_base > 0x7fffffffll ? 0x7fffffffll : scan_base;
             base = (int)capped;
+            int len_t = 0;
             if (tid == 0) {
                 scan_indptr[li] = base;
+                if (LIST || li == nl - 1) len_t = scan_nnz[t];
+            }
+            const int next = li + (int)gridDim.x;
+            int longer = 0, longest = 0;
+            scan_base += length_sum(li, next < nl ? next : nl, &longer, &longest);
+            if (tid == 0) {
+                if (LIST) {
+                    if (len_t > XR_APPLY_LONG_ROW) apply_long_rows[list_base] = (int32_t)(n_stored - nl + li);
+                    if (li == nl - 1) {
+                        const int n_listed = list_base + (len_t > XR_APPLY_LONG_ROW ? 1 : 0);
+                        listed->n_apply_long = n_listed;
+                        if (n_listed > 0) listed->max_row = len_t > list_max ? len_t : list_max;
+                    }
+                }
                 if (li == nl - 1) {
-                    const long long all = capped + scan_nnz[t];
+                    const long long all = capped + len_t;
                     scan_indptr[nl] = (int32_t)(all > 0x7fffffffll ? 0x7fffffff : all);
                     *scan_total = scan_indptr[nl];
                 }
             }
-            const int next = li + (int)gridDim.x;
-            scan_base += length_sum(li, next < nl ? next : nl);
+            list_base += longer;
+            list_max = longest > list_max ? longest : list_max;
         } else {
             base = row_base >= 0 ? indptr[row_base + li] : indptr[t];
         }
@@ -1158,19 +1202,27 @@
     int64_t row_base;
     const int32_t *skip_if = nullptr, *scan_nnz = nullptr;
     int32_t *scan_indptr = nullptr, *scan_total = nullptr;
+    int32_t *apply_long_rows = nullptr;
+    FusedCounters *listed = nullptr;
+    int64_t n_stored = 0;
 };
 static void launch_row_fill_long(int row_class, const xr_mesh *tree, const SearchLists &l, const double *tree_area, bool relative,
                                  const LongRows &r) {
-    allow_dynamic_lds<&k_row_fill_long>(ROW_FILL_LONG_LDS);
     const bool light = row_class == 1;
-    XR_LAUNCH(row_class == 2 ? "row_fill_huge" : "row_fill_long", k_row_fill_long, dim3(engine().num_cu * (light ? 6 : 1)), dim3(256),
-              light ? ROW_FILL_LIGHT_LDS : ROW_FILL_LONG_LDS, l.cand_off.get(), l.cand_count.get(), r.cand_sid, r.cand_area,
-              r.indptr, tree_area, relative, tree->n_face, r.indices, r.data, r.long_rows, r.n_long, r.row_base, r.skip_if,
-              r.scan_nnz, r.scan_indptr, r.scan_total, row_class);
+    auto launch = [&](auto list) {
+        allow_dynamic_lds<&k_row_fill_long<list()>>(ROW_FILL_LONG_LDS);
+        XR_LAUNCH(row_class == 2 ? "row_fill_huge" : "row_fill_long", k_row_fill_long<list()>, dim3(engine().num_cu * (light ? 6 : 1)),
+                  dim3(256), light ? ROW_FILL_LIGHT_LDS : ROW_FILL_LONG_LDS, l.cand_off.get(), l.cand_count.get(), r.cand_sid,
+                  r.cand_area, r.indptr, tree_area, relative, tree->n_face, r.indices, r.data, r.long_rows, r.n_long, r.row_base,
+                  r.skip_if, r.scan_nnz, r.scan_indptr, r.scan_total, row_class, r.apply_long_rows, r.listed, r.n_stored);
+    };
+    if (light && r.apply_long_rows && r.scan_nnz) launch(std::true_type());
+    else launch(std::false_type());
 }
 
 struct EarlyApply {
     std::function<void(const xr_csr *)> fn;
+    bool takes_tail = false;
     bool done = false;
 };
 
@@ -1195,7 +1247,7 @@
     DevBuf<int32_t> slot_face((size_t)T), big_indptr((size_t)T + 1);
     DevBuf<int32_t> cand_tgt((size_t)reg_capacity), cand_src((size_t)reg_capacity), cand_sid((size_t)reg_capacity);
     DevBuf<double> cand_area((size_t)reg_capacity);
-    csr->n_long.alloc(2);
+    csr->n_long.alloc(TAIL_WORDS);
     csr->row_order.alloc((size_t)T);
     csr->has_row_order = true;
     int32_t *const tile_key = csr->has_tile_key ? csr->tile_key.get() : nullptr;
@@ -1242,7 +1294,8 @@
             launch_clip_queue("clip_big", std::integral_constant<int, 2>(), 1, big_queue, big_area.get(), big_sid.get(),
                               &fc->error, l.nnz_row.get(), n_pending_dev, nullptr);
             const LongRows big_rows{big_sid.get(), big_area.get(), big_indptr.get(), big_indices.get(), big_data.get(), slot_face.get(),
-                                    n_big_dev, 0, n_pending_dev, l.nnz_row.get(), big_indptr.get(), &fc->p_big};
+                                    n_big_dev, 0, n_pending_dev, l.nnz_row.get(), big_indptr.get(), &fc->p_big,
+                                    csr->long_rows.get(), fc, T};
             SideForkScope fork;
             launch_row_fill_long(2, tree, l, tree_area, relative, big_rows);
             fork.end_launches();
@@ -1256,27 +1309,31 @@
         XR_LAUNCH("assemble", k_assemble, dim3(grid), dim3(FB), 0, query->qo_bbox(), query->qo_fxy(), query->qo_len(), query->m,
                   query->qo_perm(), T, cand_tgt.get(), l.cand_off.get(), l.cand_count.get(), l.block_seg.get(), l.is_big.get(), cand_area.get(), cand_sid.get(),
                   tree_area, relative, tile, tile_key, fc,
-                  csr->indptr.get(), csr->indices.get(), csr->data.get(), csr->row_order.get(),
-                  csr->long_rows.get(), cap, remap, scan_mode == 1 ? blk_base.get() : (const int32_t *)nullptr,
+                  csr->indptr.get(), csr->indices.get(), csr->data.get(), csr->row_order.get(), cap, remap, scan_mode == 1 ? blk_base.get() : (const int32_t *)nullptr,
                   scan_mode == 1 ? blk_base.get() + grid : (const int32_t *)nullptr,
                   scan_mode == 2 ? blk_rows : (const int32_t *)nullptr, scan_mode == 2 ? blk_surv : (const int32_t *)nullptr);
         side_join();
-        XR_LAUNCH("place_big", k_place_big, dim3(64), dim3(256), 0, n_big_dev, slot_face.get(), big_indptr.get(),
-                  big_indices.get(), big_data.get(), T, query->qo_perm(), query->qo_bbox(), query->qo_fxy(), query->qo_len(),
-                  query->m, tile, tile_key, fc, csr->indptr.get(), csr->indices.get(),
-                  csr->data.get(), csr->row_order.get(), csr->long_rows.get(), cap, n_pending_dev);
+        const PlaceBig place{n_big_dev, slot_face.get(), big_indptr.get(), big_indices.get(), big_data.get(), T, query->qo_perm(),
+                             query->qo_bbox(), query->qo_fxy(), query->qo_len(), query->m, tile, tile_key, fc, csr->indptr.get(),
+                             csr->indices.get(), csr->data.get(), csr->row_order.get(), cap, n_pending_dev};
+        const bool tail_fused = early && early->takes_tail && option(OPT_TAIL_FUSED) != 0;
+        auto enqueue_early = [&](const ApplyTail *tail) {
+            csr->nnz = 0;
+            csr->has_long = true;
+            csr->max_row_len = -1;
+            csr->apply_gated = true;
+            csr->apply_tail = tail;
+            early->fn(csr);
+            csr->apply_tail = nullptr;
+            csr->apply_gated = false;
+        };
+        if (!tail_fused) XR_LAUNCH("place_big", k_place_big, dim3(TAIL_PLACE_BLOCKS), dim3(256), 0, place);
         host_stamp(5);
         const int32_t seq = mailbox_next_seq();
         XR_LAUNCH("publish", k_publish_all, dim3(1), dim3(64), 0, ctl, fc, csr->n_long.get(), mail, seq, cap, big_capacity);
         if (ctl_cached) zero_scratch_done(1);
-        if (early) {
-            csr->nnz = 0;
-            csr->has_long = true;
-            csr->max_row_len = -1;
-            csr->apply_gated = true;
-            early->fn(csr);
-            csr->apply_gated = false;
-        }
+        const ApplyTail tail{place, csr->n_long.get()};
+        if (early) enqueue_early(tail_fused ? &tail : nullptr);
         host_stamp(6);
         mailbox_wait_seq(seq);
         host_stamp(7);
@@ -1473,6 +1530,7 @@
     EarlyApply early;
     early.fn = [&](const xr_csr *c) { csr_apply_dev(c, method, percentile, source_dev, source_dtype, K, out_dev); };
     const bool can_early = K == 1 && method != XR_MODE && method != XR_PERCENTILE;
+    early.takes_tail = can_early;
     overlap(tree, query, relative != 0, csr.get(), can_early ? &early : nullptr);
     host_stamp(8);
     if (!early.done && K > 0) csr_apply_dev(csr.get(), method, percentile, source_dev, source_dtype, K, out_dev);
diff --git a/xugrid_amd/csrc/xr_overlap_fused.h b/xugrid_amd/csrc/xr_overlap_fused.h
--- a/xugrid_amd/csrc/xr_overlap_fused.h
+++ b/xugrid_amd/csrc/xr_overlap_fused.h
@@ -5,32 +5,6 @@
 static constexpr int FB = 256;
 static constexpr int FWAVES = FB / 64;
 
-struct FusedCounters {
-    int32_t n_apply_long;
-    int32_t error;
-    int32_t p_regular;
-    int32_t rows_regular;
-    int32_t p_big;
-    int32_t pad0;
-    int32_t max_row;
-    int32_t pad2;
-};
-
-enum CtlWord : int {
-    CTL_REG_CURSOR = 0,
-    CTL_BIG_CURSOR = 1,
-    CTL_N_BIG = 2,
-    CTL_N_PENDING = 3,
-    CTL_BIG_OVERFLOW = 4,
-    CTL_COUNTERS = 8,
-    CTL_LINE = 16,
-    CTL_REGION_CURSOR = 32,
-    CTL_WORDS = CTL_REGION_CURSOR + 8 * QCUR_STRIDE
-};
-#define XR_CTL_COUNTER(field) (xr::CTL_COUNTERS + (int)(offsetof(xr::FusedCounters, field) / sizeof(int32_t)))
-static_assert(CTL_COUNTERS + sizeof(FusedCounters) / sizeof(int32_t) <= CTL_LINE && CTL_BIG_OVERFLOW < CTL_COUNTERS &&
-                  CTL_LINE <= CTL_REGION_CURSOR && CTL_LINE + 8 <= 64,
-              "the counters lie inside the line k_publish_all's one wave fetches, the region cursors behind it");
 enum MailSlot : int {
     MAIL_REG_PAIRS = 0,
     MAIL_BIG_PAIRS = 1,
@@ -235,7 +209,7 @@
            const int32_t *__restrict__ cand_sid, const double *__restrict__ src_area, bool relative, MortonParams tile,
            int32_t *__restrict__ tile_key, FusedCounters *__restrict__ counters,
            int32_t *__restrict__ indptr, int32_t *__restrict__ indices, double *__restrict__ data, int32_t *__restrict__ row_order,
-           int32_t *__restrict__ apply_long_rows, int64_t csr_capacity, bool remap,
+           int64_t csr_capacity, bool remap,
            const int32_t *__restrict__ base_rows = nullptr, const int32_t *__restrict__ base_nnz = nullptr,
            const int32_t *__restrict__ blk_rows = nullptr, const int32_t *__restrict__ blk_surv = nullptr) {
     __shared__ int32_t sh_stage[SLOTS * FB];
@@ -327,10 +301,6 @@
             const int64_t mid = (t & ~(int64_t)(tile.n_run - 1)) + tile.n_run / 2;
             tile_key[r] = morton_key(tile, query_face_box_rt(q_bbox, q_fxy, q_len, q_m, mid < n_query ? mid : n_query - 1));
         }
-        if (my_nnz > XR_APPLY_LONG_ROW) {
-            apply_long_rows[atomicAdd(&counters->n_apply_long, 1)] = (int32_t)r;
-            atomicMax(&counters->max_row, my_nnz);
-        }
     }
     bool overflow_cap = false;
     for (int i0 = tid; i0 < total; i0 += 4 * FB) {
@@ -365,45 +335,7 @@
 }
 
 
-__global__ void __launch_bounds__(256)
-k_place_big(const int32_t *__restrict__ n_big_dev, const int32_t *__restrict__ slot_face,
-            const int32_t *__restrict__ big_indptr, const int32_t *__restrict__ big_indices,
-            const double *__restrict__ big_data, int64_t n_query, const int32_t *__restrict__ q_perm,
-            const double *__restrict__ q_bbox, const double *__restrict__ q_fxy, const uint8_t *__restrict__ q_len, int q_m,
-            MortonParams tile, int32_t *__restrict__ tile_key,
-            FusedCounters *counters, int32_t *__restrict__ indptr, int32_t *__restrict__ indices,
-            double *__restrict__ data, int32_t *__restrict__ row_order, int32_t *__restrict__ apply_long_rows,
-            int64_t csr_capacity, const int32_t *__restrict__ skip_if) {
-    const int n_big = *n_big_dev;
-    if (n_big == 0 || *skip_if > 0) return;
-    const int64_t p_regular = counters->p_regular, t_reg = n_query - n_big;
-    const int64_t p_big = big_indptr[n_big];
-    if (p_regular + p_big > csr_capacity) {
-        if (blockIdx.x == 0 && threadIdx.x == 0) atomicOr(&counters->error, 4);
-        return;
-    }
-    const int64_t i0 = (int64_t)blockIdx.x * 256 + threadIdx.x, stride = (int64_t)gridDim.x * 256;
-    for (int64_t k = i0; k < n_big; k += stride) {
-        const int f = slot_face[k];
-        const int64_t r = t_reg + k;
-        const int n = big_indptr[k + 1] - big_indptr[k];
-        indptr[r] = (int32_t)(p_regular + big_indptr[k]);
-        row_order[r] = q_perm ? q_perm[f] : f;
-        if (tile_key) {
-            const int64_t mid = ((int64_t)f & ~(int64_t)(tile.n_run - 1)) + tile.n_run / 2;
-            tile_key[r] = morton_key(tile, query_face_box_rt(q_bbox, q_fxy, q_len, q_m, mid < n_query ? mid : n_query - 1));
-        }
-        if (n > XR_APPLY_LONG_ROW) {
-            apply_long_rows[atomicAdd(&counters->n_apply_long, 1)] = (int32_t)r;
-            atomicMax(&counters->max_row, n);
-        }
-    }
-    for (int64_t e = i0; e < p_big; e += stride) {
-        indices[p_regular + e] = big_indices[e];
-        data[p_regular + e] = big_data[e];
-    }
-    if (i0 == 0) indptr[n_query] = (int32_t)(p_regular + p_big);
-}
+__global__ void __launch_bounds__(256) k_place_big(PlaceBig p) { place_big_rows<false>(p, (int)blockIdx.x, (int)gridDim.x); }
 
 __global__ void k_publish_all(int32_t *c , FusedCounters *fc,
                               int32_t *__restrict__ n_apply_long_out, int32_t *mail , int32_t seq, int64_t cap,
@@ -425,13 +357,12 @@
     else if (t == XR_CTL_COUNTER(max_row)) slot = MAIL_MAX_ROW;
     if (slot >= 0) mail[slot] = w;
     if (region_lane) mail[MAIL_REGION_LEN + (t - CTL_LINE)] = cur;
-    if (t == XR_CTL_COUNTER(n_apply_long)) *n_apply_long_out = w;
+    if (t == XR_CTL_COUNTER(n_apply_long)) n_apply_long_out[TAIL_N_LONG] = w;
+    if (t == CTL_N_BIG) n_apply_long_out[TAIL_N_BIG] = w;
+    if (t == XR_CTL_COUNTER(p_regular)) n_apply_long_out[TAIL_P_REGULAR] = w;
     if (t == 0) {
-        const int32_t c_reg = c_reg_sum, c_big = c[CTL_BIG_CURSOR], n_pending = c[CTL_N_PENDING], err = c[XR_CTL_COUNTER(error)],
-                      p_reg = c[XR_CTL_COUNTER(p_regular)], p_big = c[XR_CTL_COUNTER(p_big)];
-        const bool ok = c_reg >= 0 && c_big >= 0 && !(err & (1 | 4 | 8)) && n_pending == 0 && (int64_t)c_big <= big_capacity &&
-                        (int64_t)p_reg + p_big <= cap;
-        n_apply_long_out[1] = ok ? 1 : 0;
+        const bool ok = fused_attempt_final(c, c_reg_sum, cap, big_capacity);
+        n_apply_long_out[TAIL_GATE] = ok ? 1 : 0;
     }
     __builtin_amdgcn_s_waitcnt(0);
     if (t < CTL_LINE) c[t] = 0;
diff --git a/xugrid_amd/csrc/xr_overlap_tail.h b/xugrid_amd/csrc/xr_overlap_tail.h
--- /dev/null
+++ b/xugrid_amd/csrc/xr_overlap_tail.h
@@ -0,0 +1,101 @@
+#pragma once
+#include <cstddef>
+
+#include "xr_geom.h"
+
+namespace xr {
+
+static constexpr int QCUR_STRIDE = 32;
+
+struct FusedCounters {
+    int32_t n_apply_long;
+    int32_t error;
+    int32_t p_regular;
+    int32_t rows_regular;
+    int32_t p_big;
+    int32_t pad0;
+    int32_t max_row;
+    int32_t pad2;
+};
+
+enum CtlWord : int {
+    CTL_REG_CURSOR = 0,
+    CTL_BIG_CURSOR = 1,
+    CTL_N_BIG = 2,
+    CTL_N_PENDING = 3,
+    CTL_BIG_OVERFLOW = 4,
+    CTL_COUNTERS = 8,
+    CTL_LINE = 16,
+    CTL_REGION_CURSOR = 32,
+    CTL_WORDS = CTL_REGION_CURSOR + 8 * QCUR_STRIDE
+};
+#define XR_CTL_COUNTER(field) (xr::CTL_COUNTERS + (int)(offsetof(xr::FusedCounters, field) / sizeof(int32_t)))
+static_assert(CTL_COUNTERS + sizeof(FusedCounters) / sizeof(int32_t) <= CTL_LINE && CTL_BIG_OVERFLOW < CTL_COUNTERS &&
+                  CTL_LINE <= CTL_REGION_CURSOR && CTL_LINE + 8 <= 64,
+              "the counters lie inside the line k_publish_all's one wave fetches, the region cursors behind it");
+
+__device__ __forceinline__ bool fused_attempt_final(const int32_t *c, int32_t c_reg, int64_t cap, int64_t big_capacity) {
+    const int32_t c_big = c[CTL_BIG_CURSOR], n_pending = c[CTL_N_PENDING], err = c[XR_CTL_COUNTER(error)],
+                  p_reg = c[XR_CTL_COUNTER(p_regular)], p_big = c[XR_CTL_COUNTER(p_big)];
+    return c_reg >= 0 && c_big >= 0 && !(err & (1 | 4 | 8)) && n_pending == 0 && (int64_t)c_big <= big_capacity &&
+           (int64_t)p_reg + p_big <= cap;
+}
+
+struct PlaceBig {
+    const int32_t *n_big_dev, *slot_face, *big_indptr, *big_indices;
+    const double *big_data;
+    int64_t n_query;
+    const int32_t *q_perm;
+    const double *q_bbox, *q_fxy;
+    const uint8_t *q_len;
+    int q_m;
+    MortonParams tile;
+    int32_t *tile_key;
+    FusedCounters *counters;
+    int32_t *indptr, *indices;
+    double *data;
+    int32_t *row_order;
+    int64_t csr_capacity;
+    const int32_t *skip_if;
+};
+
+template <bool IN_TAIL>
+__device__ __forceinline__ void place_big_copy(const PlaceBig &p, int n_big, int64_t p_regular, int64_t p_big, int block, int n_blocks) {
+    const int64_t t_reg = p.n_query - n_big;
+    const int64_t i0 = (int64_t)block * 256 + threadIdx.x, stride = (int64_t)n_blocks * 256;
+    for (int64_t k = i0; k < n_big; k += stride) {
+        const int f = p.slot_face[k];
+        const int64_t r = t_reg + k;
+        if (!(IN_TAIL && k == 0)) p.indptr[r] = (int32_t)(p_regular + p.big_indptr[k]);
+        p.row_order[r] = p.q_perm ? p.q_perm[f] : f;
+        if (p.tile_key) {
+            const int64_t mid = ((int64_t)f & ~(int64_t)(p.tile.n_run - 1)) + p.tile.n_run / 2;
+            p.tile_key[r] = morton_key(p.tile, query_face_box_rt(p.q_bbox, p.q_fxy, p.q_len, p.q_m, mid < p.n_query ? mid : p.n_query - 1));
+        }
+    }
+    for (int64_t e = i0; e < p_big; e += stride) {
+        p.indices[p_regular + e] = p.big_indices[e];
+        p.data[p_regular + e] = p.big_data[e];
+    }
+    if (i0 == 0) p.indptr[p.n_query] = (int32_t)(p_regular + p_big);
+}
+template <bool IN_TAIL>
+__device__ __forceinline__ void place_big_rows(const PlaceBig &p, int block, int n_blocks) {
+    const int n_big = *p.n_big_dev;
+    if (n_big == 0 || *p.skip_if > 0) return;
+    const int64_t p_regular = p.counters->p_regular, p_big = p.big_indptr[n_big];
+    if (p_regular + p_big > p.csr_capacity) {
+        if (block == 0 && threadIdx.x == 0) atomicOr(&p.counters->error, 4);
+        return;
+    }
+    place_big_copy<IN_TAIL>(p, n_big, p_regular, p_big, block, n_blocks);
+}
+
+struct ApplyTail {
+    PlaceBig place;
+    const int32_t *words;
+};
+enum TailWord : int { TAIL_N_LONG = 0, TAIL_GATE = 1, TAIL_N_BIG = 2, TAIL_P_REGULAR = 3, TAIL_WORDS = 4 };
+static constexpr int TAIL_PLACE_BLOCKS = 64;
+
+}
diff --git a/xugrid_amd/engine.py b/xugrid_amd/engine.py
--- a/xugrid_amd/engine.py
+++ b/xugrid_amd/engine.py
@@ -1125,6 +1125,13 @@
         check(_lib.load().xr_csr_row_order(self._h, 0, _ptr(out)))
         return out
 
+    def long_rows(self):
+        n = ctypes.c_int64()
+        check(_lib.load().xr_csr_long_rows(self._h, 0, None, ctypes.byref(n)))
+        out = np.empty(n.value, dtype=np.int64)
+        check(_lib.load().xr_csr_long_rows(self._h, n.value, _ptr(out), ctypes.byref(n)))
+        return out
+
     def download(self):
         data = np.empty(self.nnz, dtype=np.float64)
         indices = np.empty(self.nnz, dtype=np.int64)
```

After: 2.199 billion target cells/s, median of 6. 1.6% higher.
